# Cyruscxy/TinyPathTracer

Measured on AMD Instinct MI355X. Metric: Mrays/s at 1920x1080x1024spp (box.gltf, 8 bounces); achieved GB/s vs peak, higher is better.
Workload: dtype f32

## Files before the change

### include/tpt.h

```cpp
#ifndef TPT_H
#define TPT_H

#include <stdint.h>
#include <stddef.h>

#ifdef __cplusplus
extern "C" {
#endif

#define TPT_VERSION_MAJOR 0
#define TPT_VERSION_MINOR 1

typedef enum {
    TPT_OK = 0,
    TPT_ERR_INVALID_ARG = 1,
    TPT_ERR_HIP = 2,
    TPT_ERR_OOM = 3,
    TPT_ERR_IO = 4,
    TPT_ERR_PARSE = 5,
    TPT_ERR_NO_DEVICE = 6
} tpt_status;

typedef struct {
    float base_color[3];
    float emission_factor;
    float eta;
    float metallic;
    float subsurface, specular, roughness, specular_tint, anisotropic,
          sheen, sheen_tint, clearcoat, clearcoat_gloss;
} tpt_material;

typedef struct {
    int32_t type;
    float color[3];
    float intensity;
    float pos[3];
    float direction[3];
    float cos_outer;
    float inv_cos_cone_diff;
} tpt_light;

typedef struct {
    int32_t begin;
    int32_t mtl;
} tpt_interval;

typedef struct {
    const uint32_t* indices;      uint32_t n_faces;
    const float* vertices;        const float* normals;  uint32_t n_vertices;
    const tpt_interval* lut;      uint32_t n_objects;
    const float* vert_trans;      const float* normal_trans;
    const tpt_material* materials; uint32_t n_materials;
    const tpt_light* lights;      uint32_t n_lights;
    uint32_t flags;
} tpt_scene_desc;

#define TPT_DESC_DELTALIGHT_LAYOUT 0x1

typedef struct {
    float c2w[16];
    float vfov;
    float aspect;
    float znear;
} tpt_camera;

typedef struct {
    int32_t width, height;
    int32_t spp;
    int32_t max_depth;
    uint64_t seed;
    int32_t band_rows, band_count, band_index;
    int32_t spp_per_launch;
    int32_t flags;
    int32_t refill;
    int32_t pipe_sets, pipe_chunks;
    int32_t lanes_per_pixel;
    int32_t leaf_batch;
    int32_t wf_slots, wf_refill;
    int32_t band_list_len;
    const int32_t* band_list;
    float* band_cost;
} tpt_params;

#define TPT_FLAG_NO_COUNTERS   0x1
#define TPT_FLAG_REF_ORDER     0x2
#define TPT_FLAG_ENV_IS        0x8
#define TPT_FLAG_APPROX_CULL   0x10
#define TPT_FLAG_WAVEFRONT     0x20
#define TPT_FLAG_FAST          0x40
#define TPT_FLAG_ACCUMULATE    0x4

typedef struct {
    uint64_t traversals;
    uint64_t internal_visits;
    uint64_t leaf_tests;
    uint64_t shade_hits;
    uint64_t pixels;
    uint64_t samples;
    double rng_init_ms;
    double trace_ms;
    double resolve_ms;
    double total_ms;
    int32_t trace_launches;
    int32_t pad;
    uint64_t wide_visits;
    uint64_t accumulated_spp;
    double trace_kernel_ms;
    uint64_t local_rays;
    double tree_wait_ms;
    uint64_t resident_lanes;
    int32_t lanes_per_pixel;
    int32_t drained;
} tpt_stats;

typedef struct tpt_scene tpt_scene;
typedef struct tpt_env tpt_env;

const char* tpt_version(void);
const char* tpt_last_error(void);
int tpt_device_count(void);

tpt_status tpt_scene_create(const tpt_scene_desc* desc, int device, tpt_scene** out);
tpt_status tpt_scene_build(tpt_scene* scene);
tpt_status tpt_scene_build_async(tpt_scene* scene);
tpt_status tpt_scene_set_build_threads(tpt_scene* scene, int32_t threads);
tpt_status tpt_scene_set_transforms(tpt_scene* scene, uint32_t first_object, uint32_t n_objects,
                                    const float* vert_trans, const float* normal_trans);
void tpt_scene_destroy(tpt_scene* scene);

tpt_status tpt_env_create(const uint8_t* rgba, int32_t width, int32_t height, int device, tpt_env** out);
void tpt_env_destroy(tpt_env* env);

tpt_status tpt_env_load(const char* path, int device, tpt_env** out);
tpt_status tpt_image_load(const char* path, uint8_t** rgba, int32_t* width, int32_t* height);
void tpt_image_free(uint8_t* rgba);
tpt_status tpt_render(tpt_scene* scene, const tpt_env* env, const tpt_camera* camera,
                      const tpt_params* params, float* radiance_out, uint8_t* bgra_out,
                      tpt_stats* stats);

tpt_status tpt_render_frames(tpt_scene* scene, const tpt_env* env, const tpt_camera* camera,
                             const tpt_params* params, int32_t n_frames, const uint64_t* seeds,
                             float* const* radiance_outs, uint8_t* const* bgra_outs, tpt_stats* stats);


typedef struct {
    float*   albedo;
    float*   normal;
    float*   depth;
    int32_t* face;
    int32_t* material;
} tpt_aov;

tpt_status tpt_render_aov(tpt_scene* scene, const tpt_camera* camera, int32_t width, int32_t height,
                          const tpt_aov* out, double* trace_ms);

#define TPT_DENOISE_DEMODULATE 0x1
#define TPT_DENOISE_DIRECT     0x2

typedef struct {
    int32_t iterations;
    float   sigma_color;
    float   sigma_normal;
    float   sigma_depth;
    int32_t flags;
} tpt_denoise_params;

typedef struct { double pack_ms, filter_ms, resolve_ms; } tpt_denoise_stats;

tpt_status tpt_denoise(tpt_scene* scene, int32_t width, int32_t height, const float* radiance_in,
                       const tpt_aov* guides, const tpt_denoise_params* params, float* radiance_out,
                       uint8_t* bgra_out, tpt_denoise_stats* stats);

typedef struct tpt_history tpt_history;
tpt_status tpt_history_create(tpt_scene* scene, int32_t width, int32_t height, tpt_history** out);
tpt_status tpt_history_reset(tpt_history* h);
void tpt_history_destroy(tpt_history* h);

#define TPT_TEMPORAL_DEMODULATE 0x1
#define TPT_TEMPORAL_TILES      0x2

typedef struct {
    float   alpha;
    float   depth_tol;
    float   normal_min;
    int32_t max_history;
    int32_t flags;
} tpt_temporal_params;

typedef struct {
    double   kernel_ms;
    uint64_t reprojected;
} tpt_temporal_stats;

tpt_status tpt_temporal(tpt_history* h, const tpt_camera* camera, const float* radiance_in,
                        const tpt_aov* guides, const tpt_temporal_params* params,
                        float* radiance_out, float* variance_out, float* history_len_out,
                        uint8_t* bgra_out, tpt_temporal_stats* stats);

tpt_status tpt_temporal_motion(tpt_history* h, const tpt_camera* camera, const float* radiance_in,
                               const tpt_aov* guides, const tpt_temporal_params* params,
                               float* radiance_out, float* variance_out, float* history_len_out,
                               float* motion_out, uint8_t* bgra_out, tpt_temporal_stats* stats);

#define TPT_SVGF_DEMODULATE 0x1
#define TPT_SVGF_DIRECT     0x2

typedef struct {
    int32_t iterations;
    float   sigma_lum;
    float   sigma_normal;
    float   sigma_depth;
    int32_t min_history;
    int32_t flags;
} tpt_svgf_params;

typedef struct {
    double   pack_ms, estimate_ms, filter_ms, resolve_ms;
    uint64_t estimated;
} tpt_svgf_stats;

tpt_status tpt_denoise_svgf(tpt_scene* scene, int32_t width, int32_t height, const float* radiance_in,
                            const tpt_aov* guides, const float* variance_in, const float* history_len_in,
                            const tpt_svgf_params* params, float* radiance_out, float* variance_out,
                            uint8_t* bgra_out, tpt_svgf_stats* stats);

tpt_status tpt_scene_read_bvh(tpt_scene* scene, void* nodes36, int64_t* keys);
tpt_status tpt_scene_read_world(tpt_scene* scene, float* wverts, float* wnorms);
tpt_status tpt_debug_rng_init(int device, uint64_t seed, uint64_t first_pixel, uint32_t n, uint32_t* states);
tpt_status tpt_debug_trace_rays(tpt_scene* scene, uint32_t n, const float* origins, const float* dirs,
                                const int32_t* origin_fid, int32_t mode, int32_t* hit, float* t, float* uv);
tpt_status tpt_debug_hot_kat(int device, int32_t op, uint32_t n, const float* in, float* out);
tpt_status tpt_debug_step_latency(tpt_scene* scene, uint32_t n, const float* origins, const float* dirs,
                                  int32_t mode, int32_t flags, uint64_t* out);
int32_t tpt_wide_tree_build(int32_t n, const float* leaf_box, const uint32_t* leaf_emit, float* nodes,
                            int32_t cap, int32_t* stack_need, int32_t threads);

int32_t tpt_motion_matrices(uint32_t n_objects, const float* prev16, const float* cur16, float* out24);

typedef struct tpt_gltf tpt_gltf;
tpt_status tpt_gltf_load(const char* path, tpt_gltf** out);
tpt_status tpt_gltf_desc(const tpt_gltf* g, tpt_scene_desc* desc, tpt_camera* camera);
int tpt_gltf_missing_material(const tpt_gltf* g);
void tpt_gltf_free(tpt_gltf* g);

#ifdef __cplusplus
}
#endif
#endif
```

### tinypathtracer_amd/_lib.py

```python
from __future__ import annotations

import ctypes as C
import os

HERE = os.path.dirname(os.path.abspath(__file__))
LIB_PATH = os.environ.get("TPT_LIB", os.path.join(HERE, "libtpt.so"))

TPT_OK = 0
STATUS_NAMES = {0: "OK", 1: "INVALID_ARG", 2: "HIP_ERROR", 3: "OOM", 4: "IO", 5: "PARSE", 6: "NO_DEVICE"}
FLAG_NO_COUNTERS = 0x1
FLAG_REF_ORDER = 0x2
FLAG_ACCUMULATE = 0x4
FLAG_ENV_IS = 0x8
FLAG_APPROX_CULL = 0x10
FLAG_WAVEFRONT = 0x20
FLAG_FAST = 0x40
DESC_DELTALIGHT_LAYOUT = 0x1
DENOISE_DEMODULATE = 0x1
DENOISE_DIRECT = 0x2
TEMPORAL_DEMODULATE = 0x1
TEMPORAL_TILES = 0x2
MOTION_TRACKED, MOTION_IDENTITY, MOTION_UNTRACKED = 0, 1, 2
SVGF_DEMODULATE = 0x1
SVGF_DIRECT = 0x2


class Material(C.Structure):
    _fields_ = [("base_color", C.c_float * 3), ("emission_factor", C.c_float), ("eta", C.c_float),
                ("metallic", C.c_float), ("subsurface", C.c_float), ("specular", C.c_float),
                ("roughness", C.c_float), ("specular_tint", C.c_float), ("anisotropic", C.c_float),
                ("sheen", C.c_float), ("sheen_tint", C.c_float), ("clearcoat", C.c_float),
                ("clearcoat_gloss", C.c_float)]


class Light(C.Structure):
    _fields_ = [("type", C.c_int32), ("color", C.c_float * 3), ("intensity", C.c_float),
                ("pos", C.c_float * 3), ("direction", C.c_float * 3), ("cos_outer", C.c_float),
                ("inv_cos_cone_diff", C.c_float)]


class Interval(C.Structure):
    _fields_ = [("begin", C.c_int32), ("mtl", C.c_int32)]


class SceneDesc(C.Structure):
    _fields_ = [("indices", C.POINTER(C.c_uint32)), ("n_faces", C.c_uint32),
                ("vertices", C.POINTER(C.c_float)), ("normals", C.POINTER(C.c_float)),
                ("n_vertices", C.c_uint32), ("lut", C.POINTER(Interval)), ("n_objects", C.c_uint32),
                ("vert_trans", C.POINTER(C.c_float)), ("normal_trans", C.POINTER(C.c_float)),
                ("materials", C.POINTER(Material)), ("n_materials", C.c_uint32),
                ("lights", C.POINTER(Light)), ("n_lights", C.c_uint32), ("flags", C.c_uint32)]


class Camera(C.Structure):
    _fields_ = [("c2w", C.c_float * 16), ("vfov", C.c_float), ("aspect", C.c_float), ("znear", C.c_float)]


class Params(C.Structure):
    _fields_ = [("width", C.c_int32), ("height", C.c_int32), ("spp", C.c_int32), ("max_depth", C.c_int32),
                ("seed", C.c_uint64), ("band_rows", C.c_int32), ("band_count", C.c_int32),
                ("band_index", C.c_int32), ("spp_per_launch", C.c_int32), ("flags", C.c_int32),
                ("refill", C.c_int32), ("pipe_sets", C.c_int32), ("pipe_chunks", C.c_int32),
                ("lanes_per_pixel", C.c_int32), ("leaf_batch", C.c_int32), ("wf_slots", C.c_int32),
                ("wf_refill", C.c_int32), ("band_list_len", C.c_int32), ("band_list", C.POINTER(C.c_int32)),
                ("band_cost", C.POINTER(C.c_float))]


class SvgfParams(C.Structure):
    _fields_ = [("iterations", C.c_int32), ("sigma_lum", C.c_float), ("sigma_normal", C.c_float),
                ("sigma_depth", C.c_float), ("min_history", C.c_int32), ("flags", C.c_int32)]


class SvgfStats(C.Structure):
    _fields_ = [("pack_ms", C.c_double), ("estimate_ms", C.c_double), ("filter_ms", C.c_double),
                ("resolve_ms", C.c_double), ("estimated", C.c_uint64)]

    def as_dict(self):
        return {k: getattr(self, k) for k, _ in self._fields_}


class Stats(C.Structure):
    _fields_ = [("traversals", C.c_uint64), ("internal_visits", C.c_uint64), ("leaf_tests", C.c_uint64),
                ("shade_hits", C.c_uint64), ("pixels", C.c_uint64), ("samples", C.c_uint64),
                ("rng_init_ms", C.c_double), ("trace_ms", C.c_double), ("resolve_ms", C.c_double),
                ("total_ms", C.c_double), ("trace_launches", C.c_int32), ("pad", C.c_int32),
                ("wide_visits", C.c_uint64), ("accumulated_spp", C.c_uint64), ("trace_kernel_ms", C.c_double),
                ("local_rays", C.c_uint64), ("tree_wait_ms", C.c_double), ("resident_lanes", C.c_uint64),
                ("lanes_per_pixel", C.c_int32), ("drained", C.c_int32)]

    def as_dict(self):
        return {k: getattr(self, k) for k, _ in self._fields_ if k != "pad"}


class Aov(C.Structure):
    _fields_ = [("albedo", C.c_void_p), ("normal", C.c_void_p), ("depth", C.c_void_p), ("face", C.c_void_p),
                ("material", C.c_void_p)]


class DenoiseParams(C.Structure):
    _fields_ = [("iterations", C.c_int32), ("sigma_color", C.c_float), ("sigma_normal", C.c_float),
                ("sigma_depth", C.c_float), ("flags", C.c_int32)]


class DenoiseStats(C.Structure):
    _fields_ = [("pack_ms", C.c_double), ("filter_ms", C.c_double), ("resolve_ms", C.c_double)]

    def as_dict(self):
        return {k: getattr(self, k) for k, _ in self._fields_}


class TemporalParams(C.Structure):
    _fields_ = [("alpha", C.c_float), ("depth_tol", C.c_float), ("normal_min", C.c_float),
                ("max_history", C.c_int32), ("flags", C.c_int32)]


class TemporalStats(C.Structure):
    _fields_ = [("kernel_ms", C.c_double), ("reprojected", C.c_uint64)]

    def as_dict(self):
        return {k: getattr(self, k) for k, _ in self._fields_}


SIGNATURES = [
    ("tpt_version", C.c_char_p, []),
    ("tpt_last_error", C.c_char_p, []),
    ("tpt_device_count", C.c_int, []),
    ("tpt_scene_create", C.c_int, [C.POINTER(SceneDesc), C.c_int, C.POINTER(C.c_void_p)]),
    ("tpt_scene_build", C.c_int, [C.c_void_p]),
    ("tpt_scene_build_async", C.c_int, [C.c_void_p]),
    ("tpt_scene_set_build_threads", C.c_int, [C.c_void_p, C.c_int32]),
    ("tpt_scene_set_transforms", C.c_int, [C.c_void_p, C.c_uint32, C.c_uint32, C.c_void_p, C.c_void_p]),
    ("tpt_scene_destroy", None, [C.c_void_p]),
    ("tpt_env_create", C.c_int, [C.c_void_p, C.c_int32, C.c_int32, C.c_int, C.POINTER(C.c_void_p)]),
    ("tpt_env_destroy", None, [C.c_void_p]),
    ("tpt_env_load", C.c_int, [C.c_char_p, C.c_int, C.POINTER(C.c_void_p)]),
    ("tpt_image_load", C.c_int, [C.c_char_p, C.POINTER(C.POINTER(C.c_uint8)), C.POINTER(C.c_int32),
                                 C.POINTER(C.c_int32)]),
    ("tpt_image_free", None, [C.c_void_p]),
    ("tpt_render", C.c_int, [C.c_void_p, C.c_void_p, C.POINTER(Camera), C.POINTER(Params), C.c_void_p,
                             C.c_void_p, C.POINTER(Stats)]),
    ("tpt_render_frames", C.c_int, [C.c_void_p, C.c_void_p, C.POINTER(Camera), C.POINTER(Params), C.c_int32,
                                    C.POINTER(C.c_uint64), C.POINTER(C.c_void_p), C.POINTER(C.c_void_p),
                                    C.POINTER(Stats)]),
    ("tpt_render_aov", C.c_int, [C.c_void_p, C.POINTER(Camera), C.c_int32, C.c_int32, C.POINTER(Aov),
                                 C.POINTER(C.c_double)]),
    ("tpt_denoise", C.c_int, [C.c_void_p, C.c_int32, C.c_int32, C.c_void_p, C.POINTER(Aov),
                              C.POINTER(DenoiseParams), C.c_void_p, C.c_void_p, C.POINTER(DenoiseStats)]),
    ("tpt_history_create", C.c_int, [C.c_void_p, C.c_int32, C.c_int32, C.POINTER(C.c_void_p)]),
    ("tpt_history_reset", C.c_int, [C.c_void_p]),
    ("tpt_history_destroy", None, [C.c_void_p]),
    ("tpt_temporal", C.c_int, [C.c_void_p, C.POINTER(Camera), C.c_void_p, C.POINTER(Aov),
                               C.POINTER(TemporalParams), C.c_void_p, C.c_void_p, C.c_void_p, C.c_void_p,
                               C.POINTER(TemporalStats)]),
    ("tpt_temporal_motion", C.c_int, [C.c_void_p, C.POINTER(Camera), C.c_void_p, C.POINTER(Aov),
                                      C.POINTER(TemporalParams), C.c_void_p, C.c_void_p, C.c_void_p, C.c_void_p,
                                      C.c_void_p, C.POINTER(TemporalStats)]),
    ("tpt_motion_matrices", C.c_int32, [C.c_uint32, C.c_void_p, C.c_void_p, C.c_void_p]),
    ("tpt_denoise_svgf", C.c_int, [C.c_void_p, C.c_int32, C.c_int32, C.c_void_p, C.POINTER(Aov), C.c_void_p,
                                   C.c_void_p, C.POINTER(SvgfParams), C.c_void_p, C.c_void_p, C.c_void_p,
                                   C.POINTER(SvgfStats)]),
    ("tpt_scene_read_bvh", C.c_int, [C.c_void_p, C.c_void_p, C.c_void_p]),
    ("tpt_scene_read_world", C.c_int, [C.c_void_p, C.c_void_p, C.c_void_p]),
    ("tpt_debug_rng_init", C.c_int, [C.c_int, C.c_uint64, C.c_uint64, C.c_uint32, C.c_void_p]),
    ("tpt_debug_trace_rays", C.c_int, [C.c_void_p, C.c_uint32, C.c_void_p, C.c_void_p, C.c_void_p, C.c_int32,
                                       C.c_void_p, C.c_void_p, C.c_void_p]),
    ("tpt_debug_hot_kat", C.c_int, [C.c_int, C.c_int32, C.c_uint32, C.c_void_p, C.c_void_p]),
    ("tpt_debug_step_latency", C.c_int, [C.c_void_p, C.c_uint32, C.c_void_p, C.c_void_p, C.c_int32, C.c_int32,
                                         C.c_void_p]),
    ("tpt_wide_tree_build", C.c_int32, [C.c_int32, C.c_void_p, C.c_void_p, C.c_void_p, C.c_int32,
                                        C.POINTER(C.c_int32), C.c_int32]),
    ("tpt_gltf_load", C.c_int, [C.c_char_p, C.POINTER(C.c_void_p)]),
    ("tpt_gltf_desc", C.c_int, [C.c_void_p, C.POINTER(SceneDesc), C.POINTER(Camera)]),
    ("tpt_gltf_missing_material", C.c_int, [C.c_void_p]),
    ("tpt_gltf_free", None, [C.c_void_p]),
]


class TPTError(RuntimeError):
    def __init__(self, status, msg):
        super().__init__(f"tpt error {STATUS_NAMES.get(status, status)}: {msg}")
        self.status = status


_lib = None


def build_identity() -> dict:
    import hashlib
    h = hashlib.sha256()
    with open(LIB_PATH, "rb") as f:
        for chunk in iter(lambda: f.read(1 << 20), b""):
            h.update(chunk)
    ident = {"lib_sha256": h.hexdigest()[:16], "git_head": None}
    try:
        with open(os.path.splitext(LIB_PATH)[0] + ".build") as f:
            ident["git_head"] = f.read().strip() or None
    except OSError:
        pass
    return ident


def lib():
    global _lib
    if _lib is None:
        try:
            import torch
        except Exception:
            pass
        if not os.path.exists(LIB_PATH):
            raise ImportError(f"libtpt.so not found at {LIB_PATH}: build it with "
                              f"`make -C {HERE}` or __graft_entry__.build()")
        L = C.CDLL(LIB_PATH)
        older = bool(os.environ.get("TPT_LIB"))
        for name, res, args in SIGNATURES:
            if older and name.startswith("tpt_debug_") and not hasattr(L, name):
                continue
            fn = getattr(L, name)
            fn.restype = res
            fn.argtypes = args
        _lib = L
    return _lib


def check(status):
    if status != TPT_OK:
        raise TPTError(status, lib().tpt_last_error().decode(errors="replace"))
```

### tinypathtracer_amd/csrc/common/device_api.hpp

```cpp
#pragma once

#include <hip/hip_runtime_api.h>
#include <stdint.h>

namespace tpt {

struct DevLight {
    int32_t type;
    float color[3];
    float intensity;
    float pos[3];
    float dir[3];
    float cos_outer;
    float inv_cos_cone_diff;
};

constexpr int kMaxLights = 16;
constexpr int kRngJumps = 16;
constexpr int kJumpWords = 160 * 5;

struct TraceArgs {
    const float4* inner;
    const float4* inner4;
    int32_t n4;
    int32_t lds_nodes;
    int32_t lds_nodes_offset;
    const float4* tri;
    const float4* shade;
    const float4* mtl;
    int32_t n_faces;
    int32_t n_materials;
    int32_t n_lights;
    int32_t stack_depth;
    const DevLight* lights;
    const uint32_t* env;
    int32_t env_w, env_h;
    int32_t is_b, is_bw, is_bh;
    const float* is_cond;
    const float* is_row;
    const float* is_marg;
    float is_total;
    const int32_t* is_guide_r;
    const int32_t* is_guide_c;
    int32_t is_kr, is_kc;
    int32_t env_is;
    float c2w[16];
    float origin[3];
    float sensor_w, sensor_h;
    float half_sw, half_sh;
    float inv_w, inv_h;
    int32_t width, height;
    int32_t band_rows, band_count, band_index, band_height;
    const int32_t* band_list;
    unsigned long long* band_cost;
    int32_t n_frames;
    int32_t max_depth;
    int32_t samples;
    int32_t flags;
    int32_t refill;
    int32_t leaf_kb;
    int32_t boxes_finite;
    int32_t any_emitter;
    int32_t emit_root;
    float4 emit_box[8];
    int32_t n_emit_box;
    const float4* sliver_groups;
    const float4* sliver_list;
    int32_t n_sliver_groups;
    float cull_eps;
    int32_t graze;
    int32_t pair;
    int32_t drained;
    int32_t quad;
    int32_t xcd_run;
    int32_t xcd_rot;
    int32_t lds_rec_offset;
    int32_t rec_lds_levels;
    int32_t stack_lds_slots;
    int32_t lds_stack_offset;
    int32_t lds_mtl_offset;
    int32_t mtl_in_lds;
    uint32_t* rng;
    float* accum;
    unsigned long long* counters;
    unsigned long long* debug_waves;
};

__host__ __device__ inline int rec_words(int n_lights, int n_materials) {
    return (n_lights > 0 || n_materials >= 0x7ffe) ? 5 : 2;
}

struct ResolveArgs {
    const float* accum;
    float* radiance;
    uint8_t* bgra;
    int32_t width, height;
    int32_t band_rows, band_count, band_index, band_height;
    const int32_t* band_list;
    int32_t spp;
};

hipError_t launch_rng_init(const uint32_t* jumps, uint64_t seed, int32_t width, int32_t band_rows,
                           int32_t band_count, int32_t band_index, const int32_t* band_list, int32_t band_height,
                           int32_t height, uint32_t* rng, hipStream_t s);
hipError_t launch_rng_init_linear(const uint32_t* jumps, uint64_t seed, uint64_t first, uint32_t n,
                                  uint32_t* states_aos, hipStream_t s);

struct BuildBuffers {
    int32_t n_faces, n_vertices, n_objects, n_materials;
    const uint32_t* indices;
    const float* vertices;
    const float* normals;
    const int2* lut;
    const float* vert_trans;
    const float* normal_trans;
    const float4* mtl;
    float* wverts;
    float* wnorms;
    unsigned long long* keys;
    unsigned long long* keys_sorted;
    uint32_t* fids;
    uint32_t* fids_sorted;
    float* leaf_box;
    int2* children;
    uint32_t* parent;
    float* node_box;
    uint32_t* flags;
    uint32_t* max_depth;
    unsigned long long* bfs_keys;
    unsigned long long* bfs_keys_sorted;
    uint32_t* bfs_ids;
    uint32_t* bfs_ids_sorted;
    uint32_t* bfs_newid;
    uint32_t* emit;
    void* sort_tmp;
    size_t sort_tmp_bytes;
    float4* inner;
    float4* inner4;
    float4* tri;
    float4* shade;
    void* nodes36;
    uint32_t out_max_depth;
    uint32_t out_boxes_finite;
    uint32_t out_n4;
};
constexpr uint32_t kMaxLbvhDepth = 4096;
hipError_t build_sort_tmp_bytes(int32_t n, size_t* bytes);
hipError_t launch_build(BuildBuffers& b, hipStream_t s);
hipError_t launch_sliver_scan(const float4* tri, int32_t n, uint8_t* sliver, unsigned long long* coord_max,
                              hipStream_t s);

constexpr int kWfShards = 8;
constexpr int kWfCtlStride = 1024;
constexpr int kWfCtlWords = (4 * kWfShards + 1) * kWfCtlStride;
struct WfArgs {
    TraceArgs t;
    int32_t n_slots;
    int32_t state_words;
    int32_t rec_words;
    int32_t ordered;
    uint32_t* st0;
    uint32_t* st1;
    float* rec;
    float4* q_ray0;
    float4* q_ray1;
    float4* q_hit;
    uint32_t* ctl;
    int32_t shard_cap;
    int32_t n_claims;
    int32_t refill;
    int32_t chunk;
    int32_t batch;
    int32_t logic_blocks, trace_blocks;
    int32_t it;
    int32_t stack_lds_slots, lds_stack_offset, lds_bytes;
};
hipError_t launch_wavefront(WfArgs w, uint32_t* h_count, hipEvent_t ev[2], int32_t* iterations, hipStream_t s);

hipError_t launch_trace(const TraceArgs& a, hipStream_t s);
bool trace_quad_fits(const TraceArgs& a);
int trace_waves_per_simd();
hipError_t launch_trace_ptr(const void* a, hipStream_t s);
hipError_t launch_step_latency_ptr(const void* a, uint32_t n, const float* o, const float* d, int nodes_lds,
                                   unsigned long long* out, hipStream_t s);
hipError_t launch_resolve(const ResolveArgs& a, hipStream_t s);
hipError_t launch_hot_kat(int op, uint32_t n, const float* in, float* out, hipStream_t s);
hipError_t launch_trace_rays(const TraceArgs& a, uint32_t n, const float* o, const float* d, const int32_t* ofid,
                             int mode, int32_t* hit, float* t, float* uv, hipStream_t s);

struct AovArgs {
    float* albedo;
    float* normal;
    float* depth;
    int32_t* face;
    int32_t* material;
};
hipError_t launch_aov(const TraceArgs& a, const AovArgs& o, hipStream_t s);

struct DenoiseArgs {
    const float* radiance_in;
    const float* albedo;
    const float* normal;
    const float* depth;
    float4* color0;
    float4* guide;
    float* radiance_out;
    uint8_t* bgra;
    size_t npix;
    int32_t width, height;
    int32_t demodulate;
};
struct AtrousArgs {
    const float4* src;
    const float4* guide;
    float4* dst;
    int32_t width, height;
    int32_t step;
    float inv_sc2;
    float inv_sn2;
    float sz2;
};
hipError_t launch_denoise_pack(const DenoiseArgs& a, hipStream_t s);
hipError_t launch_atrous(const AtrousArgs& a, bool use_lds, hipStream_t s);
hipError_t launch_denoise_resolve(const DenoiseArgs& a, hipStream_t s);

struct TemporalArgs {
    float c2w[16];
    float origin[3];
    float sensor_w, sensor_h, half_sw, half_sh;
    float inv_w, inv_h;
    float prev_inv[16];
    float prev_origin[3];
    float prev_sensor_w, prev_sensor_h, prev_half_sw, prev_half_sh;
    int32_t has_prev;
    int32_t width, height;
    int32_t demodulate;
    int32_t tiles;
    float alpha, depth_tol, normal_min, max_history;
    const float* radiance_in;
    const float* albedo;
    const float* normal;
    const float* depth;
    const int32_t* material;
    const float4* prev[3];
    float4* next[3];
    float* radiance_out;
    float* variance_out;
    float* history_out;
    uint8_t* bgra;
    unsigned long long* reprojected;
};
constexpr int kTemporalSlots = 256;
constexpr int kTemporalSlotStride = 16;
hipError_t launch_temporal(const TemporalArgs& a, hipStream_t s);

struct MotionArgs {
    const int32_t* face;
    const int32_t* face_object;
    const float4* records;
    float* motion_out;
    int32_t n_faces;
};
constexpr int kMotionRecordFloats = 24;
constexpr int32_t kMotionTracked = 0, kMotionIdentity = 1, kMotionUntracked = 2;
hipError_t launch_temporal_motion(const TemporalArgs& a, const MotionArgs& mo, hipStream_t s);

struct SvgfArgs {
    const float* radiance_in;
    const float* albedo;
    const float* normal;
    const float* depth;
    const float* variance_in;
    const float* history_len;
    const float4* src;
    float4* dst;
    float4* guide;
    float* radiance_out;
    float* variance_out;
    uint8_t* bgra;
    unsigned long long* estimated;
    size_t npix;
    int32_t width, height;
    int32_t demodulate;
    int32_t passthrough;
    float min_history;
    float inv_sn2;
    float sz2;
};
struct SvgfFilterArgs {
    const float4* src;
    const float4* guide;
    float4* dst;
    int32_t width, height;
    int32_t step;
    float sigma_lum;
    float inv_sn2;
    float sz2;
};
hipError_t launch_svgf_pack(const SvgfArgs& a, hipStream_t s);
hipError_t launch_svgf_estimate(const SvgfArgs& a, hipStream_t s);
hipError_t launch_svgf_filter(const SvgfFilterArgs& a, bool use_lds, hipStream_t s);
hipError_t launch_svgf_resolve(const SvgfArgs& a, hipStream_t s);

}

namespace tpt_fast {
hipError_t launch_trace_ptr(const void* a, hipStream_t s);
hipError_t launch_step_latency_ptr(const void* a, uint32_t n, const float* o, const float* d, int nodes_lds,
                                   unsigned long long* out, hipStream_t s);
}
```

### tinypathtracer_amd/csrc/host/api.cpp

```cpp
#include <cstdlib>
#include <new>

#include "api_internal.hpp"

static thread_local std::string g_last_error;

tpt_status tpt::host::fail(tpt_status st, const std::string& msg) {
    g_last_error = msg;
    return st;
}

extern "C" {

const char* tpt_version(void) { return "tpt-mi355x 0.1 (gfx950)"; }

const char* tpt_last_error(void) { return g_last_error.c_str(); }

int tpt_device_count(void) {
    int n = 0;
    if (hipGetDeviceCount(&n) != hipSuccess) {
        (void)hipGetLastError();
        return 0;
    }
    return n;
}

tpt_status tpt_image_load(const char* path, uint8_t** rgba, int32_t* width, int32_t* height) {
    if (!path || !rgba || !width || !height) return fail(TPT_ERR_INVALID_ARG, "null argument");
    *rgba = nullptr;
    std::vector<uint8_t> px;
    int w = 0, h = 0;
    try {
        tpt::load_image(path, px, w, h);
    } catch (const tpt::io_error& e) {
        return fail(TPT_ERR_IO, e.what());
    } catch (const std::exception& e) {
        return fail(TPT_ERR_PARSE, e.what());
    }
    uint8_t* buf = static_cast<uint8_t*>(std::malloc(px.size()));
    if (!buf) return fail(TPT_ERR_OOM, "host allocation failed");
    std::memcpy(buf, px.data(), px.size());
    *rgba = buf;
    *width = w;
    *height = h;
    return TPT_OK;
}

void tpt_image_free(uint8_t* rgba) { std::free(rgba); }

tpt_status tpt_scene_read_bvh(tpt_scene* s, void* nodes36, int64_t* keys) {
    if (!s || !s->built) return fail(TPT_ERR_INVALID_ARG, "scene not built");
    DeviceGuard g(s->device);
    const size_t n = (size_t)s->n_faces;
    if (nodes36) HIP_OR_FAIL(hipMemcpy(nodes36, s->nodes36.p, 36 * (2 * n - 1), hipMemcpyDeviceToHost));
    if (keys) HIP_OR_FAIL(hipMemcpy(keys, s->keys_sorted.p, 8 * n, hipMemcpyDeviceToHost));
    return TPT_OK;
}

tpt_status tpt_scene_read_world(tpt_scene* s, float* wv, float* wn) {
    if (!s || !s->built) return fail(TPT_ERR_INVALID_ARG, "scene not built");
    DeviceGuard g(s->device);
    const size_t nv = (size_t)s->n_vertices;
    if (wv) HIP_OR_FAIL(hipMemcpy(wv, s->wverts.p, 12 * nv, hipMemcpyDeviceToHost));
    if (wn) HIP_OR_FAIL(hipMemcpy(wn, s->wnorms.p, 12 * nv, hipMemcpyDeviceToHost));
    return TPT_OK;
}

tpt_status tpt_debug_rng_init(int device, uint64_t seed, uint64_t first, uint32_t n, uint32_t* states) {
    if (!states && n) return fail(TPT_ERR_INVALID_ARG, "null output");
    int ndev = tpt_device_count();
    if (ndev <= 0) return fail(TPT_ERR_NO_DEVICE, "no HIP device available");
    if (device < 0 || device >= ndev) return fail(TPT_ERR_INVALID_ARG, "bad device index");
    DeviceGuard g(device);
    DevBuf<uint32_t> jumps, out;
    const auto& hj = host_jumps();
    HIP_OR_FAIL(jumps.upload(hj.data(), hj.size(), nullptr));
    HIP_OR_FAIL(out.alloc(6 * (size_t)std::max(n, 1u)));
    HIP_OR_FAIL(tpt::launch_rng_init_linear(jumps.p, seed, first, n, out.p, nullptr));
    HIP_OR_FAIL(hipDeviceSynchronize());
    if (n) HIP_OR_FAIL(hipMemcpy(states, out.p, 24 * (size_t)n, hipMemcpyDeviceToHost));
    return TPT_OK;
}

tpt_status tpt_debug_trace_rays(tpt_scene* s, uint32_t n, const float* o, const float* d, const int32_t* origin_fid,
                                int32_t mode, int32_t* hit, float* t, float* uv) {
    if (!s || !s->built) return fail(TPT_ERR_INVALID_ARG, "scene not built");
    if (mode < 0 || mode > 3) return fail(TPT_ERR_INVALID_ARG, "unknown trace mode");
    {
        const tpt_status bs = finish_pending(s);
        if (bs != TPT_OK) return bs;
    }
    if (n && (!o || !d || !hit || !t || !uv)) return fail(TPT_ERR_INVALID_ARG, "null argument");
    DeviceGuard g(s->device);
    DevBuf<float> dorg, ddir, dt, duv;
    DevBuf<int32_t> dhit, dofid;
    HIP_OR_FAIL(dorg.upload(o, 3 * (size_t)n, s->stream));
    if (origin_fid) {
        for (uint32_t i = 0; i < n; ++i)
            if (origin_fid[i] >= s->n_faces) return fail(TPT_ERR_INVALID_ARG, "origin face out of range");
        HIP_OR_FAIL(dofid.upload(origin_fid, n, s->stream));
    }
    HIP_OR_FAIL(ddir.upload(d, 3 * (size_t)n, s->stream));
    HIP_OR_FAIL(dhit.alloc(n));
    HIP_OR_FAIL(dt.alloc(n));
    HIP_OR_FAIL(duv.alloc(2 * (size_t)n));
    tpt::TraceArgs a{};
    fill_trace_args(s, nullptr, nullptr, a);
    HIP_OR_FAIL(tpt::launch_trace_rays(a, n, dorg.p, ddir.p, origin_fid ? dofid.p : nullptr, mode, dhit.p, dt.p, duv.p,
                                       s->stream));
    HIP_OR_FAIL(hipStreamSynchronize(s->stream));
    if (n) {
        HIP_OR_FAIL(hipMemcpy(hit, dhit.p, 4 * (size_t)n, hipMemcpyDeviceToHost));
        HIP_OR_FAIL(hipMemcpy(t, dt.p, 4 * (size_t)n, hipMemcpyDeviceToHost));
        HIP_OR_FAIL(hipMemcpy(uv, duv.p, 8 * (size_t)n, hipMemcpyDeviceToHost));
    }
    return TPT_OK;
}

tpt_status tpt_debug_step_latency(tpt_scene* s, uint32_t n, const float* o, const float* d, int32_t mode,
                                  int32_t flags, uint64_t* out) {
    if (!s || !s->built) return fail(TPT_ERR_INVALID_ARG, "scene not built");
    if (n > 64 || (n && (!o || !d || !out))) return fail(TPT_ERR_INVALID_ARG, "1..64 rays and outputs");
    if (mode < 0 || mode > 2)
        return fail(TPT_ERR_INVALID_ARG, "mode: 0 nodes in global memory, 1 in LDS, 2 four lanes per ray");
    if (mode == 2 && n > 16) return fail(TPT_ERR_INVALID_ARG, "four lanes per ray: at most 16 rays");
    {
        const tpt_status bs = finish_pending(s);
        if (bs != TPT_OK) return bs;
    }
    const int nodes_lds = mode == 1 ? s->n4 : (mode == 2 ? -1 : 0);
    if ((size_t)std::max(nodes_lds, 0) * 128 + 64 * 256 * sizeof(int) > 160 * 1024)
        return fail(TPT_ERR_INVALID_ARG, "the 4-wide tree does not fit in LDS");
    DeviceGuard g(s->device);
    DevBuf<float> dorg, ddir;
    DevBuf<unsigned long long> dout;
    HIP_OR_FAIL(dorg.upload(o, 3 * (size_t)std::max(n, 1u), s->stream));
    HIP_OR_FAIL(ddir.upload(d, 3 * (size_t)std::max(n, 1u), s->stream));
    HIP_OR_FAIL(dout.alloc(4 * 64));
    tpt::TraceArgs a{};
    fill_trace_args(s, nullptr, nullptr, a);
    if (mode == 2 && a.stack_depth + 3 > 64) return fail(TPT_ERR_INVALID_ARG, "four lanes per ray: stack too deep");
    if (flags & TPT_FLAG_FAST) {
        a.cull_eps = 0.0f;
        a.n_sliver_groups = 0;
        a.graze = 0;
        HIP_OR_FAIL(tpt_fast::launch_step_latency_ptr(&a, n, dorg.p, ddir.p, nodes_lds, dout.p, s->stream));
    } else {
        HIP_OR_FAIL(tpt::launch_step_latency_ptr(&a, n, dorg.p, ddir.p, nodes_lds, dout.p, s->stream));
    }
    HIP_OR_FAIL(hipStreamSynchronize(s->stream));
    HIP_OR_FAIL(hipMemcpy(out, dout.p, 4 * 64 * sizeof(unsigned long long), hipMemcpyDeviceToHost));
    return TPT_OK;
}

tpt_status tpt_debug_hot_kat(int device, int32_t op, uint32_t n, const float* in, float* out) {
    static const int kIn[4] = {12, 15, 16, 3}, kOut[4] = {2, 4, 6, 3};
    if (op < 0 || op > 3) return fail(TPT_ERR_INVALID_ARG, "unknown KAT op");
    if (n && (!in || !out)) return fail(TPT_ERR_INVALID_ARG, "null argument");
    int ndev = tpt_device_count();
    if (ndev <= 0) return fail(TPT_ERR_NO_DEVICE, "no HIP device available");
    if (device < 0 || device >= ndev) return fail(TPT_ERR_INVALID_ARG, "bad device index");
    DeviceGuard g(device);
    DevBuf<float> din, dout;
    HIP_OR_FAIL(din.upload(in, (size_t)kIn[op] * n, nullptr));
    HIP_OR_FAIL(dout.alloc((size_t)kOut[op] * std::max(n, 1u)));
    HIP_OR_FAIL(tpt::launch_hot_kat(op, n, din.p, dout.p, nullptr));
    HIP_OR_FAIL(hipDeviceSynchronize());
    if (n) HIP_OR_FAIL(hipMemcpy(out, dout.p, sizeof(float) * kOut[op] * (size_t)n, hipMemcpyDeviceToHost));
    return TPT_OK;
}

tpt_status tpt_gltf_load(const char* path, tpt_gltf** out) {
    if (!path || !out) return fail(TPT_ERR_INVALID_ARG, "null argument");
    *out = nullptr;
    tpt_gltf* g = new (std::nothrow) tpt_gltf();
    if (!g) return fail(TPT_ERR_OOM, "host allocation failed");
    try {
        tpt::load_gltf(path, g->hs);
    } catch (const tpt::io_error& e) {
        delete g;
        return fail(TPT_ERR_IO, e.what());
    } catch (const std::exception& e) {
        delete g;
        return fail(TPT_ERR_PARSE, e.what());
    }
    *out = g;
    return TPT_OK;
}

tpt_status tpt_gltf_desc(const tpt_gltf* g, tpt_scene_desc* d, tpt_camera* cam) {
    if (!g || !d) return fail(TPT_ERR_INVALID_ARG, "null argument");
    const tpt::HostScene& h = g->hs;
    d->indices = h.indices.data();
    d->n_faces = (uint32_t)(h.indices.size() / 3);
    d->vertices = h.vertices.data();
    d->normals = h.normals.data();
    d->n_vertices = (uint32_t)(h.vertices.size() / 3);
    d->lut = h.lut.data();
    d->n_objects = (uint32_t)h.lut.size();
    d->vert_trans = h.vert_trans.data();
    d->normal_trans = h.normal_trans.data();
    d->materials = h.materials.empty() ? nullptr : h.materials.data();
    d->n_materials = (uint32_t)h.materials.size();
    d->lights = h.lights.empty() ? nullptr : h.lights.data();
    d->n_lights = (uint32_t)h.lights.size();
    d->flags = 0;
    if (cam) *cam = h.camera;
    return TPT_OK;
}

int tpt_gltf_missing_material(const tpt_gltf* g) { return g && g->hs.missing_material ? 1 : 0; }

void tpt_gltf_free(tpt_gltf* g) { delete g; }

}
```

### tinypathtracer_amd/csrc/host/api_render.cpp

```cpp
#include <chrono>
#include <cstdio>
#include <cstdlib>

#include "api_internal.hpp"

#ifndef TPT_XCD_ROT
#define TPT_XCD_ROT 1
#endif

void tpt::host::fill_trace_args(tpt_scene* s, const tpt_env* env, const tpt_camera* cam, tpt::TraceArgs& a) {
    a.inner = s->inner.p;
    a.inner4 = s->inner4.p;
    a.n4 = s->n4;
    a.tri = s->tri.p;
    a.shade = s->shade.p;
    a.mtl = s->mtl.p;
    a.n_faces = s->n_faces;
    a.n_materials = s->n_materials;
    a.n_lights = s->n_lights;
    a.lights = s->lights.p;
    a.stack_depth = s->stack_depth;
    a.boxes_finite = s->boxes_finite;
    a.any_emitter = s->any_emitter;
    a.emit_root = s->emit_root;
    a.n_emit_box = s->any_emitter ? s->n_emit_box : 0;
    for (int k = 0; k < a.n_emit_box; ++k) {
        const float* b = s->emit_box + 6 * k;
        a.emit_box[2 * k] = make_float4(b[0], b[1], b[2], 0.0f);
        a.emit_box[2 * k + 1] = make_float4(b[3], b[4], b[5], 0.0f);
    }
    a.sliver_groups = s->sliver_groups.p;
    a.sliver_list = s->sliver_list.p;
    a.n_sliver_groups = s->n_sliver_groups;
    a.cull_eps = s->cull_eps;
    a.graze = 1;
    a.env = env ? env->texels.p : nullptr;
    a.env_w = env ? env->w : 0;
    a.env_h = env ? env->h : 0;
    a.is_b = env ? env->is_b : 1;
    a.is_bw = env ? env->is_bw : 0;
    a.is_bh = env ? env->is_bh : 0;
    a.is_cond = env ? env->is_cond.p : nullptr;
    a.is_row = env ? env->is_row.p : nullptr;
    a.is_marg = env ? env->is_marg.p : nullptr;
    a.is_total = env ? env->is_total : 0.0f;
    a.is_guide_r = env ? env->is_guide_r.p : nullptr;
    a.is_guide_c = env ? env->is_guide_c.p : nullptr;
    a.is_kr = env ? env->is_kr : 1;
    a.is_kc = env ? env->is_kc : 1;
    if (cam) set_camera(a, camera_consts(cam));
}

namespace {

tpt_status render_wavefront(tpt_scene* s, const tpt::TraceArgs& a, const tpt_params* p, int n_frames, int bh,
                            double& trace_ms, double& kernel_ms, int& launches) {
    hipStream_t st = s->stream;
    const bool ordered = !(p->flags & TPT_FLAG_REF_ORDER);
    const bool lights = !ordered || a.env_is || tpt::rec_words(s->n_lights, s->n_materials) == 5;
    tpt::WfArgs w{};
    w.t = a;
    w.t.samples = p->spp;
    w.ordered = ordered ? 1 : 0;
    w.state_words = lights ? 32 : 16;
    w.rec_words = lights ? 5 : 2;
    const size_t gx = (size_t)(p->width + 15) / 16, gy = (size_t)((bh + 15) / 16) * (size_t)n_frames;
    const size_t claims = gx * gy * 256;
    if (bh <= 0) return TPT_OK;
    if (claims > (size_t)INT32_MAX / 2) return fail(TPT_ERR_INVALID_ARG, "wavefront: frame batch too large");
    if (p->wf_slots < 0 || p->wf_refill < 0 || p->wf_refill > 64)
        return fail(TPT_ERR_INVALID_ARG, "wavefront: wf_slots >= 0, wf_refill 0..64");
    size_t slots = p->wf_slots > 0 ? (size_t)p->wf_slots : claims;
    slots = std::min(slots, claims);
    slots = (slots + 255) / 256 * 256;
    w.n_claims = (int32_t)claims;
    w.n_slots = (int32_t)slots;
    HIP_OR_FAIL(s->wf_rec.alloc(slots * (size_t)p->max_depth * (size_t)w.rec_words));
    const size_t cap = ((slots / 256) + tpt::kWfShards - 1) / tpt::kWfShards * 256;
    const size_t qn = cap * tpt::kWfShards;
    HIP_OR_FAIL(s->wf_q0.alloc(2 * qn));
    HIP_OR_FAIL(s->wf_q1.alloc(2 * qn));
    HIP_OR_FAIL(s->wf_hit.alloc(qn));
    HIP_OR_FAIL(s->wf_state.alloc(2 * qn * (size_t)w.state_words));
    HIP_OR_FAIL(s->wf_ctl.alloc(tpt::kWfCtlWords));
    HIP_OR_FAIL(s->wf_count.alloc(2 * tpt::kWfShards));
    w.shard_cap = (int32_t)cap;
    for (auto& e : s->wf_ev)
        if (!e) HIP_OR_FAIL(hipEventCreateWithFlags(&e, hipEventDisableTiming));
    w.st0 = s->wf_state.p;
    w.st1 = s->wf_state.p + qn * (size_t)w.state_words;
    w.rec = s->wf_rec.p;
    w.q_ray0 = s->wf_q0.p;
    w.q_ray1 = s->wf_q1.p;
    w.q_hit = s->wf_hit.p;
    w.ctl = s->wf_ctl.p;
    w.refill = p->wf_refill > 0 ? p->wf_refill : 40;
    w.chunk = 128;
    w.batch = 32;
    w.logic_blocks = (int32_t)((std::min<size_t>((slots + 255) / 256, 2048) + tpt::kWfShards - 1) / tpt::kWfShards *
                               tpt::kWfShards);
    w.trace_blocks = 0;
    int32_t iters = 0;
    HIP_OR_FAIL(tpt::launch_wavefront(w, s->wf_count.p, s->wf_ev, &iters, st));
    HIP_OR_FAIL(hipEventRecord(s->ev[2], st));
    HIP_OR_FAIL(hipEventSynchronize(s->ev[2]));
    float ms = 0.0f;
    HIP_OR_FAIL(hipEventElapsedTime(&ms, s->ev[1], s->ev[2]));
    trace_ms = ms;
    kernel_ms = ms;
    launches = 1 + 2 * iters;
    return TPT_OK;
}

struct WaveDump {
    const char* path = nullptr;
    size_t words = 0;
};

tpt_status render_planned(tpt_scene* s, const tpt::TraceArgs& a, const tpt_params* p, const tpt::LaunchPlan& plan,
                          size_t list_len, WaveDump& dump, double& trace_ms, double& kernel_ms, int& launches) {
    hipStream_t st = s->stream;
    const int nset = plan.nset;
    const size_t nf = (size_t)a.n_frames;
    const bool listed = a.band_list != nullptr;
#if defined(TPT_PROFILE_PHASES) || defined(TPT_VERIFY_CULL)
    dump.path = std::getenv("TPT_DEBUG_WAVES");
#endif
    const size_t dbg_launch =
        8ull * 4 * (size_t)((a.width + 7) / 8) * (size_t)((std::max(a.band_height, 1) + 7) / 8) * nf;
    dump.words = dbg_launch * std::max<size_t>(plan.launches.size(), 1);
    if (dump.path) {
        HIP_OR_FAIL(s->debug.alloc(dump.words));
        HIP_OR_FAIL(hipMemsetAsync(s->debug.p, 0, dump.words * sizeof(unsigned long long), st));
    }
    HIP_OR_FAIL(s->ensure_launch_events(2 * plan.launches.size()));
    if (listed && nset > 1) {
        for (int k = 0; k < nset; ++k)
            std::copy(plan.set_list[k].begin(), plan.set_list[k].end(), s->band_lists_h.begin() + plan.set_off[k]);
        HIP_OR_FAIL(hipMemcpyAsync(s->band_lists.p + list_len, s->band_lists_h.data() + list_len,
                                   list_len * sizeof(int32_t), hipMemcpyHostToDevice, st));
    }
    hipStream_t qs[tpt::kMaxPipe] = {st};
    if (nset > 1) {
        HIP_OR_FAIL(s->ensure_pipe(nset));
        HIP_OR_FAIL(hipEventRecord(s->pipe_ev[0], st));
        for (int k = 0; k < nset; ++k) {
            qs[k] = s->pipe[k];
            HIP_OR_FAIL(hipStreamWaitEvent(qs[k], s->pipe_ev[0], 0));
        }
    }
#define SET_OR_FAIL(expr)                                                                                      \
    do {                                                                                                       \
        hipError_t e_ = (expr);                                                                                \
        if (e_ != hipSuccess) {                                                                                \
            for (int k_ = 0; nset > 1 && k_ < nset; ++k_) (void)hipStreamSynchronize(qs[k_]);                  \
            (void)hipStreamSynchronize(st);                                                                    \
            return fail(e_ == hipErrorOutOfMemory ? TPT_ERR_OOM : TPT_ERR_HIP,                                 \
                        std::string(#expr) + ": " + hipGetErrorString(e_));                                    \
        }                                                                                                      \
    } while (0)
    int set_chunks[tpt::kMaxPipe] = {};
    for (size_t oi = 0; oi < plan.order.size(); ++oi) {
        const size_t j = plan.order[oi];
        const int k = plan.launches[j].set;
        if (plan.set_rows[k] <= 0) continue;
        tpt::TraceArgs ak = a;
        ak.samples = plan.launches[j].samples;
        ak.xcd_rot = TPT_XCD_ROT ? (set_chunks[k]++ & 7) : 0;
        if (nset > 1) {
            ak.band_count = a.band_count * nset;
            ak.band_index = a.band_index + k * a.band_count;
            ak.band_height = plan.set_rows[k];
            if (listed) ak.band_list = s->band_lists.p + plan.set_off[k];
        }
#ifdef TPT_VERIFY_CULL
        if (dump.path) ak.debug_waves = s->debug.p;
#else
        if (dump.path) ak.debug_waves = s->debug.p + oi * dbg_launch;
#endif
        SET_OR_FAIL(hipEventRecord(s->lev[2 * j], qs[k]));
        SET_OR_FAIL((p->flags & TPT_FLAG_FAST) ? tpt_fast::launch_trace_ptr(&ak, qs[k]) : tpt::launch_trace(ak, qs[k]));
        SET_OR_FAIL(hipEventRecord(s->lev[2 * j + 1], qs[k]));
    }
    for (int k = 0; nset > 1 && k < nset; ++k) {
        SET_OR_FAIL(hipEventRecord(s->pipe_ev[1 + k], qs[k]));
        SET_OR_FAIL(hipStreamWaitEvent(st, s->pipe_ev[1 + k], 0));
    }
    SET_OR_FAIL(hipEventRecord(s->ev[2], st));
    SET_OR_FAIL(hipEventSynchronize(s->ev[2]));
#undef SET_OR_FAIL
    float ms = 0.0f;
    HIP_OR_FAIL(hipEventElapsedTime(&ms, s->ev[1], s->ev[2]));
    trace_ms = ms;
    for (size_t j = 0; j < plan.launches.size(); ++j) {
        if (plan.set_rows[plan.launches[j].set] <= 0) continue;
        HIP_OR_FAIL(hipEventElapsedTime(&ms, s->lev[2 * j], s->lev[2 * j + 1]));
        kernel_ms += ms;
        ++launches;
    }
    return TPT_OK;
}

}

extern "C" {

tpt_status tpt_render(tpt_scene* s, const tpt_env* env, const tpt_camera* cam, const tpt_params* p,
                      float* radiance_out, uint8_t* bgra_out, tpt_stats* stats) {
    if (!p) return fail(TPT_ERR_INVALID_ARG, "null argument");
    const uint64_t seed = p->seed;
    return tpt_render_frames(s, env, cam, p, 1, &seed, &radiance_out, &bgra_out, stats);
}

tpt_status tpt_render_frames(tpt_scene* s, const tpt_env* env, const tpt_camera* cam, const tpt_params* p,
                             int32_t n_frames, const uint64_t* seeds, float* const* radiance_outs,
                             uint8_t* const* bgra_outs, tpt_stats* stats) {
    auto t_start = std::chrono::steady_clock::now();
    if (!s || !cam || !p || !seeds) return fail(TPT_ERR_INVALID_ARG, "null argument");
    if (n_frames < 1 || n_frames > 65535) return fail(TPT_ERR_INVALID_ARG, "bad frame count");
    if (!s->built) return fail(TPT_ERR_INVALID_ARG, "scene not built (call tpt_scene_build)");
    if (p->width <= 0 || p->height <= 0 || p->spp <= 0 || p->max_depth < 1 || p->max_depth > 64)
        return fail(TPT_ERR_INVALID_ARG, "bad frame parameters");
    if ((int64_t)p->width * p->height > (int64_t)1 << 30) return fail(TPT_ERR_INVALID_ARG, "frame too large");
    const int band_rows = p->band_rows > 0 ? p->band_rows : 16;
    const bool listed = p->band_list != nullptr;
    const int band_count = listed ? 1 : (p->band_count > 0 ? p->band_count : 1);
    const int band_index = listed ? 0 : p->band_index;
    if (!listed && (p->band_index < 0 || p->band_index >= band_count))
        return fail(TPT_ERR_INVALID_ARG, "bad band index");
    if (env && env->device != s->device) return fail(TPT_ERR_INVALID_ARG, "env lives on another device");
    const int W = p->width, H = p->height;
    const int n_bands = (H + band_rows - 1) / band_rows;
    std::vector<int32_t> list;
    if (listed) {
        if (p->band_list_len < 0 || p->band_list_len > n_bands)
            return fail(TPT_ERR_INVALID_ARG, "band_list_len: 0 .. ceil(height / band_rows)");
        list.assign(p->band_list, p->band_list + p->band_list_len);
        std::vector<uint8_t> seen((size_t)n_bands, 0);
        const bool partial = H % band_rows != 0;
        for (size_t i = 0; i < list.size(); ++i) {
            if (list[i] < 0 || list[i] >= n_bands || seen[(size_t)list[i]]++ ||
                (partial && list[i] == n_bands - 1 && i + 1 != list.size()))
                return fail(TPT_ERR_INVALID_ARG, "band_list: distinct band ids below ceil(height / band_rows), "
                                                 "a short last band last");
        }
    }
    DeviceGuard g(s->device);
    hipStream_t st = s->stream;
    const size_t npix = (size_t)W * (size_t)H;
    const size_t nf = (size_t)n_frames;
    const int bh = listed ? tpt::band_list_rows(list.data(), list.size(), band_rows, H)
                          : tpt::band_height_of(H, band_rows, band_count, band_index);
    const std::vector<uint64_t> fseeds(seeds, seeds + nf);

    const bool resume = (p->flags & TPT_FLAG_ACCUMULATE) && s->acc_valid && s->acc_w == W && s->acc_h == H &&
                        s->acc_rows == band_rows && s->acc_count == band_count && s->acc_index == band_index &&
                        s->acc_list == list && s->acc_seeds == fseeds && s->rng.n == 6 * npix * nf &&
                        s->accum.n == 3 * npix * nf;
    s->acc_valid = false;
    HIP_OR_FAIL(s->rng.alloc(6 * npix * nf));
    HIP_OR_FAIL(s->accum.alloc(3 * npix * nf));
    HIP_OR_FAIL(s->counters.alloc(32));
    if (!resume) HIP_OR_FAIL(hipMemsetAsync(s->accum.p, 0, 3 * npix * nf * sizeof(float), st));
    HIP_OR_FAIL(hipMemsetAsync(s->counters.p, 0, 32 * sizeof(unsigned long long), st));
    const int32_t* d_list = nullptr;
    if (listed && !list.empty()) {
        s->band_lists_h.assign(2 * list.size(), 0);
        std::copy(list.begin(), list.end(), s->band_lists_h.begin());
        HIP_OR_FAIL(s->band_lists.alloc(std::max(s->band_lists.n, 2 * list.size())));
        HIP_OR_FAIL(hipMemcpyAsync(s->band_lists.p, s->band_lists_h.data(), list.size() * sizeof(int32_t),
                                   hipMemcpyHostToDevice, st));
        d_list = s->band_lists.p;
    }
    if (p->band_cost) {
        HIP_OR_FAIL(s->band_cost.alloc(std::max<size_t>(s->band_cost.n, (size_t)n_bands)));
        HIP_OR_FAIL(hipMemsetAsync(s->band_cost.p, 0, (size_t)n_bands * sizeof(unsigned long long), st));
    }

    HIP_OR_FAIL(hipEventRecord(s->ev[0], st));
    if (bh > 0 && !resume)
        for (size_t f = 0; f < nf; ++f)
            HIP_OR_FAIL(tpt::launch_rng_init(s->jumps.p, fseeds[f], W, band_rows, band_count, band_index, d_list, bh,
                                             H, s->rng.p + f * 6 * npix, st));
    HIP_OR_FAIL(hipEventRecord(s->ev[1], st));
    double tree_wait_ms = 0.0;
    {
        const tpt_status bs = finish_pending(s, &tree_wait_ms);
        if (bs != TPT_OK) return bs;
    }
    const uint64_t total_spp = (resume ? s->acc_spp : 0) + (uint64_t)p->spp;
    if (total_spp > (uint64_t)INT32_MAX) return fail(TPT_ERR_INVALID_ARG, "accumulated spp overflow");

    tpt::TraceArgs a{};
    fill_trace_args(s, env, cam, a);
    a.inv_w = 1.0f / (float)W;
    a.inv_h = 1.0f / (float)H;
    a.width = W;
    a.height = H;
    a.band_rows = band_rows;
    a.band_count = band_count;
    a.band_index = band_index;
    a.band_list = d_list;
    a.band_cost = p->band_cost ? s->band_cost.p : nullptr;
    a.band_height = bh;
    a.n_frames = n_frames;
    a.max_depth = p->max_depth;
    a.flags = p->flags;
    if (p->flags & (TPT_FLAG_APPROX_CULL | TPT_FLAG_FAST)) {
        a.cull_eps = 0.0f;
        a.n_sliver_groups = 0;
        a.graze = 0;
    }
    a.env_is = ((p->flags & TPT_FLAG_ENV_IS) && env && env->is_total > 0.0f) ? 1 : 0;
    a.rng = s->rng.p;
    a.accum = s->accum.p;
    a.counters = s->counters.p;
    a.debug_waves = nullptr;

    tpt::PlanInput pin;
    pin.width = W;
    pin.band_rows = band_rows;
    pin.bh = bh;
    pin.height = H;
    pin.n_frames = n_frames;
    pin.band_count = band_count;
    pin.band_index = band_index;
    pin.listed = listed;
    pin.list = list.data();
    pin.list_len = list.size();
    pin.spp = p->spp;
    pin.flags = p->flags;
    pin.lanes_per_pixel = p->lanes_per_pixel;
    pin.refill = p->refill;
    pin.leaf_batch = p->leaf_batch;
    pin.spp_per_launch = p->spp_per_launch;
    pin.pipe_sets = p->pipe_sets;
    pin.pipe_chunks = p->pipe_chunks;
    pin.n_faces = s->n_faces;
    pin.n_lights = s->n_lights;
    pin.n_materials = s->n_materials;
    pin.resident_lanes = s->resident_lanes;
    pin.env_is = a.env_is != 0;
    pin.quad_fits = tpt::trace_quad_fits(a);
    const tpt::LaunchPlan plan = tpt::plan_launches(pin);
    if (plan.status != TPT_OK) return fail(plan.status, plan.message);
    a.pair = plan.pair ? 1 : 0;
    a.quad = plan.quad ? 1 : 0;
    a.refill = plan.refill;
    a.drained = plan.drained ? 1 : 0;
    a.leaf_kb = plan.leaf_kb;
    a.xcd_run = plan.xcd_run;
    a.xcd_rot = 0;

    double trace_ms = 0.0, kernel_ms = 0.0;
    int launches = 0;
    WaveDump dump;
    if ((p->flags & TPT_FLAG_WAVEFRONT) && (p->flags & (TPT_FLAG_FAST | TPT_FLAG_APPROX_CULL)))
        return fail(TPT_ERR_INVALID_ARG, "TPT_FLAG_WAVEFRONT runs the exact traversal only");
    const tpt_status ts = (p->flags & TPT_FLAG_WAVEFRONT)
                              ? render_wavefront(s, a, p, n_frames, bh, trace_ms, kernel_ms, launches)
                              : render_planned(s, a, p, plan, list.size(), dump, trace_ms, kernel_ms, launches);
    if (ts != TPT_OK) return ts;

    HIP_OR_FAIL(hipEventRecord(s->ev[2], st));
    Staging sg(st);
    for (size_t f = 0; f < nf; ++f) {
        tpt::ResolveArgs r{};
        r.accum = s->accum.p + f * 3 * npix;
        r.width = W;
        r.height = H;
        r.band_rows = band_rows;
        r.band_count = band_count;
        r.band_index = band_index;
        r.band_list = d_list;
        r.band_height = bh;
        r.spp = (int)total_spp;
        HIP_OR_FAIL(sg.inout(s->radiance_tmp, radiance_outs ? radiance_outs[f] : nullptr, 3 * npix, &r.radiance));
        HIP_OR_FAIL(sg.inout(s->bgra_tmp, bgra_outs ? bgra_outs[f] : nullptr, 4 * npix, &r.bgra));
        if (bh > 0 && (r.radiance || r.bgra)) HIP_OR_FAIL(tpt::launch_resolve(r, st));
        HIP_OR_FAIL(sg.finish());
    }
    HIP_OR_FAIL(hipEventRecord(s->ev[3], st));
    unsigned long long cnt[32] = {0};
    HIP_OR_FAIL(hipMemcpyAsync(cnt, s->counters.p, sizeof cnt, hipMemcpyDeviceToHost, st));
    HIP_OR_FAIL(hipStreamSynchronize(st));
    if (cnt[4] != 0) return fail(TPT_ERR_HIP, "traversal stack overflow (BVH deeper than sized)");
    if (p->band_cost) {
        s->band_cost_h.resize((size_t)n_bands);
        HIP_OR_FAIL(hipMemcpy(s->band_cost_h.data(), s->band_cost.p, (size_t)n_bands * sizeof(unsigned long long),
                              hipMemcpyDeviceToHost));
        for (int b = 0; b < n_bands; ++b) {
            const bool mine = listed ? std::find(list.begin(), list.end(), b) != list.end()
                                     : b % band_count == band_index;
            if (mine) p->band_cost[b] = (float)((double)s->band_cost_h[(size_t)b] / 100.0);
        }
    }
    if (dump.path) {
#ifdef TPT_VERIFY_CULL
        const size_t dump_words = std::min<size_t>(dump.words, 16 * std::min<unsigned long long>(cnt[24], 4096));
#else
        const size_t dump_words = dump.words;
#endif
        std::vector<unsigned long long> h(dump_words);
        if (dump_words)
            HIP_OR_FAIL(hipMemcpy(h.data(), s->debug.p, dump_words * sizeof(unsigned long long), hipMemcpyDeviceToHost));
        if (FILE* f = std::fopen(dump.path, "wb")) {
            std::fwrite(h.data(), sizeof(unsigned long long), h.size(), f);
            std::fclose(f);
        }
    }
#if defined(TPT_PROFILE_PHASES) || defined(TPT_VERIFY_CULL)
    if (std::getenv("TPT_DEBUG_COUNTERS")) {
        std::fprintf(stderr, "tpt counters:");
        for (int i = 0; i < 32; ++i) std::fprintf(stderr, " %llu", cnt[i]);
        std::fprintf(stderr, "\n");
    }
#endif
    if (stats) {
        std::memset(stats, 0, sizeof *stats);
        stats->traversals = cnt[0];
        stats->internal_visits = cnt[1];
        stats->wide_visits = cnt[5];
        stats->local_rays = cnt[9];
        stats->accumulated_spp = total_spp;
        stats->leaf_tests = cnt[2];
        stats->shade_hits = cnt[3];
        stats->pixels = (uint64_t)W * (uint64_t)bh * (uint64_t)nf;
        stats->samples = stats->pixels * (uint64_t)p->spp;
        float ms = 0.0f;
        (void)hipEventElapsedTime(&ms, s->ev[0], s->ev[1]);
        stats->rng_init_ms = ms;
        stats->trace_ms = trace_ms;
        stats->trace_kernel_ms = kernel_ms;
        stats->tree_wait_ms = tree_wait_ms;
        (void)hipEventElapsedTime(&ms, s->ev[2], s->ev[3]);
        stats->resolve_ms = ms;
        stats->trace_launches = launches;
        stats->resident_lanes = s->resident_lanes;
        stats->lanes_per_pixel = plan.quad ? 4 : (plan.pair_kernel ? 2 : 1);
        stats->drained = a.drained;
        stats->total_ms =
            std::chrono::duration<double, std::milli>(std::chrono::steady_clock::now() - t_start).count();
    }
    s->acc_valid = true;
    s->acc_w = W;
    s->acc_h = H;
    s->acc_rows = band_rows;
    s->acc_count = band_count;
    s->acc_index = band_index;
    s->acc_list = list;
    s->acc_seeds = fseeds;
    s->acc_spp = total_spp;
    return TPT_OK;
}

}
```

### tinypathtracer_amd/csrc/kernels/trace.hip

```cpp
#include <type_traits>

#include "trace_dev.hpp"

namespace tpt {
#ifdef TPT_VERIFY_CULL
template <bool ORDERED>
__device__ __forceinline__ void trav_lane(Trav& r, const TraceArgs& a, LaneStack<int>& stk, uint32_t& c_ovf);
constexpr unsigned long long kVerifyCap = 4096;
__device__ __noinline__ void verify_ray(const TraceArgs& a, const Trav& r, int phase, const float4* mtl) {
    Trav q;
    trav_begin(q, r.o, r.d, TM_CLOSEST);
    LaneStack<int> vs;
    vs.lds = nullptr;
    vs.nlds = 0;
    uint32_t ovf = 0;
    trav_lane<false>(q, a, vs, ovf);
    bool bad;
    if (r.mode == TM_ANY) {
        bad = (q.fid >= 0) != (r.fid >= 0);
    } else if (r.mode == TM_CLOSEST && phase != 3) {
        bad = (q.fid != r.fid) || (__float_as_uint(q.t) != __float_as_uint(r.t)) ||
              (__float_as_uint(q.u) != __float_as_uint(r.u)) || (__float_as_uint(q.v) != __float_as_uint(r.v));
    } else {
        const float er = q.fid >= 0 ? mtl[2 * __float_as_int(a.shade[3 * q.fid].w)].w : 0.0f;
        const float eo = (r.fid >= 0 && r.mode != TM_OCCLUDED) ? mtl[2 * __float_as_int(a.shade[3 * r.fid].w)].w : 0.0f;
        bad = er != eo;
    }
    if (!bad) return;
    const unsigned long long k = atomicAdd(&a.counters[24], 1ull);
    if (k >= kVerifyCap || !a.debug_waves) return;
    unsigned long long* o = a.debug_waves + 16 * k;
    o[0] = (unsigned long long)r.mode;
    o[1] = (unsigned long long)phase;
    o[2] = (unsigned long long)(long long)r.fid;
    o[3] = (unsigned long long)(long long)q.fid;
    o[4] = __float_as_uint(r.t);
    o[5] = __float_as_uint(q.t);
    o[6] = __float_as_uint(r.o.x);
    o[7] = __float_as_uint(r.o.y);
    o[8] = __float_as_uint(r.o.z);
    o[9] = __float_as_uint(r.d.x);
    o[10] = __float_as_uint(r.d.y);
    o[11] = __float_as_uint(r.d.z);
    o[12] = (unsigned long long)(long long)r.hpos;
    o[13] = (unsigned long long)(long long)q.hpos;
    o[14] = __float_as_uint(r.u);
    o[15] = (unsigned long long)(r.fin ? 1u : 0u) | ((unsigned long long)__float_as_uint(r.lim) << 32);
}
#endif

template <int MAXD, bool ORDERED, bool LIGHTS, bool MTL_LDS, typename StackT, bool ENVIS = false, bool PAIR = false,
          bool DRAIN = false, bool QUAD = false, bool NOEMIT = false>
__global__ __launch_bounds__(256, ENVIS ? TPT_TRACE_WAVES_IS
                                        : (PAIR ? TPT_TRACE_WAVES_PAIR
                                                : (QUAD ? TPT_TRACE_WAVES_QUAD
                                                        : (DRAIN ? TPT_TRACE_WAVES_DRAIN : TPT_TRACE_WAVES))))
void k_trace(TraceArgs a) {
    static_assert(!PAIR || (ORDERED && LIGHTS), "pair mode: ordered variants with 5-word records");
    static_assert(!QUAD || (ORDERED && !LIGHTS && !PAIR && !ENVIS && !DRAIN), "four lanes per pixel: one-lane logic");
    extern __shared__ __attribute__((aligned(16))) char lds[];
    const int tid = threadIdx.x, lane = tid & 63, wave = tid >> 6;
    const int nfr = a.n_frames > 0 ? a.n_frames : 1;
    int bx = (int)blockIdx.x, by = (int)blockIdx.y;
    if (a.xcd_run > 0) {
        const int g = a.xcd_run, k = ((bx & 7) + by + a.xcd_rot) & 7, m = bx >> 3;
        bx = ((m / g) * 8 + k) * g + m % g;
    }
    const int frame = by % nfr;
    const bool side = PAIR && (lane & 1);
    const bool lead = !QUAD || (lane & 3) == 0;
    const int pl = PAIR ? (lane >> 1) : (QUAD ? (lane >> 2) : lane);
    const int x = QUAD ? bx * 8 + (wave & 1) * 4 + (pl & 3) : bx * 16 + (wave & 1) * 8 + (pl & 7);
    const int ly = PAIR   ? (by / nfr) * 8 + (wave >> 1) * 4 + (pl >> 3)
                   : QUAD ? (by / nfr) * 8 + (wave >> 1) * 4 + (pl >> 2)
                          : (by / nfr) * 16 + (wave >> 1) * 8 + (pl >> 3);
    const int y = band_row(ly, a.band_rows, a.band_count, a.band_index, a.band_list);
    const bool pixel = x < a.width && ly < a.band_height && y < a.height;
    const unsigned long long t_cost0 = a.band_cost ? wall_clock64() : 0ull;
    const bool active = pixel && !side;
    uint32_t c_trav = 0, c_inner = 0, c_wide = 0, c_leaf = 0, c_shade = 0, c_ovf = 0;
    uint32_t c_local = 0;
    const size_t npix = (size_t)a.width * (size_t)a.height;
    const size_t off = active ? (size_t)x + (size_t)y * (size_t)a.width : 0;
    uint32_t* const g_rng = a.rng + (size_t)frame * 6 * npix;
    float* const g_acc = a.accum + (size_t)frame * 3 * npix;
    const int nint = a.n_faces - 1;
    TPT_LDS char* slds = (TPT_LDS char*)lds;
    TPT_LDS LdsF4* smtl = (TPT_LDS LdsF4*)(slds + a.lds_mtl_offset);
    if constexpr (MTL_LDS) {
        for (int i = tid; i < 2 * (a.n_materials + 1); i += 256) {
            const float4 m = a.mtl[i];
            smtl[i].x = m.x;
            smtl[i].y = m.y;
            smtl[i].z = m.z;
            smtl[i].w = m.w;
        }
    }
    TPT_LDS LdsF4* snodes = (TPT_LDS LdsF4*)(slds + a.lds_nodes_offset);
    for (int i = tid; i < 8 * a.lds_nodes; i += 256) {
        const float4 m = a.inner4[i];
        snodes[i].x = m.x;
        snodes[i].y = m.y;
        snodes[i].z = m.z;
        snodes[i].w = m.w;
    }
    if (MTL_LDS || a.lds_nodes > 0) __syncthreads();
    auto MT = [&](int i) -> float4 {
        if constexpr (MTL_LDS) {
            return make_float4(smtl[i].x, smtl[i].y, smtl[i].z, smtl[i].w);
        } else {
            return a.mtl[i];
        }
    };
    LaneStack<StackT, QUAD> stk;
    stk.lds = (TPT_LDS StackT*)(slds + a.lds_stack_offset) + (QUAD ? (tid & ~3) : tid);
    stk.nlds = a.stack_lds_slots;
    PathRecords<MAXD, PAIR ? 128 : 256> rec;
    rec.lds = (TPT_LDS float*)(slds + a.lds_rec_offset) + (PAIR ? wave * 32 + pl : tid);
    rec.nlds = a.rec_lds_levels;
    rec.words = LIGHTS ? 5 : 2;

    uint32_t st[6];
    V3 total = v3(0.0f, 0.0f, 0.0f);
    if (active) {
#pragma unroll
        for (int i = 0; i < 6; ++i) st[i] = g_rng[i * npix + off];
        total = v3(g_acc[off], g_acc[npix + off], g_acc[2 * npix + off]);
    }
    int remaining = a.samples;
    int phase = PH_CAMERA;
    int depth = 0, li = 0;
    uint32_t mk = 0;
    bool env_pending = false;
    V3 env_k = v3(0.0f, 0.0f, 0.0f);
    float env_x1 = 0.0f, env_x2 = 0.0f;
    V3 env_nf = v3(0.0f, 0.0f, 0.0f);
    V3 rd = v3(0.0f, 0.0f, 0.0f), nd = rd, nrm = rd, direct = rd;
    Trav r;
    trav_begin(r, rd, v3(1.0f, 1.0f, 1.0f), TM_CLOSEST);
    int ts = active ? TS_DONE : ((PAIR && side && pixel) ? TS_IDLE : TS_DEAD);
#ifdef TPT_VERIFY_CULL
    bool vpend = false;
#endif
    bool sl_pend = false;
    Surf gsurf = no_surface();
    bool graze_next = false;
    float4 pq0 = make_float4(0.0f, 0.0f, 0.0f, 0.0f), pq1 = pq0, pq2 = pq0;
    const int refill = a.refill;
    bool delegated = false, post = false, ready = false;
    bool post_env = false;
    int pend = -1, jlevel = 0;
    auto put_level = [&](uint32_t pm, V3 dl) {
        if constexpr (PAIR) {
            rec.template put_dst<true>(depth, mk, pm, dl);
            if (!delegated) {
                rec.put(depth, 2, direct.x);
                rec.put(depth, 3, direct.y);
                rec.put(depth, 4, direct.z);
            }
        } else {
            rec.put_dst(depth, mk, pm, dl);
        }
    };

#ifdef TPT_PROFILE_PHASES
    const unsigned long long t_wave0 = wall_clock64();
    unsigned long long p_done = 0, p_trav = 0, p_steps = 0, t_iter0 = 0, t_loop0 = 0, p_outer = 0;
    unsigned long long p_lt = 0, p_lw = 0, p_lx = 0, p_lp = 0;
    unsigned int p_sec[8] = {0, 0, 0, 0, 0, 0, 0, 0};
    unsigned long long t_sec = 0;
    bool p_lead = false;
#endif
#ifdef TPT_PROFILE_PHASES
#define TPT_SEC_BEGIN()                                                       \
    {                                                                         \
        __builtin_amdgcn_s_waitcnt(0);                                        \
        t_sec = wall_clock64();                                               \
        p_lead = __builtin_amdgcn_readfirstlane(lane) == lane;                \
    }
#define TPT_SEC(k)                                                            \
    {                                                                         \
        __builtin_amdgcn_s_waitcnt(0);                                        \
        const unsigned long long t_ = wall_clock64();                         \
        if (p_lead) p_sec[k] += (unsigned int)(t_ - t_sec);                   \
        t_sec = t_;                                                           \
    }
#else
#define TPT_SEC_BEGIN()
#define TPT_SEC(k)
#endif
    for (;;) {
#ifdef TPT_PROFILE_PHASES
        {
            const unsigned long long now = wall_clock64();
            if (t_loop0) p_trav += now - t_loop0;
            t_iter0 = now;
        }
#endif
        if (ORDERED && a.n_sliver_groups > 0) {
            if (ts == TS_DONE && sl_pend) {
                sl_pend = false;
                sliver_pass(r, a, c_leaf);
            }
        }
        if (ORDERED && !NOEMIT && ts == TS_DONE && phase == PH_PROBE && r.fin && r.fid >= 0 && r.mode == TM_EMIT &&
            a.graze && grazing(Surf{a.shade[3 * r.fid + 1].w, a.shade[3 * r.fid + 2].w}, r.d)) {
            trav_begin(r, r.o, r.d, r.mode, a.boxes_finite != 0, a.emit_root, a.cull_eps, true);
            ts = TS_TRAV;
            sl_pend = false;
        }
        if (ORDERED && !NOEMIT && ts == TS_DONE && phase == PH_PROBE && r.mode == TM_EMIT && r.fid >= 0) {
            r.mode = TM_OCCL;
            r.node = 0;
            r.sp = 0;
            r.pend = -1;
            ts = TS_TRAV;
            sl_pend = true;
        }
#ifdef TPT_VERIFY_CULL
        if (ts == TS_DONE && vpend) {
            vpend = false;
            if (!(phase == PH_EXT && r.fin && r.fid >= 0 && a.graze &&
                  grazing(Surf{a.shade[3 * r.fid + 1].w, a.shade[3 * r.fid + 2].w}, r.d)))
                verify_ray(a, r, phase, a.mtl);
        }
#endif
#ifdef TPT_PROFILE_PHASES
        if (__ballot(ts == TS_DONE) != 0ull) p_lp += (unsigned long long)__popcll(__ballot(ts == TS_DONE));
#endif
        const bool in_pass = ts == TS_DONE;
        bool finish = false;
        bool redo = false;
        bool shadow = false;
        bool tg = false;
        V3 L = v3(0.0f, 0.0f, 0.0f), td = rd;
        if (in_pass) {
            TPT_SEC_BEGIN()
            bool lights_next = false, after = false;
            if (!LIGHTS) rd = r.d;
            Surf gpass = gsurf;
            if (phase == PH_EXT) {
                if (r.fid < 0) {
                    if (a.env) L = env_lookup<ENVIS>(a.env, a.env_w, a.env_h, rd);
                    finish = true;
                } else {
                    const float4* sh = a.shade + 3 * r.fid;
                    const float4 s0 = sh[0], s1 = sh[1], s2 = sh[2];
                    redo = ORDERED && r.fin && a.graze && grazing(Surf{s1.w, s2.w}, rd);
                    if (!redo) {
                        ++c_shade;
                        const float w = 1.0f - r.u - r.v;
                        nrm = normalize(((w * v3(s0.x, s0.y, s0.z)) + (r.u * v3(s1.x, s1.y, s1.z))) +
                                        (r.v * v3(s2.x, s2.y, s2.z)));
                        gpass = a.graze ? Surf{s1.w, s2.w} : no_surface();
                        if constexpr (LIGHTS) gsurf = gpass;
                        r.o = r.o + (r.t * rd);
                        const int mtl = __float_as_int(s0.w);
                        const float4 m1 = MT(2 * mtl + 1);
                        float af;
                        const float prob = new_direction(rd, nrm, m1.x, m1.y, st, nd, af);
                        graze_next = grazing(gpass, nd);
                        rec.put(depth, 0, af);
                        mk = (uint32_t)mtl | (p_kind(prob) << 30);
                        direct = v3(0.0f, 0.0f, 0.0f);
                        li = 0;
                        delegated = false;
                        env_pending = ENVIS && !(m1.x > 0.0f) && !(m1.y > 0.0f);
                        lights_next = true;
                    }
                }
            } else if (LIGHTS && phase == PH_SHADOW) {
                if (r.fid < 0) {
                    V3 ldir, lrad;
                    light_sample(a.lights, li, r.o, ldir, lrad);
                    const float4 m0 = MT(2 * (mk & 0x3fffffffu));
                    direct = direct + (v3(m0.x, m0.y, m0.z) * lrad);
                }
                ++li;
                lights_next = true;
            } else if (ENVIS && phase == PH_ENVSHADOW) {
                if (r.fid < 0) direct = direct + env_k;
                lights_next = true;
            } else if (!NOEMIT && phase == PH_PROBE) {
                V3 dl = LIGHTS ? direct : v3(0.0f, 0.0f, 0.0f);
                uint32_t pm = kNoProbe;
                if (r.fid >= 0 && r.mode != TM_OCCLUDED) {
                    pm = (uint32_t)__float_as_int(a.shade[3 * r.fid].w);
                    const float e = MT(2 * pm).w;
                    if (!PAIR) dl = (v3(1.0f, 1.0f, 1.0f) * v3(e, e, e)) + dl;
                }
                put_level(pm, dl);
                after = true;
            } else if (PAIR && phase == PH_WAIT) {
                L = direct;
                finish = true;
            }
            TPT_SEC(1)
            td = rd;
            tg = redo;
            if (PAIR && lights_next && !side && li == 0 && pend < 0 && (a.n_lights > 0 || (ENVIS && env_pending))) {
                post = true;
                jlevel = depth;
                pend = depth;
                delegated = true;
                li = a.n_lights;
                if (ENVIS && env_pending) {
                    env_pending = false;
                    env_x1 = xorwow_uniform(st);
                    env_x2 = xorwow_uniform(st);
                    env_nf = (dot(rd, nrm) > 0.0f ? -1.0f : 1.0f) * nrm;
                    post_env = true;
                }
            }
            if (PAIR && lights_next && side && li >= a.n_lights && !(ENVIS && env_pending)) {
                ready = true;
                ts = TS_IDLE;
                lights_next = false;
            }
            if (lights_next) {
                const float4 m1 = MT(2 * (mk & 0x3fffffffu) + 1);
                if (LIGHTS && li < a.n_lights) {
                    V3 lrad;
                    light_sample(a.lights, li, r.o, td, lrad);
                    tg = grazing(gsurf, td);
                    phase = PH_SHADOW;
                    shadow = true;
                } else {
                    bool env_ray = false;
                    if (ENVIS && env_pending) {
                        env_pending = false;
                        V3 nf = env_nf;
                        float x1 = env_x1, x2 = env_x2;
                        if (!(PAIR && side)) {
                            nf = (dot(rd, nrm) > 0.0f ? -1.0f : 1.0f) * nrm;
                            x1 = xorwow_uniform(st);
                            x2 = xorwow_uniform(st);
                        }
                        if (env_is_sample(a, nf, x1, x2, td, env_k)) {
                            phase = PH_ENVSHADOW;
                            shadow = true;
                            env_ray = true;
                            tg = grazing(gsurf, td);
                        }
                    }
                    if (env_ray) {
                    } else if (PAIR && side) {
                        ready = true;
                        ts = TS_IDLE;
                    } else if (!(m1.x >= 1.0f || m1.y > 0.0f)) {
                        float af2;
                        new_direction(rd, nrm, m1.x, m1.y, st, td, af2);
                        if ((ORDERED && (NOEMIT || !a.any_emitter)) ||
                            (ORDERED && probe_misses_emitters(a, r.o, td))) {
                            ++c_trav;
                            ++c_local;
                            put_level(kNoProbe, direct);
                            after = true;
                        } else {
                            tg = grazing(gpass, td);
                            phase = PH_PROBE;
                        }
                    } else {
                        put_level(kNoProbe, direct);
                        after = true;
                    }
                }
            }
            TPT_SEC(2)
            if (after) {
                const float e = MT(2 * (mk & 0x3fffffffu)).w;
                if (e > 0.0f) {
                    L = e * v3(1.0f, 1.0f, 1.0f);
                    finish = true;
                } else {
                    rd = nd;
                    td = rd;
                    tg = graze_next;
                    ++depth;
                    if (depth == a.max_depth) finish = true;
                    else phase = PH_EXT;
                }
            }
            TPT_SEC(3)
        }
        bool woke = false;
        if constexpr (PAIR && ENVIS) {
            const int jready = __shfl_xor((int)ready, 1, 64);
            const float dx = __shfl_xor(direct.x, 1, 64), dy = __shfl_xor(direct.y, 1, 64),
                        dz = __shfl_xor(direct.z, 1, 64);
            const int rl = __shfl_xor(jlevel, 1, 64);
            if (!side && jready) {
                rec.put(rl, 2, dx);
                rec.put(rl, 3, dy);
                rec.put(rl, 4, dz);
                pend = -1;
                if (!in_pass && phase == PH_WAIT) {
                    woke = true;
                    ts = TS_DONE;
                    L = direct;
                    finish = true;
                    td = rd;
                }
            }
            ready = false;
        }
        if (in_pass || woke) {
            if (PAIR && finish && pend >= 0) {
                direct = L;
                phase = PH_WAIT;
                ts = TS_IDLE;
                finish = false;
            }
            bool unwound = false;
            if constexpr (DRAIN && !LIGHTS && MAXD == 8) {
                static_assert(!PAIR && !LIGHTS, "DRAIN unwind: one-lane 2-word records");
                if (finish && rec.nlds >= 8) {
                    unwound = true;
                    float af[8];
                    uint32_t w1[8];
#pragma unroll
                    for (int k = 0; k < 8; ++k) {
                        af[k] = rec.template lds_at<2>(k, 0);
                        w1[k] = k < depth ? __float_as_uint(rec.template lds_at<2>(k, 1)) : (kNoProbe << 15);
                    }
                    float4 mb[8];
                    float ee[8];
#pragma unroll
                    for (int k = 0; k < 8; ++k) {
                        mb[k] = MT(2 * (w1[k] & 0x7fffu));
                        const uint32_t pm = (w1[k] >> 15) & 0x7fffu;
                        ee[k] = MT(2 * (pm == kNoProbe ? 0u : pm)).w;
                    }
#pragma unroll
                    for (int k = 7; k >= 0; --k) {
                        if (k < depth) {
                            const V3 att = af[k] * v3(mb[k].x, mb[k].y, mb[k].z);
                            const uint32_t kind = w1[k] >> 30;
                            const float prob = kind == 0u ? af[k] : (kind == 1u ? -0.0f : 0.0f);
                            const float ivp = 1.0f / prob;
                            const uint32_t pm = (w1[k] >> 15) & 0x7fffu;
                            const float e = pm == kNoProbe ? 0.0f : ee[k];
                            const V3 dst = pm == kNoProbe ? v3(0.0f, 0.0f, 0.0f)
                                                          : (v3(1.0f, 1.0f, 1.0f) * v3(e, e, e)) + v3(0.0f, 0.0f, 0.0f);
                            L = ivp * ((dst + L) * att);
                        }
                    }
                    total = total + L;
                    phase = PH_CAMERA;
                }
            }
            if (finish && !unwound) {
                for (int k = depth - 1; k >= 0; --k) {
                    const float af = rec.get(k, 0);
                    const uint32_t w1 = __float_as_uint(rec.get(k, 1));
                    const bool packed = rec.words == 2;
                    const float4 mb = MT(2 * (w1 & ((packed || PAIR) ? 0x7fffu : 0x3fffffffu)));
                    const V3 att = af * v3(mb.x, mb.y, mb.z);
                    const uint32_t kind = w1 >> 30;
                    const float prob = kind == 0u ? af : (kind == 1u ? -0.0f : 0.0f);
                    const float ivp = 1.0f / prob;
                    V3 dst;
                    if (packed) {
                        const uint32_t pm = (w1 >> 15) & 0x7fffu;
                        const float e = pm == kNoProbe ? 0.0f : MT(2 * pm).w;
                        dst = pm == kNoProbe ? v3(0.0f, 0.0f, 0.0f)
                                             : (v3(1.0f, 1.0f, 1.0f) * v3(e, e, e)) + v3(0.0f, 0.0f, 0.0f);
                    } else if (PAIR) {
                        const uint32_t pm = (w1 >> 15) & 0x7fffu;
                        const V3 dd = v3(rec.get(k, 2), rec.get(k, 3), rec.get(k, 4));
                        const float e = pm == kNoProbe ? 0.0f : MT(2 * pm).w;
                        dst = pm == kNoProbe ? dd : (v3(1.0f, 1.0f, 1.0f) * v3(e, e, e)) + dd;
                    } else {
                        dst = v3(rec.get(k, 2), rec.get(k, 3), rec.get(k, 4));
                    }
                    L = ivp * ((dst + L) * att);
                }
                total = total + L;
                phase = PH_CAMERA;
            }
            TPT_SEC(4)
            V3 to = r.o;
            if (phase == PH_CAMERA) {
                if (remaining == 0) {
                    ts = TS_DEAD;
                } else {
                    --remaining;
                    const float ju = xorwow_uniform(st);
                    const float jv = xorwow_uniform(st);
                    float lx = ju * 1.0f, lyf = jv * 1.0f;
                    lx = lx + (float)x;
                    lyf = lyf + (float)y;
                    lx = lx * a.inv_w;
                    lyf = lyf * a.inv_h;
                    lx = lx * a.sensor_w;
                    lyf = lyf * a.sensor_h;
                    float r4[4];
                    mat4_vec4(a.c2w, lx - a.half_sw, lyf - a.half_sh, 0.0f - 1.0f, 0.0f, r4);
                    rd = normalize(v3(r4[0], r4[1], r4[2]));
                    td = rd;
                    to = v3(a.origin[0], a.origin[1], a.origin[2]);
                    tg = false;
                    depth = 0;
                    phase = PH_EXT;
                }
            }
            TPT_SEC(5)
            if (ts != TS_DEAD && ts != TS_IDLE) {
                if (!redo) ++c_trav;
                trav_begin(r, to, td, shadow ? TM_ANY : ((ORDERED && phase == PH_PROBE) ? TM_EMIT : TM_CLOSEST),
                           a.boxes_finite != 0, a.emit_root, a.cull_eps, tg);
                ts = TS_TRAV;
                sl_pend = true;
#ifdef TPT_VERIFY_CULL
                vpend = true;
#endif
            }
            TPT_SEC(6)
        }
        if constexpr (PAIR) {
            const int jpost = __shfl_xor((int)post, 1, 64);
            const float jx = __shfl_xor(r.o.x, 1, 64), jy = __shfl_xor(r.o.y, 1, 64), jz = __shfl_xor(r.o.z, 1, 64);
            const int jmk = __shfl_xor((int)mk, 1, 64), jl = __shfl_xor(jlevel, 1, 64);
            const Surf jgs = Surf{__shfl_xor(gsurf.x, 1, 64), __shfl_xor(gsurf.y, 1, 64)};
            bool jenv = false;
            if constexpr (ENVIS) {
                jenv = __shfl_xor((int)post_env, 1, 64) != 0;
                const float e1 = __shfl_xor(env_x1, 1, 64), e2 = __shfl_xor(env_x2, 1, 64);
                const float n0 = __shfl_xor(env_nf.x, 1, 64), n1 = __shfl_xor(env_nf.y, 1, 64),
                            n2 = __shfl_xor(env_nf.z, 1, 64);
                if (side && jpost) {
                    env_pending = jenv;
                    env_x1 = e1;
                    env_x2 = e2;
                    env_nf = v3(n0, n1, n2);
                }
            }
            if (side && jpost) {
                mk = (uint32_t)jmk;
                jlevel = jl;
                gsurf = jgs;
                li = 0;
                direct = v3(0.0f, 0.0f, 0.0f);
                V3 ldir, lrad;
                const V3 jo = v3(jx, jy, jz);
                bool go = true;
                if (a.n_lights > 0) {
                    light_sample(a.lights, 0, jo, ldir, lrad);
                    phase = PH_SHADOW;
                } else if (ENVIS && env_pending) {
                    env_pending = false;
                    go = env_is_sample(a, env_nf, env_x1, env_x2, ldir, env_k);
                    phase = PH_ENVSHADOW;
                } else {
                    go = false;
                }
                if (go) {
                    ++c_trav;
                    trav_begin(r, jo, ldir, TM_ANY, a.boxes_finite != 0, a.emit_root, a.cull_eps, grazing(gsurf, ldir));
                    ts = TS_TRAV;
                    sl_pend = true;
#ifdef TPT_VERIFY_CULL
                    vpend = true;
#endif
                } else {
                    r.o = jo;
                    ready = true;
                    ts = TS_IDLE;
                }
            }
            post = false;
            post_env = false;
            const int jready = __shfl_xor((int)ready, 1, 64);
            const float dx = __shfl_xor(direct.x, 1, 64), dy = __shfl_xor(direct.y, 1, 64),
                        dz = __shfl_xor(direct.z, 1, 64);
            const int rl = __shfl_xor(jlevel, 1, 64);
            if (!side && jready) {
                rec.put(rl, 2, dx);
                rec.put(rl, 3, dy);
                rec.put(rl, 4, dz);
                pend = -1;
                if (phase == PH_WAIT) ts = TS_DONE;
            }
            ready = false;
            const int pdead = __shfl_xor((int)(ts == TS_DEAD), 1, 64);
            if (side && ts == TS_IDLE && pdead) ts = TS_DEAD;
        }
        if (__ballot(ts != TS_DEAD) == 0ull) break;
#ifdef TPT_PROFILE_PHASES
        t_loop0 = wall_clock64();
        p_done += t_loop0 - t_iter0;
        ++p_outer;
#endif
        const int thr = refill;
        for (;;) {
#ifdef TPT_PROFILE_PHASES
            ++p_steps;
#endif
            const int cnt = __popcll(__ballot(lead && ts == TS_TRAV));
#ifdef TPT_PROFILE_PHASES
            p_lt += (unsigned long long)cnt;
            p_lw += (unsigned long long)__popcll(__ballot(ts == TS_DONE));
            p_lx += (unsigned long long)__popcll(__ballot(ts == TS_DEAD || ts == TS_IDLE));
#endif
            if (cnt == 0) break;
            if (cnt < thr && __ballot(lead && ts == TS_DONE) != 0ull) break;
            bool inner_ready = false, has = false, blocked = false;
            const bool at_inner = ts == TS_TRAV && r.node >= 0 && r.node < nint;
            if (ts == TS_TRAV) {
                if (at_inner) {
                    int next;
                    if (QUAD && r.fin) {
                        ++c_wide;
                        bool stop;
                        next = inner_visit4_quad(r, a.inner4, a.tri, nint, a.cull_eps, stk, r.sp, stop, c_leaf);
                        if (stop) {
                            r.sp = 0;
                            next = -1;
                        }
                    } else if (ORDERED && r.fin) {
                        ++c_wide;
                        next = inner_visit4(r, a.inner4, a.lds_nodes, stk, r.sp);
                    } else {
                        ++c_inner;
                        int deferred;
                        bool push;
                        inner_visit<ORDERED>(r, a.inner, next, push, deferred);
                        stk.put(r.sp, deferred);
                        r.sp += push ? 1 : 0;
                    }
                    if (r.sp > a.stack_depth) {
                        ++c_ovf;
                        r.sp = 0;
                        next = -1;
                    }
                    r.node = next >= 0 ? next : (r.sp == 0 ? -1 : stk.get(--r.sp));
                }
                if (r.node >= nint && r.pend < 0) {
                    r.pend = r.node - nint;
                    r.node = r.sp == 0 ? -1 : stk.get(--r.sp);
                    if constexpr (DRAIN) {
                        const TriQ tq = tri_load(a.tri, r.pend);
                        pq0 = tq.q0;
                        pq1 = tq.q1;
                        pq2 = tq.q2;
                    }
                }
                has = r.pend >= 0;
                inner_ready = r.node >= 0 && r.node < nint;
                blocked = has && !inner_ready;
            }
            const unsigned long long hb = __ballot(has);
            if (hb != 0ull) {
                const bool go = __popcll(__ballot(blocked)) >= a.leaf_kb || __popcll(hb) >= TPT_LEAF_KP ||
                                __ballot(inner_ready) == 0ull;
                if (go && has) {
                    ++c_leaf;
                    const bool stop = DRAIN ? leaf_test_q<ORDERED>(r, pq0, pq1, pq2, r.pend, a.cull_eps)
                                            : leaf_test<ORDERED>(r, a.tri, r.pend, a.cull_eps);
                    if (stop) {
                        r.node = -1;
                        r.sp = 0;
                    }
                    r.pend = -1;
                }
            }
            if (ts == TS_TRAV && r.node < 0 && r.pend < 0) ts = TS_DONE;
        }
    }
    if (active && lead) {
#pragma unroll
        for (int i = 0; i < 6; ++i) g_rng[i * npix + off] = st[i];
        g_acc[off] = total.x;
        g_acc[npix + off] = total.y;
        g_acc[2 * npix + off] = total.z;
    }
    if (!lead) {
        c_trav = c_inner = c_wide = c_leaf = c_shade = c_ovf = c_local = 0;
    }
    const unsigned long long s_wide = wave_sum(c_wide), s_local = wave_sum(c_local);
    const unsigned long long s_trav = wave_sum(c_trav), s_inner = wave_sum(c_inner), s_leaf = wave_sum(c_leaf),
                             s_shade = wave_sum(c_shade), s_ovf = wave_sum(c_ovf);
#ifdef TPT_PROFILE_PHASES
    unsigned long long m_trav = c_trav;
#pragma unroll
    for (int off = 32; off > 0; off >>= 1) {
        const unsigned long long o2 = __shfl_xor(m_trav, off, 64);
        m_trav = o2 > m_trav ? o2 : m_trav;
    }
#endif
#ifdef TPT_PROFILE_PHASES
    unsigned long long s_sec[7];
#pragma unroll
    for (int k = 0; k < 7; ++k) s_sec[k] = wave_sum(p_sec[k]);
    if (lane == 0) {
#pragma unroll
        for (int k = 0; k < 7; ++k) atomicAdd(&a.counters[16 + k], s_sec[k]);
    }
#endif
    if (lane == 0) {
        atomicAdd(&a.counters[0], s_trav);
        atomicAdd(&a.counters[1], s_inner);
        atomicAdd(&a.counters[2], s_leaf);
        atomicAdd(&a.counters[3], s_shade);
        if (s_ovf) atomicAdd(&a.counters[4], s_ovf);
        atomicAdd(&a.counters[5], s_wide);
        atomicAdd(&a.counters[9], s_local);
        if (a.band_cost && ly < a.band_height)
            atomicAdd(&a.band_cost[band_of(ly / a.band_rows, a.band_count, a.band_index, a.band_list)],
                      wall_clock64() - t_cost0);
#ifdef TPT_PROFILE_PHASES
        atomicAdd(&a.counters[6], p_done);
        atomicAdd(&a.counters[7], p_trav);
        atomicAdd(&a.counters[8], p_steps);
        atomicAdd(&a.counters[12], p_outer);
        atomicAdd(&a.counters[25], p_lt);
        atomicAdd(&a.counters[26], p_lw);
        atomicAdd(&a.counters[27], p_lx);
        atomicAdd(&a.counters[28], p_lp);
        const unsigned long long life = wall_clock64() - t_wave0;
        atomicMax(&a.counters[13], life);
        atomicAdd(&a.counters[14], life);
        atomicAdd(&a.counters[15], 1ull);
        if (a.debug_waves) {
            const unsigned long long wid =
                ((unsigned long long)blockIdx.y * gridDim.x + blockIdx.x) * 4 + wave;
            unsigned long long* o = a.debug_waves + 8 * wid;
            o[0] = t_wave0;
            o[1] = life;
            o[2] = p_steps;
            o[3] = p_outer;
            o[4] = s_trav;
            o[5] = s_wide;
            o[6] = m_trav;
            o[7] = p_done;
        }
#endif
    }
}

__global__ void k_resolve(ResolveArgs a) {
    const int x = blockIdx.x * blockDim.x + threadIdx.x;
    const int ly = blockIdx.y;
    if (x >= a.width || ly >= a.band_height) return;
    const int y = band_row(ly, a.band_rows, a.band_count, a.band_index, a.band_list);
    if (y >= a.height) return;
    const size_t npix = (size_t)a.width * (size_t)a.height;
    const size_t off = (size_t)x + (size_t)y * (size_t)a.width;
    const float inv = 1.0f / (float)a.spp;
    const float r = (0.0f + a.accum[off]) * inv;
    const float g = (0.0f + a.accum[npix + off]) * inv;
    const float b = (0.0f + a.accum[2 * npix + off]) * inv;
    if (a.radiance) {
        a.radiance[3 * off] = r;
        a.radiance[3 * off + 1] = g;
        a.radiance[3 * off + 2] = b;
    }
    if (a.bgra) {
        uint8_t* px = a.bgra + 4 * ((size_t)(a.height - y - 1) * (size_t)a.width + (size_t)x);
        px[0] = to_uchar(b);
        px[1] = to_uchar(g);
        px[2] = to_uchar(r);
    }
}

constexpr int kRaysLdsSlots = 48;

__global__ __launch_bounds__(256) void k_trace_rays(TraceArgs a, uint32_t n, const float* __restrict__ o,
                                                    const float* __restrict__ d, const int32_t* __restrict__ ofid,
                                                    int mode, int32_t* hit, float* t, float* uv) {
    extern __shared__ __attribute__((aligned(16))) char lds[];
    const uint32_t i = blockIdx.x * 256 + threadIdx.x;
    uint32_t c_ovf = 0;
    if (i < n) {
        Trav r;
        const V3 ro = v3(o[3 * i], o[3 * i + 1], o[3 * i + 2]), rdir = v3(d[3 * i], d[3 * i + 1], d[3 * i + 2]);
        LaneStack<int> stk;
        stk.lds = (TPT_LDS int*)lds + threadIdx.x;
        stk.nlds = kRaysLdsSlots;
        int fid;
        if (mode == 0) {
            trav_begin(r, ro, rdir, TM_CLOSEST);
            trav_lane<false>(r, a, stk, c_ovf);
            fid = r.fid;
        } else {
            const int tm = mode == 1 ? TM_CLOSEST : (mode == 2 ? TM_ANY : TM_EMIT);
            const Surf gs = (a.graze && ofid && ofid[i] >= 0)
                                ? Surf{a.shade[3 * ofid[i] + 1].w, a.shade[3 * ofid[i] + 2].w}
                                : no_surface();
            trav_begin(r, ro, rdir, tm, a.boxes_finite != 0, a.emit_root, a.cull_eps, grazing(gs, rdir));
            uint32_t c_leaf = 0;
            if (mode == 3 && probe_misses_emitters(a, ro, rdir)) r.node = -1;
            trav_lane<true>(r, a, stk, c_ovf);
            if (a.n_sliver_groups > 0) sliver_pass(r, a, c_leaf);
            if (r.fin && r.fid >= 0 && ((mode == 1 && r.mode == TM_CLOSEST) || (mode == 3 && r.mode == TM_EMIT)) &&
                a.graze && grazing(Surf{a.shade[3 * r.fid + 1].w, a.shade[3 * r.fid + 2].w}, r.d)) {
                trav_begin(r, ro, rdir, r.mode, a.boxes_finite != 0, a.emit_root, a.cull_eps, true);
                trav_lane<true>(r, a, stk, c_ovf);
            }
            if (mode == 3 && r.mode == TM_EMIT && r.fid >= 0) {
                r.mode = TM_OCCL;
                r.node = 0;
                r.sp = 0;
                trav_lane<true>(r, a, stk, c_ovf);
                if (a.n_sliver_groups > 0) sliver_pass(r, a, c_leaf);
            }
            fid = (mode == 3 && r.mode == TM_OCCLUDED) ? -2 : r.fid;
            if (mode == 3 && fid >= 0) {
                const int m = __float_as_int(a.shade[3 * fid].w);
                if (a.mtl[2 * m].w == 0.0f) fid = -2;
            }
        }
        hit[i] = fid;
        t[i] = r.t;
        uv[2 * i] = r.u;
        uv[2 * i + 1] = r.v;
    }
}

__global__ __launch_bounds__(256) void k_hot_kat(int op, uint32_t n, const float* __restrict__ in,
                                                 float* __restrict__ out) {
    const uint32_t i = blockIdx.x * 256 + threadIdx.x;
    if (i >= n) return;
    if (op == 0) {
        const float* c = in + 12 * (size_t)i;
        const V3 o = v3(c[0], c[1], c[2]), d = v3(c[3], c[4], c[5]);
        const V3 inv = v3(1.0f / d.x, 1.0f / d.y, 1.0f / d.z);
        float t0, t1;
        const bool h = box_hit(o, inv, c[6], c[7], c[8], c[9], c[10], c[11], t0, t1);
        slab_minmax(o, inv, c[6], c[7], c[8], c[9], c[10], c[11], t0, t1);
        out[2 * (size_t)i] = h ? 1.0f : 0.0f;
        out[2 * (size_t)i + 1] = (fmaxf(t0, -kRealMax) <= fminf(t1, kRealMax)) ? 1.0f : 0.0f;
    } else if (op == 1) {
        const float* c = in + 15 * (size_t)i;
        const V3 v0 = v3(c[6], c[7], c[8]);
        const V3 e1 = v3(c[9], c[10], c[11]) - v0, e2 = v3(c[12], c[13], c[14]) - v0;
        float t, u, v;
        const bool h = tri_core(v3(c[0], c[1], c[2]), v3(c[3], c[4], c[5]), v0, e1, e2, t, u, v);
        float* q = out + 4 * (size_t)i;
        q[0] = h ? 1.0f : 0.0f;
        q[1] = t;
        q[2] = u;
        q[3] = v;
    } else if (op == 2) {
        const float* c = in + 16 * (size_t)i;
        DevLight L;
        L.type = (int)c[0];
        for (int k = 0; k < 3; ++k) {
            L.color[k] = c[1 + k];
            L.pos[k] = c[5 + k];
            L.dir[k] = c[8 + k];
        }
        L.intensity = c[4];
        L.cos_outer = c[11];
        L.inv_cos_cone_diff = c[12];
        V3 dir, rad;
        light_sample(&L, 0, v3(c[13], c[14], c[15]), dir, rad);
        float* q = out + 6 * (size_t)i;
        q[0] = dir.x;
        q[1] = dir.y;
        q[2] = dir.z;
        q[3] = rad.x;
        q[4] = rad.y;
        q[5] = rad.z;
    } else if (op == 3) {
        const float* c = in + 3 * (size_t)i;
        for (int k = 0; k < 3; ++k) out[3 * (size_t)i + k] = (float)to_uchar(c[k]);
    }
}

hipError_t launch_hot_kat(int op, uint32_t n, const float* in, float* out, hipStream_t s) {
    if (n == 0) return hipSuccess;
    hipLaunchKernelGGL(k_hot_kat, dim3((n + 255) / 256), dim3(256), 0, s, op, n, in, out);
    return hipGetLastError();
}

template <int MAXD, bool ORDERED, bool LIGHTS, bool MTL_LDS, typename StackT, bool ENVIS = false, bool PAIR = false,
          bool DRAIN = false, bool QUAD = false, bool NOEMIT = false>
static void launch_one(const TraceArgs& a, dim3 grid, size_t lds, hipStream_t s) {
    hipLaunchKernelGGL((k_trace<MAXD, ORDERED, LIGHTS, MTL_LDS, StackT, ENVIS, PAIR, DRAIN, QUAD, NOEMIT>), grid,
                       dim3(256), lds, s, a);
}
template <bool MTL_LDS, typename StackT>
static void launch_quad(const TraceArgs& a, dim3 grid, size_t lds, hipStream_t s) {
    if (a.max_depth <= 8) launch_one<8, true, false, MTL_LDS, StackT, false, false, false, true>(a, grid, lds, s);
    else launch_one<64, true, false, MTL_LDS, StackT, false, false, false, true>(a, grid, lds, s);
}

template <bool LIGHTS, bool MTL_LDS, typename StackT, bool PAIR = false, bool ENVIS = false, bool DRAIN = false>
static void launch_ordered_d(const TraceArgs& a, dim3 grid, size_t lds, hipStream_t s) {
    if constexpr (PAIR) {
        if (!a.any_emitter) {
            if (a.max_depth <= 8)
                launch_one<8, true, LIGHTS, MTL_LDS, StackT, ENVIS, PAIR, DRAIN, false, true>(a, grid, lds, s);
            else
                launch_one<64, true, LIGHTS, MTL_LDS, StackT, ENVIS, PAIR, DRAIN, false, true>(a, grid, lds, s);
            return;
        }
    }
    if (a.max_depth <= 8) launch_one<8, true, LIGHTS, MTL_LDS, StackT, ENVIS, PAIR, DRAIN>(a, grid, lds, s);
    else launch_one<64, true, LIGHTS, MTL_LDS, StackT, ENVIS, PAIR, DRAIN>(a, grid, lds, s);
}
template <bool LIGHTS, bool MTL_LDS, typename StackT, bool PAIR = false, bool ENVIS = false>
static void launch_ordered(const TraceArgs& a, dim3 grid, size_t lds, hipStream_t s) {
    if constexpr (!PAIR && !ENVIS) {
        if (a.drained) {
            launch_ordered_d<LIGHTS, MTL_LDS, StackT, PAIR, ENVIS, true>(a, grid, lds, s);
            return;
        }
    }
    launch_ordered_d<LIGHTS, MTL_LDS, StackT, PAIR, ENVIS, false>(a, grid, lds, s);
}

constexpr size_t kLdsBudget = (163840 / TPT_TRACE_WAVES) & ~(size_t)255;
constexpr size_t kLdsBudgetIS = (163840 / TPT_TRACE_WAVES_IS) & ~(size_t)255;
constexpr size_t kLdsBudgetPair = (163840 / TPT_TRACE_WAVES_PAIR) & ~(size_t)255;
constexpr size_t kLdsBudgetQuad = (163840 / TPT_TRACE_WAVES_QUAD) & ~(size_t)255;
#ifndef TPT_MTL_LDS_MAX
#define TPT_MTL_LDS_MAX 2048
#endif
constexpr size_t kLdsMtlMax = TPT_MTL_LDS_MAX;

size_t trace_lds_bytes(TraceArgs& a, int words, size_t elem, bool mtl_lds, int rec_cols = 256,
                       size_t lds_budget = kLdsBudget, bool quad = false) {
    const size_t mtl_bytes = mtl_lds ? ((size_t)(a.n_materials + 1) * 2 * 16 + 127) / 128 * 128 : 0;
    a.mtl_in_lds = mtl_lds ? 1 : 0;
    a.lds_mtl_offset = 0;
    const size_t budget = lds_budget - mtl_bytes;
    const size_t slot = quad ? 64 * elem : 256 * elem;
    const size_t level = (size_t)words * (size_t)rec_cols * sizeof(float);
    size_t slots = (size_t)a.stack_depth + 3;
    const size_t want = std::min<size_t>((size_t)a.max_depth, (budget - 12 * slot) / level);
    if (slots * slot + want * level > budget)
        slots = std::min(slots, std::max<size_t>(12, ((budget - want * level) / slot) & ~(size_t)1));
    const size_t stack = quad ? ((slots + 3) / 4 * 4 * slot + 15) / 16 * 16
                              : ((slots + 1) / 2 * 2 * slot + 15) / 16 * 16;
    size_t levels = (budget - stack) / level;
    if (levels > (size_t)a.max_depth) levels = (size_t)a.max_depth;
    a.lds_nodes = 0;
    a.lds_nodes_offset = (int)mtl_bytes;
    a.stack_lds_slots = (int)slots;
    a.lds_stack_offset = (int)mtl_bytes;
    a.lds_rec_offset = (int)(mtl_bytes + stack);
    a.rec_lds_levels = (int)levels;
    return mtl_bytes + stack + levels * level;
}

int trace_waves_per_simd() { return TPT_TRACE_WAVES; }

bool trace_quad_fits(const TraceArgs& a_in) {
    TraceArgs a = a_in;
    const bool small = (2 * (size_t)a.n_faces - 1) <= 65535;
    const bool mtl_lds = (size_t)(a.n_materials + 1) * 2 * sizeof(float4) <= kLdsMtlMax;
    trace_lds_bytes(a, 2, small ? 2 : 4, mtl_lds, 256, kLdsBudgetQuad, true);
    return rec_words(a.n_lights, a.n_materials) == 2 && a.stack_lds_slots >= a.stack_depth + 3;
}

template <typename F>
static void for_mtl_stack(bool mtl_lds, bool small, F f) {
    if (mtl_lds) {
        if (small) f(std::true_type{}, uint16_t{});
        else f(std::true_type{}, int{});
    } else {
        if (small) f(std::false_type{}, uint16_t{});
        else f(std::false_type{}, int{});
    }
}

hipError_t launch_trace(const TraceArgs& a_in, hipStream_t s) {
    TraceArgs a = a_in;
    dim3 grid((a.width + 15) / 16, ((a.band_height + 15) / 16) * (a.n_frames > 0 ? a.n_frames : 1));
    if (a.xcd_run > 0 && (grid.x % 8 != 0 || (grid.x / 8) % (unsigned)a.xcd_run != 0)) a.xcd_run = 0;
    if (a.flags & TPT_FLAG_REF_ORDER) {
        const size_t lds = trace_lds_bytes(a, 5, sizeof(int), false);
        if (a.env_is) launch_one<64, false, true, false, int, true>(a, grid, lds, s);
        else launch_one<64, false, true, false, int>(a, grid, lds, s);
        return hipGetLastError();
    }
    const bool small = (2 * (size_t)a.n_faces - 1) <= 65535;
    const bool mtl_lds = (size_t)(a.n_materials + 1) * 2 * sizeof(float4) <= kLdsMtlMax;
    if (a.env_is) {
        const bool pair_is = a.pair && (a.n_materials + 1) < (int)kNoProbe;
        if (pair_is) grid.y = ((a.band_height + 7) / 8) * (a.n_frames > 0 ? a.n_frames : 1);
        const size_t lds = trace_lds_bytes(a, 5, small ? 2 : 4, mtl_lds, pair_is ? 128 : 256, kLdsBudgetIS);
        for_mtl_stack(mtl_lds, small, [&](auto m, auto st) {
            if (pair_is) launch_ordered<true, decltype(m)::value, decltype(st), true, true>(a, grid, lds, s);
            else launch_ordered<true, decltype(m)::value, decltype(st), false, true>(a, grid, lds, s);
        });
        return hipGetLastError();
    }
    const bool lights = rec_words(a.n_lights, a.n_materials) == 5;
    if (a.quad) {
        grid = dim3((a.width + 7) / 8, ((a.band_height + 7) / 8) * (a.n_frames > 0 ? a.n_frames : 1));
        a.xcd_run = 0;
        const size_t lds = trace_lds_bytes(a, 2, small ? 2 : 4, mtl_lds, 256, kLdsBudgetQuad, true);
        if (lights || a.stack_lds_slots < a.stack_depth + 3) return hipErrorInvalidValue;
        for_mtl_stack(mtl_lds, small, [&](auto m, auto st) {
            launch_quad<decltype(m)::value, decltype(st)>(a, grid, lds, s);
        });
        return hipGetLastError();
    }
    const bool pair = a.pair && lights && a.n_lights > 0 && (a.n_materials + 1) < (int)kNoProbe;
    if (pair) {
        grid.y = ((a.band_height + 7) / 8) * (a.n_frames > 0 ? a.n_frames : 1);
        const size_t lds = trace_lds_bytes(a, 5, small ? 2 : 4, mtl_lds, 128, kLdsBudgetPair);
        for_mtl_stack(mtl_lds, small, [&](auto m, auto st) {
            launch_ordered<true, decltype(m)::value, decltype(st), true>(a, grid, lds, s);
        });
        return hipGetLastError();
    }
    const size_t lds = trace_lds_bytes(a, lights ? 5 : 2, small ? 2 : 4, mtl_lds);
    for_mtl_stack(mtl_lds, small, [&](auto m, auto st) {
        if (lights) launch_ordered<true, decltype(m)::value, decltype(st)>(a, grid, lds, s);
        else launch_ordered<false, decltype(m)::value, decltype(st)>(a, grid, lds, s);
    });
    return hipGetLastError();
}

constexpr int kLatStackSlots = 64;
constexpr size_t kLatStackBytes = (size_t)kLatStackSlots * 256 * sizeof(int);
__global__ __launch_bounds__(64) void k_step_latency(TraceArgs a, uint32_t n, const float* __restrict__ o,
                                                     const float* __restrict__ d, int nodes_lds,
                                                     unsigned long long* __restrict__ out) {
    extern __shared__ __attribute__((aligned(16))) char lds[];
    TPT_LDS char* slds = (TPT_LDS char*)lds;
    const int lane = threadIdx.x;
    TPT_LDS LdsF4* snodes = (TPT_LDS LdsF4*)slds;
    for (int i = lane; i < 8 * nodes_lds; i += 64) {
        const float4 m = a.inner4[i];
        snodes[i].x = m.x;
        snodes[i].y = m.y;
        snodes[i].z = m.z;
        snodes[i].w = m.w;
    }
    __syncthreads();
    LaneStack<int> stk;
    stk.lds = (TPT_LDS int*)(slds + (size_t)nodes_lds * 128) + lane;
    stk.nlds = kLatStackSlots;
    const int nint = a.n_faces - 1;
    const bool active = (uint32_t)lane < n;
    Trav r;
    trav_begin(r, active ? v3(o[3 * lane], o[3 * lane + 1], o[3 * lane + 2]) : v3(0.0f, 0.0f, 0.0f),
               active ? v3(d[3 * lane], d[3 * lane + 1], d[3 * lane + 2]) : v3(1.0f, 1.0f, 1.0f), TM_CLOSEST,
               a.boxes_finite != 0, a.emit_root, a.cull_eps, false);
    if (!active) r.node = -1;
    unsigned long long steps = 0, iters = 0;
    __builtin_amdgcn_s_waitcnt(0);
    const unsigned long long t0 = __builtin_amdgcn_s_memtime();
    while (__ballot(r.node >= 0) != 0ull) {
        ++iters;
        if (r.node >= 0) {
            ++steps;
            if (r.node < nint) {
                int next;
                if (r.fin) {
                    if (r.node < nodes_lds) {
                        const TPT_LDS LdsF4* nd = snodes + 8 * r.node;
                        next = inner_visit4_q(r, lds_f4(nd), lds_f4(nd + 1), lds_f4(nd + 2), lds_f4(nd + 3),
                                              lds_f4(nd + 4), lds_f4(nd + 5), lds_f4(nd + 6), stk, r.sp);
                    } else {
                        next = inner_visit4(r, a.inner4, 0, stk, r.sp);
                    }
                } else {
                    int deferred;
                    bool push;
                    inner_visit<true>(r, a.inner, next, push, deferred);
                    stk.put(r.sp, deferred);
                    r.sp += push ? 1 : 0;
                }
                if (r.sp > a.stack_depth) {
                    r.sp = 0;
                    next = -1;
                }
                r.node = next >= 0 ? next : (r.sp == 0 ? -1 : stk.get(--r.sp));
            } else {
                const bool stop = leaf_test<true>(r, a.tri, r.node - nint, a.cull_eps);
                r.node = (stop || r.sp == 0) ? -1 : stk.get(--r.sp);
            }
        }
    }
    __builtin_amdgcn_s_waitcnt(0);
    const unsigned long long t1 = __builtin_amdgcn_s_memtime();
    uint32_t c_leaf = 0;
    if (a.n_sliver_groups > 0 && r.fin) sliver_pass(r, a, c_leaf);
    out[4 * lane] = steps;
    out[4 * lane + 1] = iters;
    out[4 * lane + 2] = t1 - t0;
    out[4 * lane + 3] = (unsigned long long)(long long)r.fid;
}

__global__ __launch_bounds__(64) void k_step_latency_quad(TraceArgs a, uint32_t n, const float* __restrict__ o,
                                                          const float* __restrict__ d,
                                                          unsigned long long* __restrict__ out) {
    extern __shared__ __attribute__((aligned(16))) char lds[];
    const int lane = threadIdx.x, q = lane >> 2, k = lane & 3;
    LaneStack<int, true> stk;
    stk.lds = (TPT_LDS int*)lds + 4 * q;
    stk.nlds = kLatStackSlots;
    const int nint = a.n_faces - 1;
    const bool active = (uint32_t)q < n;
    Trav r;
    trav_begin(r, active ? v3(o[3 * q], o[3 * q + 1], o[3 * q + 2]) : v3(0.0f, 0.0f, 0.0f),
               active ? v3(d[3 * q], d[3 * q + 1], d[3 * q + 2]) : v3(1.0f, 1.0f, 1.0f), TM_CLOSEST,
               a.boxes_finite != 0, a.emit_root, a.cull_eps, false);
    if (!active || !r.fin) r.node = -1;
    unsigned long long steps = 0, iters = 0;
    uint32_t c_leaf = 0;
    __builtin_amdgcn_s_waitcnt(0);
    const unsigned long long t0 = __builtin_amdgcn_s_memtime();
    while (__ballot(r.node >= 0) != 0ull) {
        ++iters;
        if (r.node >= 0) {
            ++steps;
            if (r.node >= nint) {
                leaf_test<true>(r, a.tri, r.node - nint, a.cull_eps);
                r.node = -1;
            } else {
                bool stop;
                int next = inner_visit4_quad(r, a.inner4, a.tri, nint, a.cull_eps, stk, r.sp, stop, c_leaf);
                if (stop || r.sp > a.stack_depth) {
                    r.sp = 0;
                    next = -1;
                }
                r.node = next >= 0 ? next : (r.sp == 0 ? -1 : stk.get(--r.sp));
            }
        }
    }
    __builtin_amdgcn_s_waitcnt(0);
    const unsigned long long t1 = __builtin_amdgcn_s_memtime();
    if (a.n_sliver_groups > 0 && r.fin) sliver_pass(r, a, c_leaf);
    if (k == 0) {
        out[4 * q] = steps;
        out[4 * q + 1] = iters;
        out[4 * q + 2] = t1 - t0;
        out[4 * q + 3] = (unsigned long long)(long long)r.fid;
    }
}

hipError_t launch_step_latency_ptr(const void* a, uint32_t n, const float* o, const float* d, int nodes_lds,
                                   unsigned long long* out, hipStream_t s) {
    if (nodes_lds < 0) {
        hipLaunchKernelGGL(k_step_latency_quad, dim3(1), dim3(64), kLatStackBytes, s,
                           *static_cast<const TraceArgs*>(a), n, o, d, out);
        return hipGetLastError();
    }
    const size_t lds = (size_t)nodes_lds * 128 + kLatStackBytes;
    hipLaunchKernelGGL(k_step_latency, dim3(1), dim3(64), lds, s, *static_cast<const TraceArgs*>(a), n, o, d,
                       nodes_lds, out);
    return hipGetLastError();
}

hipError_t launch_trace_ptr(const void* a, hipStream_t s) { return launch_trace(*static_cast<const TraceArgs*>(a), s); }

hipError_t launch_resolve(const ResolveArgs& a, hipStream_t s) {
    dim3 grid((a.width + 255) / 256, a.band_height);
    hipLaunchKernelGGL(k_resolve, grid, dim3(256), 0, s, a);
    return hipGetLastError();
}

hipError_t launch_trace_rays(const TraceArgs& a, uint32_t n, const float* o, const float* d, const int32_t* ofid,
                             int mode, int32_t* hit, float* t, float* uv, hipStream_t s) {
    if (n == 0) return hipSuccess;
    const size_t lds = (size_t)kRaysLdsSlots * 256 * sizeof(int);
    hipLaunchKernelGGL(k_trace_rays, dim3((n + 255) / 256), dim3(256), lds, s, a, n, o, d, ofid, mode, hit, t, uv);
    return hipGetLastError();
}

}
```

### tinypathtracer_amd/csrc/kernels/trace_dev.hpp

```cpp
#pragma once
#include <hip/hip_runtime.h>

#include <algorithm>

#include "../common/device_api.hpp"
#include "../common/ptrig.hpp"
#include "../common/rng.hpp"
#include "../common/tri_rec.hpp"
#include "../common/tpt_math.hpp"
#include "tpt.h"

#ifndef TPT_FAST
#define TPT_FAST 0
#endif
#ifndef TPT_FAST_SINCOS
#define TPT_FAST_SINCOS 1
#endif
#ifndef TPT_FAST_RCP
#define TPT_FAST_RCP 1
#endif
#ifndef TPT_LEAF_KP
#define TPT_LEAF_KP 24
#endif
#ifndef TPT_TRACE_WAVES
#define TPT_TRACE_WAVES 5
#endif

#ifndef TPT_TRACE_WAVES_IS
#define TPT_TRACE_WAVES_IS 4
#endif
#ifndef TPT_TRACE_WAVES_PAIR
#define TPT_TRACE_WAVES_PAIR 4
#endif
#ifndef TPT_TRACE_WAVES_DRAIN
#define TPT_TRACE_WAVES_DRAIN 4
#endif
#ifndef TPT_TRACE_WAVES_QUAD
#define TPT_TRACE_WAVES_QUAD 4
#endif

namespace tpt {

#define TPT_LDS __attribute__((address_space(3)))
struct alignas(16) LdsF4 {
    float x, y, z, w;
};
__device__ __forceinline__ float4 lds_f4(const TPT_LDS LdsF4* p) { return make_float4(p->x, p->y, p->z, p->w); }

__device__ __forceinline__ bool box_hit(const V3& o, const V3& inv, float nx, float ny, float nz, float xx,
                                        float xy, float xz, float& t0, float& t1) {
    bool miss;
    float a, b, lo, hi;
    t0 = -kRealMax;
    t1 = kRealMax;
    a = (nx - o.x) * inv.x;
    b = (xx - o.x) * inv.x;
    lo = a > b ? b : a;
    hi = a > b ? a : b;
    miss = (t0 > hi) | (lo > t1);
    t0 = fmx(t0, lo);
    t1 = fmn(t1, hi);
    a = (ny - o.y) * inv.y;
    b = (xy - o.y) * inv.y;
    lo = a > b ? b : a;
    hi = a > b ? a : b;
    miss = miss | (t0 > hi) | (lo > t1);
    t0 = fmx(t0, lo);
    t1 = fmn(t1, hi);
    a = (nz - o.z) * inv.z;
    b = (xz - o.z) * inv.z;
    lo = a > b ? b : a;
    hi = a > b ? a : b;
    miss = miss | (t0 > hi) | (lo > t1);
    t0 = fmx(t0, lo);
    t1 = fmn(t1, hi);
    return !miss;
}

enum : int { TM_CLOSEST = 0, TM_ANY = 1, TM_EMIT = 2, TM_OCCL = 3, TM_OCCLUDED = 4 };
constexpr int kLinkMask = 0x3fffffff;

struct Trav {
    V3 o, d, inv;
    int node, sp, hpos, fid;
    int pend;
    float t, u, v;
    float lim;
    int mode;
    bool fin;
};

__device__ __forceinline__ void trav_begin(Trav& r, V3 o, V3 d, int mode, bool boxes_finite = false,
                                           int emit_root = -1, float cull_eps = 0.0f, bool graze = false) {
    r.o = o;
    r.d = d;
    if (TPT_FAST && TPT_FAST_RCP)
        r.inv = v3(__builtin_amdgcn_rcpf(d.x), __builtin_amdgcn_rcpf(d.y), __builtin_amdgcn_rcpf(d.z));
    else
        r.inv = v3(1.0f / d.x, 1.0f / d.y, 1.0f / d.z);
    r.node = 0;
    r.sp = 0;
    r.pend = -1;
    r.hpos = -1;
    r.fid = -1;
    r.t = kRealMax;
    r.u = 0.0f;
    r.v = 0.0f;
    r.mode = mode;
    r.fin = boxes_finite & !graze & __builtin_isfinite(o.x) & __builtin_isfinite(o.y) & __builtin_isfinite(o.z) &
            __builtin_isfinite(r.inv.x) & __builtin_isfinite(r.inv.y) & __builtin_isfinite(r.inv.z);
    r.lim = kRealMax;
    (void)cull_eps;
    if (mode == TM_EMIT && r.fin) {
        if (emit_root >= 0) r.node = emit_root;
        else r.mode = TM_CLOSEST;
    }
}

constexpr float kGraze = 1e-3f;
struct Surf {
    float x, y;
};
__device__ __forceinline__ Surf no_surface() { return Surf{__builtin_nanf(""), 0.0f}; }
__device__ __forceinline__ bool grazing(Surf g, V3 d) {
    if (!(g.x == g.x)) return false;
    const float zz = fmaxf(0.0f, 1.0f - g.x * g.x - g.y * g.y);
    const float z = (__float_as_uint(g.x) & 1u) ? -__builtin_amdgcn_sqrtf(zz) : __builtin_amdgcn_sqrtf(zz);
    const float dn = d.x * g.x + d.y * g.y + d.z * z;
    const float dd = d.x * d.x + d.y * d.y + d.z * d.z;
    return dn * dn < (kGraze * kGraze) * dd;
}

template <bool ORDERED>
__device__ __forceinline__ void inner_visit(const Trav& r, const float4* __restrict__ inner, int& next, bool& push,
                                            int& deferred) {
    const float4* nd = inner + 4 * r.node;
    const float4 q0 = nd[0], q1 = nd[1], q2 = nd[2], q3 = nd[3];
    float l0, l1, r0, r1;
    bool hl = box_hit(r.o, r.inv, q0.x, q0.y, q0.z, q0.w, q1.x, q1.y, l0, l1);
    bool hr = box_hit(r.o, r.inv, q1.z, q1.w, q2.x, q2.y, q2.z, q2.w, r0, r1);
    const int lraw = __float_as_int(q3.x), rraw = __float_as_int(q3.y);
    const int lc = lraw & kLinkMask, rc = rraw & kLinkMask;
    if (ORDERED && r.mode == TM_EMIT) {
        hl = hl & ((lraw >> 30) != 0);
        hr = hr & ((rraw >> 30) != 0);
    }
    const bool lfirst = ORDERED && (l0 < r0);
    push = hl & hr;
    deferred = lfirst ? rc : lc;
    next = push ? (lfirst ? lc : rc) : (hl ? lc : (hr ? rc : -1));
}

__device__ __forceinline__ void slab_minmax(const V3& o, const V3& inv, float nx, float ny, float nz, float xx,
                                            float xy, float xz, float& t0, float& t1) {
#if TPT_FAST
    const float ox = -(o.x * inv.x), oy = -(o.y * inv.y), oz = -(o.z * inv.z);
    const float ax = __builtin_fmaf(nx, inv.x, ox), bx = __builtin_fmaf(xx, inv.x, ox);
    const float ay = __builtin_fmaf(ny, inv.y, oy), by = __builtin_fmaf(xy, inv.y, oy);
    const float az = __builtin_fmaf(nz, inv.z, oz), bz = __builtin_fmaf(xz, inv.z, oz);
#else
    const float ax = (nx - o.x) * inv.x, bx = (xx - o.x) * inv.x;
    const float ay = (ny - o.y) * inv.y, by = (xy - o.y) * inv.y;
    const float az = (nz - o.z) * inv.z, bz = (xz - o.z) * inv.z;
#endif
    t0 = fmaxf(fmaxf(fminf(ax, bx), fminf(ay, by)), fminf(az, bz));
    t1 = fminf(fminf(fmaxf(ax, bx), fmaxf(ay, by)), fmaxf(az, bz));
}


constexpr int kMaxStackSlots = 160 + 3;

template <typename StackT, bool QS = false>
struct LaneStack {
    TPT_LDS StackT* lds;
    int nlds;
    StackT deep[kMaxStackSlots];
    __device__ static __forceinline__ int off(int i) {
        if constexpr (QS) return (i >> 2) * 256 + (i & 3);
        else return i * 256;
    }
    __device__ __forceinline__ void put(int i, int v) {
        if (i < nlds) lds[off(i)] = (StackT)v;
        else deep[i - nlds] = (StackT)v;
    }
    __device__ __forceinline__ int get(int i) const {
        return i < nlds ? (int)lds[off(i)] : (int)deep[i - nlds];
    }
};

template <typename StackT, bool QS>
__device__ __forceinline__ int inner_visit4_q(const Trav& r, float4 q0, float4 q1, float4 q2, float4 q3, float4 q4,
                                              float4 q5, float4 q6, LaneStack<StackT, QS>& stk, int& sp) {
    float k0, k1, k2, k3, e0, e1, e2, e3;
    slab_minmax(r.o, r.inv, q0.x, q0.y, q0.z, q0.w, q1.x, q1.y, k0, e0);
    slab_minmax(r.o, r.inv, q1.z, q1.w, q2.x, q2.y, q2.z, q2.w, k1, e1);
    slab_minmax(r.o, r.inv, q3.x, q3.y, q3.z, q3.w, q4.x, q4.y, k2, e2);
    slab_minmax(r.o, r.inv, q4.z, q4.w, q5.x, q5.y, q5.z, q5.w, k3, e3);
    const float hi = r.lim;
    int i0 = __float_as_int(q6.x), i1 = __float_as_int(q6.y), i2 = __float_as_int(q6.z), i3 = __float_as_int(q6.w);
    const float hd = 0.5f * kDelta;
    const bool h0 = (i0 >= 0) & (fmaxf(k0, hd) <= fminf(e0, hi));
    const bool h1 = (i1 >= 0) & (fmaxf(k1, hd) <= fminf(e1, hi));
    const bool h2 = (i2 >= 0) & (fmaxf(k2, hd) <= fminf(e2, hi));
    const bool h3 = (i3 >= 0) & (fmaxf(k3, hd) <= fminf(e3, hi));
    const int m = (int)h0 + (int)h1 + (int)h2 + (int)h3;
    i0 &= kLinkMask;
    i1 &= kLinkMask;
    i2 &= kLinkMask;
    i3 &= kLinkMask;
    const float inf = __builtin_inff();
    k0 = h0 ? k0 : inf;
    k1 = h1 ? k1 : inf;
    k2 = h2 ? k2 : inf;
    k3 = h3 ? k3 : inf;
    i0 = h0 ? i0 : -1;
    i1 = h1 ? i1 : -1;
    i2 = h2 ? i2 : -1;
    i3 = h3 ? i3 : -1;
#define TPT_CX(ka, ia, kb, ib)          \
    {                                   \
        const bool sw = kb < ka;        \
        const float tk = sw ? kb : ka;  \
        kb = sw ? ka : kb;              \
        ka = tk;                        \
        const int ti = sw ? ib : ia;    \
        ib = sw ? ia : ib;              \
        ia = ti;                        \
    }
    TPT_CX(k0, i0, k1, i1)
    TPT_CX(k2, i2, k3, i3)
    TPT_CX(k0, i0, k2, i2)
    TPT_CX(k1, i1, k3, i3)
    TPT_CX(k1, i1, k2, i2)
#undef TPT_CX
    const int np = m > 0 ? m - 1 : 0;
    const int v0 = np == 3 ? i3 : (np == 2 ? i2 : i1), v1 = np == 3 ? i2 : i1;
    if (sp + 3 <= stk.nlds) {
        stk.lds[stk.off(sp)] = (StackT)v0;
        stk.lds[stk.off(sp + 1)] = (StackT)v1;
        stk.lds[stk.off(sp + 2)] = (StackT)i1;
    } else {
        stk.put(sp, v0);
        stk.put(sp + 1, v1);
        stk.put(sp + 2, i1);
    }
    sp += np;
    return i0;
}
template <typename StackT, bool QS>
__device__ __forceinline__ int inner_visit4(const Trav& r, const float4* __restrict__ inner4, int nlds_nodes,
                                            LaneStack<StackT, QS>& stk, int& sp) {
    const float4* nd = inner4 + 8 * r.node;
    return inner_visit4_q(r, nd[0], nd[1], nd[2], nd[3], nd[4], nd[5], nd[6], stk, sp);
}

__device__ __forceinline__ bool tri_core(const V3& o, const V3& d, const V3& v0, const V3& e1, const V3& e2, float& t,
                                         float& u, float& v) {
    const V3 tv = o - v0;
    const V3 p = cross(d, e2);
    const V3 q = cross(tv, e1);
    const float denom = dot(p, e1);
    const float id = (TPT_FAST && TPT_FAST_RCP) ? __builtin_amdgcn_rcpf(denom) : 1.0f / denom;
    u = dot(p, tv) * id;
    v = dot(q, d) * id;
    t = dot(q, e2) * id;
    return (denom != 0.0f) & !((u < 0.0f) | (v < 0.0f) | (u + v > 1.0f));
}

__device__ __forceinline__ float cull_slack(const V3& inv, float cull_eps) {
    return cull_eps * fmaxf(fmaxf(fabsf(inv.x), fabsf(inv.y)), fabsf(inv.z));
}
template <bool ORDERED>
__device__ __forceinline__ bool leaf_test_q(Trav& r, const float4 q0, const float4 q1, const float4 q2, int pos,
                                            float cull_eps) {
    const V3 v0 = v3(q0.x, q0.y, q0.z), e1 = v3(q1.x, q1.y, q1.z), e2 = v3(q2.x, q2.y, q2.z);
    float t, u, v;
    const bool inside = tri_core(r.o, r.d, v0, e1, e2, t, u, v);
    const bool better = ORDERED ? ((t < r.t) | ((t == r.t) & (r.hpos >= 0) & (pos > r.hpos))) : (t < r.t);
    const bool take = inside & better & (t > kDelta);
    r.t = take ? t : r.t;
    if (ORDERED) r.lim = take ? fminf(kRealMax, t * 1.0001f + cull_slack(r.inv, cull_eps)) : r.lim;
    r.fid = take ? __float_as_int(q0.w) : r.fid;
    r.u = take ? u : r.u;
    r.v = take ? v : r.v;
    r.hpos = take ? pos : r.hpos;
    const bool occl = r.mode == TM_OCCL;
    r.mode = (take & occl) ? TM_OCCLUDED : r.mode;
    return take & ((r.mode == TM_ANY) | occl);
}
template <bool ORDERED>
__device__ __forceinline__ bool leaf_test(Trav& r, const float4* __restrict__ tri, int pos, float cull_eps) {
    const TriQ tq = tri_load(tri, pos);
    return leaf_test_q<ORDERED>(r, tq.q0, tq.q1, tq.q2, pos, cull_eps);
}

template <int CTRL>
__device__ __forceinline__ int quad_mov(int v) {
    return __builtin_amdgcn_update_dpp(0, v, CTRL, 0xf, 0xf, false);
}
template <int CTRL>
__device__ __forceinline__ float quad_mov(float v) {
    return __int_as_float(__builtin_amdgcn_update_dpp(0, __float_as_int(v), CTRL, 0xf, 0xf, false));
}
constexpr int kQuadXor1 = 0xb1, kQuadXor2 = 0x4e;
template <int CTRL>
__device__ __forceinline__ void quad_best(Trav& r) {
    const float t2 = quad_mov<CTRL>(r.t), u2 = quad_mov<CTRL>(r.u), v2 = quad_mov<CTRL>(r.v), l2 = quad_mov<CTRL>(r.lim);
    const int p2 = quad_mov<CTRL>(r.hpos), f2 = quad_mov<CTRL>(r.fid), m2 = quad_mov<CTRL>(r.mode);
    const bool take = (t2 < r.t) | ((t2 == r.t) & (r.hpos >= 0) & (p2 > r.hpos));
    r.t = take ? t2 : r.t;
    r.u = take ? u2 : r.u;
    r.v = take ? v2 : r.v;
    r.lim = take ? l2 : r.lim;
    r.hpos = take ? p2 : r.hpos;
    r.fid = take ? f2 : r.fid;
    r.mode = take ? m2 : r.mode;
}
template <typename StackT, bool QS>
__device__ __forceinline__ int inner_visit4_quad(Trav& r, const float4* __restrict__ inner4,
                                                 const float4* __restrict__ tri, int nint, float cull_eps,
                                                 LaneStack<StackT, QS>& stk, int& sp, bool& stop, uint32_t& c_leaf) {
    const int lane = (int)__lane_id(), k = lane & 3;
    const float* nf = (const float*)(inner4 + 8 * (size_t)r.node);
    const float2 b0 = *(const float2*)(nf + 6 * k), b1 = *(const float2*)(nf + 6 * k + 2),
                 b2 = *(const float2*)(nf + 6 * k + 4);
    const int link = ((const int*)nf)[24 + k];
    float kk, ee;
    slab_minmax(r.o, r.inv, b0.x, b0.y, b1.x, b1.y, b2.x, b2.y, kk, ee);
    const float hd = 0.5f * kDelta;
    const int id = link & kLinkMask;
    const bool h = (link >= 0) & (fmaxf(kk, hd) <= fminf(ee, r.lim));
    const bool lf = h & (id >= nint);
    stop = false;
    TriQ tq = TriQ{make_float4(0.0f, 0.0f, 0.0f, 0.0f), make_float4(0.0f, 0.0f, 0.0f, 0.0f),
                   make_float4(0.0f, 0.0f, 0.0f, 0.0f)};
    if (lf) tq = tri_load(tri, id - nint);
    const bool in = h & (id < nint);
    const float key = in ? kk : __builtin_inff();
    const float c0 = quad_mov<0x00>(key), c1 = quad_mov<0x55>(key), c2 = quad_mov<0xaa>(key), c3 = quad_mov<0xff>(key);
    const int rank = ((c0 < key) | ((c0 == key) & (0 < k))) + ((c1 < key) | ((c1 == key) & (1 < k))) +
                     ((c2 < key) | ((c2 == key) & (2 < k))) + ((c3 < key) | ((c3 == key) & (3 < k)));
    const int n_in = __popcll((__ballot(in) >> (lane & ~3)) & 0xfull);
    if (in & (rank > 0)) stk.put(sp + n_in - 1 - rank, id);
    int near = (in & (rank == 0)) ? id : -1;
    near = max(near, quad_mov<kQuadXor1>(near));
    near = max(near, quad_mov<kQuadXor2>(near));
    sp += n_in > 0 ? n_in - 1 : 0;
    if (__ballot(lf) != 0ull) {
        int s = 0;
        if (lf) {
            ++c_leaf;
            s = leaf_test_q<true>(r, tq.q0, tq.q1, tq.q2, id - nint, cull_eps) ? 1 : 0;
        }
        quad_best<kQuadXor1>(r);
        quad_best<kQuadXor2>(r);
        s |= quad_mov<kQuadXor1>(s);
        s |= quad_mov<kQuadXor2>(s);
        stop = s != 0;
    }
    return near;
}

__device__ __forceinline__ bool probe_misses_emitters(const TraceArgs& a, V3 o, V3 d) {
    if (a.n_emit_box <= 0) return false;
    const V3 inv = v3(__builtin_amdgcn_rcpf(d.x), __builtin_amdgcn_rcpf(d.y), __builtin_amdgcn_rcpf(d.z));
    bool miss = __builtin_isfinite(inv.x) & __builtin_isfinite(inv.y) & __builtin_isfinite(inv.z) &
                __builtin_isfinite(o.x) & __builtin_isfinite(o.y) & __builtin_isfinite(o.z);
    for (int k = 0; k < a.n_emit_box; ++k) {
        const float4 lo = a.emit_box[2 * k], hi = a.emit_box[2 * k + 1];
        float t0, t1;
        slab_minmax(o, inv, lo.x, lo.y, lo.z, hi.x, hi.y, hi.z, t0, t1);
        miss = miss & ((t0 - t1) > 0x1p-16f * (fabs_(t0) + fabs_(t1)));
    }
    return miss;
}

struct SliverHit {
    float t, u, v;
    int fid, hpos, mode, tests;
};
__device__ __forceinline__ SliverHit sliver_scan(const float4* __restrict__ groups, const float4* __restrict__ list,
                                              int n_groups, const float4* __restrict__ tri, V3 o, V3 d, V3 inv,
                                              float cull_eps, SliverHit h) {
    Trav r;
    r.o = o;
    r.d = d;
    r.inv = inv;
    r.t = h.t;
    r.u = h.u;
    r.v = h.v;
    r.fid = h.fid;
    r.hpos = h.hpos;
    r.mode = h.mode;
    r.lim = fminf(kRealMax, h.t * 1.0001f + cull_slack(inv, cull_eps));
    int tests = 0;
    float t0, t1;
    const float hd = 0.5f * kDelta, lim = r.lim;
    {
        const float4 lo = groups[0], hi = groups[1];
        if (!box_hit(o, inv, lo.x, lo.y, lo.z, hi.x, hi.y, hi.z, t0, t1) || (t0 >= hd && t1 <= lim)) n_groups = 0;
    }
    for (int g = 1; g < n_groups; ++g) {
        const float4 lo = groups[2 * g], hi = groups[2 * g + 1];
        if (!box_hit(o, inv, lo.x, lo.y, lo.z, hi.x, hi.y, hi.z, t0, t1)) continue;
        const int first = __float_as_int(lo.w), count = __float_as_int(hi.w);
        bool stop = false;
        for (int i = first; i < first + count && !stop; ++i) {
            const float4 bl = list[2 * i], bh = list[2 * i + 1];
            const int e = __float_as_int(bl.w);
            if (r.mode == TM_EMIT && !((e >> 30) & 1)) continue;
            const int pos = e & kLinkMask;
            if (!box_hit(o, inv, bl.x, bl.y, bl.z, bh.x, bh.y, bh.z, t0, t1)) continue;
            if (t1 >= hd && t0 <= lim) continue;
            ++tests;
            stop = leaf_test<true>(r, tri, pos, cull_eps);
        }
        if (stop) break;
    }
    return SliverHit{r.t, r.u, r.v, r.fid, r.hpos, r.mode, tests};
}
__device__ __forceinline__ void sliver_pass(Trav& r, const TraceArgs& a, uint32_t& c_leaf) {
    if (!r.fin || r.mode == TM_OCCLUDED || (r.mode == TM_ANY && r.fid >= 0)) return;
    const SliverHit h = sliver_scan(a.sliver_groups, a.sliver_list, a.n_sliver_groups, a.tri, r.o, r.d, r.inv, a.cull_eps,
                                    SliverHit{r.t, r.u, r.v, r.fid, r.hpos, r.mode, 0});
    r.t = h.t;
    r.u = h.u;
    r.v = h.v;
    r.fid = h.fid;
    r.hpos = h.hpos;
    r.mode = h.mode;
    r.lim = fminf(kRealMax, r.t * 1.0001f + cull_slack(r.inv, a.cull_eps));
    c_leaf += (uint32_t)h.tests;
}

__device__ __forceinline__ V3 reflect_dir(V3 d, V3 n) { return d - (2.0f * dot(d, n)) * n; }

struct Hemi {
    V3 n, xb;
    float q, r;
};
__device__ __forceinline__ Hemi hemi_basis(V3 d, V3 n) {
    const float sign = dot(d, n) > 0.0f ? -1.0f : 1.0f;
    n = sign * n;
    const float q = n.z == 0.0f ? 0.0f : -n.x / n.z;
    V3 xb = n.z == 0.0f ? v3(0.0f, 0.0f, 1.0f) : v3(1.0f, 0.0f, q);
    const float r = 1.0f / fsqrt(norm2(xb));
    xb = r * xb;
    return Hemi{n, xb, q, r};
}

__device__ __forceinline__ float new_direction(V3 d, V3 n, float eta_m, float metallic, uint32_t st[6], V3& next,
                                               float& atten) {
    if (eta_m > 0.0f) {
        float cos_i = dot(d, n);
        const float eta = cos_i > 0.0f ? eta_m : 1.0f / eta_m;
        const V3 nn = cos_i > 0.0f ? -n : n;
        cos_i = fabs_(cos_i);
        const float sin2i = 1.0f - cos_i * cos_i;
        const float sin2t = eta * eta * sin2i;
        const bool tir = sin2t >= 1.0f;
        V3 rf = v3(0.0f, 0.0f, 0.0f);
        float fr = 1.0f;
        if (!tir) {
            const float cos_t = fsqrt(1.0f - sin2t);
            rf = (eta * d) + ((cos_i * eta - cos_t) * nn);
            float f0 = (1.0f - eta) / (1.0f + eta);
            f0 *= f0;
            const float m = fclamp(1.0f - cos_i, 1.0f, 0.0f);
            const float m2 = m * m;
            fr = f0 + (1.0f - f0) * m2 * m2 * m;
        }
        const V3 rl = reflect_dir(d, n);
        next = xorwow_uniform(st) < fr ? rl : rf;
        atten = 1.0f;
        return 1.0f;
    } else if (metallic > 0.0f) {
        atten = 1.0f;
        next = reflect_dir(d, n);
        return 1.0f;
    }
    const Hemi hb = hemi_basis(d, n);
    n = hb.n;
    const V3 xb = hb.xb;
    const V3 zb = cross(xb, n);
    float sp, cp;
#if TPT_FAST && TPT_FAST_SINCOS
    const float u_phi = xorwow_uniform(st);
    const float cos_t = __builtin_amdgcn_sqrtf(xorwow_uniform(st));
    const float sin_t = __builtin_amdgcn_sqrtf(1.0f - cos_t * cos_t);
    sp = __builtin_amdgcn_sinf(u_phi);
    cp = __builtin_amdgcn_cosf(u_phi);
#else
    const float phi = 2.0f * kPi * xorwow_uniform(st);
    const float cos_t = fsqrt(xorwow_uniform(st));
    const float sin_t = fsqrt(1.0f - cos_t * cos_t);
    fsincos_2pi(phi, sp, cp);
#endif
    const float x = cp * sin_t;
    const float z = sp * sin_t;
    next = ((x * xb) + (cos_t * n)) + (z * zb);
    const float c = dot(next, n);
    atten = fabs_(c) / kPi;
    return (c / kPi) * (c > 0.0f ? 1.0f : 0.0f);
}

__device__ __forceinline__ void light_sample(const DevLight* __restrict__ Ls, int li, V3 p, V3& dir, V3& rad) {
    const DevLight& L = Ls[li];
    float dist = 0.0f;
    const V3 color = v3(L.color[0], L.color[1], L.color[2]);
    dir = v3(0.0f, 0.0f, 0.0f);
    rad = v3(0.0f, 0.0f, 0.0f);
    if (L.type == 0 || L.type == 2) {
        const V3 dd = v3(L.pos[0], L.pos[1], L.pos[2]) - p;
        dist = fsqrt(norm2(dd));
        dir = vdiv(dd, dist);
        rad = L.intensity * color;
        if (L.type == 2) {
            const float cos_t = dot(-dir, v3(L.dir[0], L.dir[1], L.dir[2]));
            const float fall = fsq(fsat(cos_t - L.cos_outer) * L.inv_cos_cone_diff);
            rad = fall * rad;
        }
    } else if (L.type == 1) {
        dir = -v3(L.dir[0], L.dir[1], L.dir[2]);
        rad = L.intensity * color;
    }
    const float d2 = dist * dist;
    float att = 1.0f / (d2 + 1.0f);
    att *= fsq(fsat(1.0f - fsq(d2 * 0.01f)));
    rad = att * rad;
}

__device__ __forceinline__ int env_col_exact(float z, float x, int w) {
    float u = patan2_fast(z, x) / (2.0f * kPi);
    if (u < 0.0f) u += 1.0f;
    const int ix = (int)floorf(u * (float)w);
    return ix < 0 ? 0 : (ix > w - 1 ? w - 1 : ix);
}
__device__ __forceinline__ int env_row_exact(float y, int h) {
    const float v = 1.0f - pacos_fast(fclamp(y, 1.0f, -1.0f)) / kPi;
    const int iy = (int)floorf(v * (float)h);
    return iy < 0 ? 0 : (iy > h - 1 ? h - 1 : iy);
}
static __device__ __noinline__ int env_col_exact_call(float z, float x, int w) { return env_col_exact(z, x, w); }
static __device__ __noinline__ int env_row_exact_call(float y, int h) { return env_row_exact(y, h); }
template <bool COLD>
__device__ __forceinline__ V3 env_lookup_inl(const uint32_t* __restrict__ env, int w, int h, V3 d) {
    int ix = env_col_fast(d.z, d.x, w);
    int iy = env_row_fast(d.y, h);
    if (ix < 0) ix = COLD ? env_col_exact_call(d.z, d.x, w) : env_col_exact(d.z, d.x, w);
    if (iy < 0) iy = COLD ? env_row_exact_call(d.y, h) : env_row_exact(d.y, h);
    const uint32_t t = env[(size_t)iy * (size_t)w + (size_t)ix];
    return (1.0f / 255.0f) * v3((float)(t & 0xffu), (float)((t >> 8) & 0xffu), (float)((t >> 16) & 0xffu));
}
static __device__ __noinline__ V3 env_lookup_call(const uint32_t* __restrict__ env, int w, int h, V3 d) {
    return env_lookup_inl<false>(env, w, h, d);
}
template <bool INLINE>
__device__ __forceinline__ V3 env_lookup(const uint32_t* __restrict__ env, int w, int h, V3 d) {
    if constexpr (INLINE) return env_lookup_inl<true>(env, w, h, d);
    else return env_lookup_call(env, w, h, d);
}

__device__ __forceinline__ int band_of(int lb, int band_count, int band_index, const int32_t* band_list) {
    return band_list ? band_list[lb] : lb * band_count + band_index;
}
__device__ __forceinline__ int band_row(int ly, int band_rows, int band_count, int band_index,
                                        const int32_t* band_list) {
    return band_of(ly / band_rows, band_count, band_index, band_list) * band_rows + (ly % band_rows);
}

__device__ __forceinline__ unsigned long long wave_sum(uint32_t v) {
    unsigned long long s = v;
#pragma unroll
    for (int off = 32; off > 0; off >>= 1) s += __shfl_xor(s, off, 64);
    return s;
}

enum : int { PH_CAMERA = 0, PH_EXT = 1, PH_SHADOW = 2, PH_PROBE = 3, PH_ENVSHADOW = 4 };

__device__ __forceinline__ int lower_bound_guided(const float* __restrict__ a, int n, float t, float x,
                                                  const int32_t* __restrict__ g, int K) {
    int k = (int)(x * (float)K);
    k = k < 0 ? 0 : (k > K ? K : k);
    int lo = g[k];
    int hi = k < K ? g[k + 1] : n - 1;
    hi = hi > n - 1 ? n - 1 : hi;
    while (hi - lo > 8) {
        const int mid = (lo + hi) >> 1;
        if (a[mid] >= t) hi = mid;
        else lo = mid + 1;
    }
    int cnt = 0;
#pragma unroll
    for (int j = 0; j < 8; ++j) {
        const int i = lo + j;
        const float v = i < hi ? a[i] : t;
        cnt += v < t ? 1 : 0;
    }
    return lo + cnt;
}

__device__ __forceinline__ bool env_is_sample(const TraceArgs& a, V3 nf, float x1, float x2, V3& dir, V3& k_le) {
    const int W = a.env_w, H = a.env_h, B = a.is_b, BW = a.is_bw, BH = a.is_bh;
    const float t1 = x1 * a.is_total;
    const int by = lower_bound_guided(a.is_marg, BH, t1, x1, a.is_guide_r, a.is_kr);
    const float lo1 = by > 0 ? a.is_marg[by - 1] : 0.0f;
    const float hi1 = a.is_marg[by];
    const float f1 = fminf((t1 - lo1) / (hi1 - lo1), 0.99999994f);
    const float* cond = a.is_cond + (size_t)by * (size_t)BW;
    const float rs = a.is_row[by];
    const float t2 = x2 * rs;
    const int bx = lower_bound_guided(cond, BW, t2, x2, a.is_guide_c + (size_t)by * (size_t)(a.is_kc + 1), a.is_kc);
    const float lo2 = bx > 0 ? cond[bx - 1] : 0.0f;
    const float hi2 = cond[bx];
    const float f2 = fminf((t2 - lo2) / (hi2 - lo2), 0.99999994f);
    const int x0 = bx * B, y0 = by * B;
    const int wb = min(B, W - x0), hb = min(B, H - y0);
    const float u = ((float)x0 + f2 * (float)wb) / (float)W;
    const float v = ((float)y0 + f1 * (float)hb) / (float)H;
    float sp, cp, sth, cth;
    fsincos_2pi((2.0f * kPi) * u, sp, cp);
    fsincos_2pi(kPi * (1.0f - v), sth, cth);
    dir = v3(sth * cp, cth, sth * sp);
    const float c = dot(dir, nf);
    const float pb = ((hi2 - lo2) / rs) * ((hi1 - lo1) / a.is_total);
    const float pdf = (pb * (((float)W * (float)H) / (float)(wb * hb))) / ((2.0f * kPi * kPi) * sth);
    if (!(sth > 0.0f) || !(c > 0.0f) || !(pdf > 0.0f) || !(pdf < kRealMax)) return false;
    const int ix = x0 + min((int)(f2 * (float)wb), wb - 1);
    const int iy = y0 + min((int)(f1 * (float)hb), hb - 1);
    const uint32_t tx = a.env[(size_t)iy * (size_t)W + (size_t)ix];
    const V3 le = (1.0f / 255.0f) * v3((float)(tx & 0xffu), (float)((tx >> 8) & 0xffu), (float)((tx >> 16) & 0xffu));
    const float k = c / (kPi * pdf);
    k_le = k * le;
    return true;
}
enum : int { TS_DONE = 0, TS_TRAV = 1, TS_DEAD = 2, TS_IDLE = 3 };
enum : int { PH_WAIT = 5 };

constexpr uint32_t kNoProbe = 0x7fffu;

__device__ __forceinline__ uint32_t p_kind(float prob) {
    const uint32_t pb = __float_as_uint(prob);
    return pb == 0x80000000u ? 1u : (pb == 0u ? 2u : 0u);
}

template <int MAXD, int RS = 256>
struct PathRecords {
    TPT_LDS float* lds;
    int nlds, words;
    float deep[MAXD * 5];

    __device__ __forceinline__ void put(int level, int w, float v) {
        if (level < nlds) lds[(level * words + w) * RS] = v;
        else deep[level * 5 + w] = v;
    }
    __device__ __forceinline__ float get(int level, int w) const {
        return level < nlds ? lds[(level * words + w) * RS] : deep[level * 5 + w];
    }
    template <int WORDS>
    __device__ __forceinline__ float lds_at(int level, int w) const {
        return lds[(level * WORDS + w) * RS];
    }
    template <bool PACKED_PROBE = false>
    __device__ __forceinline__ void put_dst(int level, uint32_t mk, uint32_t probe, V3 dst) {
        if (words == 2 || PACKED_PROBE) {
            put(level, 1, __uint_as_float(mk | (probe << 15)));
        } else {
            put(level, 1, __uint_as_float(mk));
            put(level, 2, dst.x);
            put(level, 3, dst.y);
            put(level, 4, dst.z);
        }
    }
};

__device__ __forceinline__ uint8_t to_uchar(float c) { return (uint8_t)fclamp(c * 255.0f, 255.0f, 0.0f); }

template <bool ORDERED>
__device__ __forceinline__ void trav_lane(Trav& r, const TraceArgs& a, LaneStack<int>& stk, uint32_t& c_ovf) {
    const int nint = a.n_faces - 1;
    while (r.node >= 0) {
        if (r.node < nint) {
            int next;
            if (ORDERED && r.fin) {
                next = inner_visit4(r, a.inner4, 0, stk, r.sp);
            } else {
                int deferred;
                bool push;
                inner_visit<ORDERED>(r, a.inner, next, push, deferred);
                stk.put(r.sp, deferred);
                r.sp += push ? 1 : 0;
            }
            if (r.sp > a.stack_depth) {
                ++c_ovf;
                r.sp = 0;
                next = -1;
            }
            r.node = next >= 0 ? next : (r.sp == 0 ? -1 : stk.get(--r.sp));
        } else {
            const bool stop = leaf_test<ORDERED>(r, a.tri, r.node - nint, a.cull_eps);
            r.node = (stop || r.sp == 0) ? -1 : stk.get(--r.sp);
        }
    }
}

}
```

Before: 15700.

## Launch trace kernel with one-wave workgroups and per-wave LDS budget

Makes the number of waves per k_trace workgroup a compile-time parameter. The default becomes one wave for the plain ordered and drain variants and four for the others. Each 8x8 tile is split across NB workgroups, and LDS sizing is recomputed per workgroup with a small slack. One-wave groups swap __syncthreads for a wave-level fence and barrier. The aim is to free schedulers from workgroup-granular residency and barrier stalls so waves retire and refill independently. The cost is reloading materials and nodes into LDS once per wave, plus more complex block index mapping.

```diff
diff --git a/include/tpt.h b/include/tpt.h
--- a/include/tpt.h
+++ b/include/tpt.h
@@ -102,7 +102,7 @@
     double resolve_ms;
     double total_ms;
     int32_t trace_launches;
-    int32_t pad;
+    int32_t wg_waves;
     uint64_t wide_visits;
     uint64_t accumulated_spp;
     double trace_kernel_ms;
@@ -230,6 +230,7 @@
 tpt_status tpt_debug_trace_rays(tpt_scene* scene, uint32_t n, const float* origins, const float* dirs,
                                 const int32_t* origin_fid, int32_t mode, int32_t* hit, float* t, float* uv);
 tpt_status tpt_debug_hot_kat(int device, int32_t op, uint32_t n, const float* in, float* out);
+int32_t tpt_debug_trace_wg_waves(int32_t family);
 tpt_status tpt_debug_step_latency(tpt_scene* scene, uint32_t n, const float* origins, const float* dirs,
                                   int32_t mode, int32_t flags, uint64_t* out);
 int32_t tpt_wide_tree_build(int32_t n, const float* leaf_box, const uint32_t* leaf_emit, float* nodes,
diff --git a/tinypathtracer_amd/_lib.py b/tinypathtracer_amd/_lib.py
--- a/tinypathtracer_amd/_lib.py
+++ b/tinypathtracer_amd/_lib.py
@@ -83,13 +83,13 @@
     _fields_ = [("traversals", C.c_uint64), ("internal_visits", C.c_uint64), ("leaf_tests", C.c_uint64),
                 ("shade_hits", C.c_uint64), ("pixels", C.c_uint64), ("samples", C.c_uint64),
                 ("rng_init_ms", C.c_double), ("trace_ms", C.c_double), ("resolve_ms", C.c_double),
-                ("total_ms", C.c_double), ("trace_launches", C.c_int32), ("pad", C.c_int32),
+                ("total_ms", C.c_double), ("trace_launches", C.c_int32), ("wg_waves", C.c_int32),
                 ("wide_visits", C.c_uint64), ("accumulated_spp", C.c_uint64), ("trace_kernel_ms", C.c_double),
                 ("local_rays", C.c_uint64), ("tree_wait_ms", C.c_double), ("resident_lanes", C.c_uint64),
                 ("lanes_per_pixel", C.c_int32), ("drained", C.c_int32)]
 
     def as_dict(self):
-        return {k: getattr(self, k) for k, _ in self._fields_ if k != "pad"}
+        return {k: getattr(self, k) for k, _ in self._fields_}
 
 
 class Aov(C.Structure):
@@ -165,6 +165,7 @@
     ("tpt_debug_trace_rays", C.c_int, [C.c_void_p, C.c_uint32, C.c_void_p, C.c_void_p, C.c_void_p, C.c_int32,
                                        C.c_void_p, C.c_void_p, C.c_void_p]),
     ("tpt_debug_hot_kat", C.c_int, [C.c_int, C.c_int32, C.c_uint32, C.c_void_p, C.c_void_p]),
+    ("tpt_debug_trace_wg_waves", C.c_int32, [C.c_int32]),
     ("tpt_debug_step_latency", C.c_int, [C.c_void_p, C.c_uint32, C.c_void_p, C.c_void_p, C.c_int32, C.c_int32,
                                          C.c_void_p]),
     ("tpt_wide_tree_build", C.c_int32, [C.c_int32, C.c_void_p, C.c_void_p, C.c_void_p, C.c_int32,
diff --git a/tinypathtracer_amd/csrc/common/device_api.hpp b/tinypathtracer_amd/csrc/common/device_api.hpp
--- a/tinypathtracer_amd/csrc/common/device_api.hpp
+++ b/tinypathtracer_amd/csrc/common/device_api.hpp
@@ -177,10 +177,12 @@
 };
 hipError_t launch_wavefront(WfArgs w, uint32_t* h_count, hipEvent_t ev[2], int32_t* iterations, hipStream_t s);
 
-hipError_t launch_trace(const TraceArgs& a, hipStream_t s);
+constexpr int kTraceShapeWords = 6;
+hipError_t launch_trace(const TraceArgs& a, hipStream_t s, int32_t* shape = nullptr);
 bool trace_quad_fits(const TraceArgs& a);
+int trace_family_wgw(int family);
 int trace_waves_per_simd();
-hipError_t launch_trace_ptr(const void* a, hipStream_t s);
+hipError_t launch_trace_ptr(const void* a, hipStream_t s, int32_t* shape);
 hipError_t launch_step_latency_ptr(const void* a, uint32_t n, const float* o, const float* d, int nodes_lds,
                                    unsigned long long* out, hipStream_t s);
 hipError_t launch_resolve(const ResolveArgs& a, hipStream_t s);
@@ -305,7 +307,7 @@
 }
 
 namespace tpt_fast {
-hipError_t launch_trace_ptr(const void* a, hipStream_t s);
+hipError_t launch_trace_ptr(const void* a, hipStream_t s, int32_t* shape);
 hipError_t launch_step_latency_ptr(const void* a, uint32_t n, const float* o, const float* d, int nodes_lds,
                                    unsigned long long* out, hipStream_t s);
 }
diff --git a/tinypathtracer_amd/csrc/host/api.cpp b/tinypathtracer_amd/csrc/host/api.cpp
--- a/tinypathtracer_amd/csrc/host/api.cpp
+++ b/tinypathtracer_amd/csrc/host/api.cpp
@@ -152,6 +152,8 @@
     HIP_OR_FAIL(hipMemcpy(out, dout.p, 4 * 64 * sizeof(unsigned long long), hipMemcpyDeviceToHost));
     return TPT_OK;
 }
+
+int32_t tpt_debug_trace_wg_waves(int32_t family) { return tpt::trace_family_wgw(family); }
 
 tpt_status tpt_debug_hot_kat(int device, int32_t op, uint32_t n, const float* in, float* out) {
     static const int kIn[4] = {12, 15, 16, 3}, kOut[4] = {2, 4, 6, 3};
diff --git a/tinypathtracer_amd/csrc/host/api_render.cpp b/tinypathtracer_amd/csrc/host/api_render.cpp
--- a/tinypathtracer_amd/csrc/host/api_render.cpp
+++ b/tinypathtracer_amd/csrc/host/api_render.cpp
@@ -118,7 +118,8 @@
 };
 
 tpt_status render_planned(tpt_scene* s, const tpt::TraceArgs& a, const tpt_params* p, const tpt::LaunchPlan& plan,
-                          size_t list_len, WaveDump& dump, double& trace_ms, double& kernel_ms, int& launches) {
+                          size_t list_len, WaveDump& dump, double& trace_ms, double& kernel_ms, int& launches,
+                          int32_t* shape) {
     hipStream_t st = s->stream;
     const int nset = plan.nset;
     const size_t nf = (size_t)a.n_frames;
@@ -179,7 +180,8 @@
         if (dump.path) ak.debug_waves = s->debug.p + oi * dbg_launch;
 #endif
         SET_OR_FAIL(hipEventRecord(s->lev[2 * j], qs[k]));
-        SET_OR_FAIL((p->flags & TPT_FLAG_FAST) ? tpt_fast::launch_trace_ptr(&ak, qs[k]) : tpt::launch_trace(ak, qs[k]));
+        SET_OR_FAIL((p->flags & TPT_FLAG_FAST) ? tpt_fast::launch_trace_ptr(&ak, qs[k], shape)
+                                               : tpt::launch_trace(ak, qs[k], shape));
         SET_OR_FAIL(hipEventRecord(s->lev[2 * j + 1], qs[k]));
     }
     for (int k = 0; nset > 1 && k < nset; ++k) {
@@ -355,12 +357,18 @@
     double trace_ms = 0.0, kernel_ms = 0.0;
     int launches = 0;
     WaveDump dump;
+    int32_t shape[tpt::kTraceShapeWords] = {};
     if ((p->flags & TPT_FLAG_WAVEFRONT) && (p->flags & (TPT_FLAG_FAST | TPT_FLAG_APPROX_CULL)))
         return fail(TPT_ERR_INVALID_ARG, "TPT_FLAG_WAVEFRONT runs the exact traversal only");
     const tpt_status ts = (p->flags & TPT_FLAG_WAVEFRONT)
                               ? render_wavefront(s, a, p, n_frames, bh, trace_ms, kernel_ms, launches)
-                              : render_planned(s, a, p, plan, list.size(), dump, trace_ms, kernel_ms, launches);
+                              : render_planned(s, a, p, plan, list.size(), dump, trace_ms, kernel_ms, launches, shape);
     if (ts != TPT_OK) return ts;
+    if (std::getenv("TPT_DEBUG_SHAPE"))
+        std::fprintf(stderr,
+                     "tpt trace shape: wg_waves %d resident_blocks %d need_blocks %d lds_bytes %d stack_slots %d "
+                     "rec_levels %d\n",
+                     shape[0], shape[1], shape[2], shape[3], shape[4], shape[5]);
 
     HIP_OR_FAIL(hipEventRecord(s->ev[2], st));
     Staging sg(st);
@@ -436,6 +444,7 @@
         (void)hipEventElapsedTime(&ms, s->ev[2], s->ev[3]);
         stats->resolve_ms = ms;
         stats->trace_launches = launches;
+        stats->wg_waves = shape[0];
         stats->resident_lanes = s->resident_lanes;
         stats->lanes_per_pixel = plan.quad ? 4 : (plan.pair_kernel ? 2 : 1);
         stats->drained = a.drained;
diff --git a/tinypathtracer_amd/csrc/kernels/trace.hip b/tinypathtracer_amd/csrc/kernels/trace.hip
--- a/tinypathtracer_amd/csrc/kernels/trace.hip
+++ b/tinypathtracer_amd/csrc/kernels/trace.hip
@@ -1,3 +1,6 @@
+#include <array>
+#include <map>
+#include <mutex>
 #include <type_traits>
 
 #include "trace_dev.hpp"
@@ -51,21 +54,28 @@
 
 template <int MAXD, bool ORDERED, bool LIGHTS, bool MTL_LDS, typename StackT, bool ENVIS = false, bool PAIR = false,
           bool DRAIN = false, bool QUAD = false, bool NOEMIT = false>
-__global__ __launch_bounds__(256, ENVIS ? TPT_TRACE_WAVES_IS
-                                        : (PAIR ? TPT_TRACE_WAVES_PAIR
-                                                : (QUAD ? TPT_TRACE_WAVES_QUAD
-                                                        : (DRAIN ? TPT_TRACE_WAVES_DRAIN : TPT_TRACE_WAVES))))
+__global__ __launch_bounds__((64 * trace_wgw<ORDERED, ENVIS, PAIR, DRAIN, QUAD>()),
+                             ENVIS ? TPT_TRACE_WAVES_IS
+                                   : (PAIR ? TPT_TRACE_WAVES_PAIR
+                                           : (QUAD ? TPT_TRACE_WAVES_QUAD
+                                                   : (DRAIN ? TPT_TRACE_WAVES_DRAIN : TPT_TRACE_WAVES))))
 void k_trace(TraceArgs a) {
     static_assert(!PAIR || (ORDERED && LIGHTS), "pair mode: ordered variants with 5-word records");
     static_assert(!QUAD || (ORDERED && !LIGHTS && !PAIR && !ENVIS && !DRAIN), "four lanes per pixel: one-lane logic");
+    constexpr int WGW = trace_wgw<ORDERED, ENVIS, PAIR, DRAIN, QUAD>(), NB = 4 / WGW, ROW = 64 * WGW;
     extern __shared__ __attribute__((aligned(16))) char lds[];
-    const int tid = threadIdx.x, lane = tid & 63, wave = tid >> 6;
+    const int tid = threadIdx.x, lane = tid & 63;
     const int nfr = a.n_frames > 0 ? a.n_frames : 1;
-    int bx = (int)blockIdx.x, by = (int)blockIdx.y;
+    int bx = (int)blockIdx.x / NB, part = (int)blockIdx.x % NB;
+    const int by = (int)blockIdx.y;
+    [[maybe_unused]] int tile_id = bx;
     if (a.xcd_run > 0) {
-        const int g = a.xcd_run, k = ((bx & 7) + by + a.xcd_rot) & 7, m = bx >> 3;
+        const int b = (int)blockIdx.x, g = a.xcd_run, k = ((b & 7) + by + a.xcd_rot) & 7, m = (b >> 3) / NB;
+        part = (b >> 3) % NB;
+        tile_id = m * 8 + (b & 7);
         bx = ((m / g) * 8 + k) * g + m % g;
     }
+    const int wave = part * WGW + (tid >> 6);
     const int frame = by % nfr;
     const bool side = PAIR && (lane & 1);
     const bool lead = !QUAD || (lane & 3) == 0;
@@ -88,7 +98,7 @@
     TPT_LDS char* slds = (TPT_LDS char*)lds;
     TPT_LDS LdsF4* smtl = (TPT_LDS LdsF4*)(slds + a.lds_mtl_offset);
     if constexpr (MTL_LDS) {
-        for (int i = tid; i < 2 * (a.n_materials + 1); i += 256) {
+        for (int i = tid; i < 2 * (a.n_materials + 1); i += ROW) {
             const float4 m = a.mtl[i];
             smtl[i].x = m.x;
             smtl[i].y = m.y;
@@ -97,14 +107,21 @@
         }
     }
     TPT_LDS LdsF4* snodes = (TPT_LDS LdsF4*)(slds + a.lds_nodes_offset);
-    for (int i = tid; i < 8 * a.lds_nodes; i += 256) {
+    for (int i = tid; i < 8 * a.lds_nodes; i += ROW) {
         const float4 m = a.inner4[i];
         snodes[i].x = m.x;
         snodes[i].y = m.y;
         snodes[i].z = m.z;
         snodes[i].w = m.w;
     }
-    if (MTL_LDS || a.lds_nodes > 0) __syncthreads();
+    if (MTL_LDS || a.lds_nodes > 0) {
+        if constexpr (WGW == 1) {
+            __builtin_amdgcn_fence(__ATOMIC_ACQ_REL, "wavefront");
+            __builtin_amdgcn_wave_barrier();
+        } else {
+            __syncthreads();
+        }
+    }
     auto MT = [&](int i) -> float4 {
         if constexpr (MTL_LDS) {
             return make_float4(smtl[i].x, smtl[i].y, smtl[i].z, smtl[i].w);
@@ -112,11 +129,11 @@
             return a.mtl[i];
         }
     };
-    LaneStack<StackT, QUAD> stk;
+    LaneStack<StackT, QUAD, ROW> stk;
     stk.lds = (TPT_LDS StackT*)(slds + a.lds_stack_offset) + (QUAD ? (tid & ~3) : tid);
     stk.nlds = a.stack_lds_slots;
-    PathRecords<MAXD, PAIR ? 128 : 256> rec;
-    rec.lds = (TPT_LDS float*)(slds + a.lds_rec_offset) + (PAIR ? wave * 32 + pl : tid);
+    PathRecords<MAXD, PAIR ? ROW / 2 : ROW> rec;
+    rec.lds = (TPT_LDS float*)(slds + a.lds_rec_offset) + (PAIR ? (tid >> 6) * 32 + pl : tid);
     rec.nlds = a.rec_lds_levels;
     rec.words = LIGHTS ? 5 : 2;
 
@@ -723,7 +740,7 @@
         atomicAdd(&a.counters[15], 1ull);
         if (a.debug_waves) {
             const unsigned long long wid =
-                ((unsigned long long)blockIdx.y * gridDim.x + blockIdx.x) * 4 + wave;
+                ((unsigned long long)blockIdx.y * (gridDim.x / NB) + tile_id) * 4 + wave;
             unsigned long long* o = a.debug_waves + 8 * wid;
             o[0] = t_wave0;
             o[1] = life;
@@ -874,68 +891,40 @@
     return hipGetLastError();
 }
 
-template <int MAXD, bool ORDERED, bool LIGHTS, bool MTL_LDS, typename StackT, bool ENVIS = false, bool PAIR = false,
-          bool DRAIN = false, bool QUAD = false, bool NOEMIT = false>
-static void launch_one(const TraceArgs& a, dim3 grid, size_t lds, hipStream_t s) {
-    hipLaunchKernelGGL((k_trace<MAXD, ORDERED, LIGHTS, MTL_LDS, StackT, ENVIS, PAIR, DRAIN, QUAD, NOEMIT>), grid,
-                       dim3(256), lds, s, a);
-}
-template <bool MTL_LDS, typename StackT>
-static void launch_quad(const TraceArgs& a, dim3 grid, size_t lds, hipStream_t s) {
-    if (a.max_depth <= 8) launch_one<8, true, false, MTL_LDS, StackT, false, false, false, true>(a, grid, lds, s);
-    else launch_one<64, true, false, MTL_LDS, StackT, false, false, false, true>(a, grid, lds, s);
-}
-
-template <bool LIGHTS, bool MTL_LDS, typename StackT, bool PAIR = false, bool ENVIS = false, bool DRAIN = false>
-static void launch_ordered_d(const TraceArgs& a, dim3 grid, size_t lds, hipStream_t s) {
-    if constexpr (PAIR) {
-        if (!a.any_emitter) {
-            if (a.max_depth <= 8)
-                launch_one<8, true, LIGHTS, MTL_LDS, StackT, ENVIS, PAIR, DRAIN, false, true>(a, grid, lds, s);
-            else
-                launch_one<64, true, LIGHTS, MTL_LDS, StackT, ENVIS, PAIR, DRAIN, false, true>(a, grid, lds, s);
-            return;
-        }
-    }
-    if (a.max_depth <= 8) launch_one<8, true, LIGHTS, MTL_LDS, StackT, ENVIS, PAIR, DRAIN>(a, grid, lds, s);
-    else launch_one<64, true, LIGHTS, MTL_LDS, StackT, ENVIS, PAIR, DRAIN>(a, grid, lds, s);
-}
-template <bool LIGHTS, bool MTL_LDS, typename StackT, bool PAIR = false, bool ENVIS = false>
-static void launch_ordered(const TraceArgs& a, dim3 grid, size_t lds, hipStream_t s) {
-    if constexpr (!PAIR && !ENVIS) {
-        if (a.drained) {
-            launch_ordered_d<LIGHTS, MTL_LDS, StackT, PAIR, ENVIS, true>(a, grid, lds, s);
-            return;
-        }
-    }
-    launch_ordered_d<LIGHTS, MTL_LDS, StackT, PAIR, ENVIS, false>(a, grid, lds, s);
-}
-
-constexpr size_t kLdsBudget = (163840 / TPT_TRACE_WAVES) & ~(size_t)255;
-constexpr size_t kLdsBudgetIS = (163840 / TPT_TRACE_WAVES_IS) & ~(size_t)255;
-constexpr size_t kLdsBudgetPair = (163840 / TPT_TRACE_WAVES_PAIR) & ~(size_t)255;
-constexpr size_t kLdsBudgetQuad = (163840 / TPT_TRACE_WAVES_QUAD) & ~(size_t)255;
 #ifndef TPT_MTL_LDS_MAX
 #define TPT_MTL_LDS_MAX 2048
 #endif
 constexpr size_t kLdsMtlMax = TPT_MTL_LDS_MAX;
-
-size_t trace_lds_bytes(TraceArgs& a, int words, size_t elem, bool mtl_lds, int rec_cols = 256,
-                       size_t lds_budget = kLdsBudget, bool quad = false) {
-    const size_t mtl_bytes = mtl_lds ? ((size_t)(a.n_materials + 1) * 2 * 16 + 127) / 128 * 128 : 0;
-    a.mtl_in_lds = mtl_lds ? 1 : 0;
+constexpr size_t kLdsSlack = 512;
+
+struct LdsSpec {
+    int words;
+    size_t elem;
+    bool mtl_lds;
+    bool pair;
+    bool quad;
+    int waves;
+};
+
+size_t trace_lds_bytes(TraceArgs& a, const LdsSpec& sp, int wgw, size_t max_slots = (size_t)-1,
+                       size_t max_levels = (size_t)-1) {
+    size_t lds_budget = ((163840 / (size_t)sp.waves) & ~(size_t)255) * (size_t)wgw / 4;
+    if (wgw < 4) lds_budget -= kLdsSlack * (size_t)wgw;
+    const size_t row = 64 * (size_t)wgw;
+    const size_t mtl_bytes = sp.mtl_lds ? ((size_t)(a.n_materials + 1) * 2 * 16 + 127) / 128 * 128 : 0;
+    a.mtl_in_lds = sp.mtl_lds ? 1 : 0;
     a.lds_mtl_offset = 0;
     const size_t budget = lds_budget - mtl_bytes;
-    const size_t slot = quad ? 64 * elem : 256 * elem;
-    const size_t level = (size_t)words * (size_t)rec_cols * sizeof(float);
-    size_t slots = (size_t)a.stack_depth + 3;
-    const size_t want = std::min<size_t>((size_t)a.max_depth, (budget - 12 * slot) / level);
+    const size_t slot = sp.quad ? row / 4 * sp.elem : row * sp.elem;
+    const size_t level = (size_t)sp.words * (sp.pair ? row / 2 : row) * sizeof(float);
+    size_t slots = std::min((size_t)a.stack_depth + 3, max_slots);
+    const size_t want = std::min(std::min<size_t>((size_t)a.max_depth, (budget - 12 * slot) / level), max_levels);
     if (slots * slot + want * level > budget)
         slots = std::min(slots, std::max<size_t>(12, ((budget - want * level) / slot) & ~(size_t)1));
-    const size_t stack = quad ? ((slots + 3) / 4 * 4 * slot + 15) / 16 * 16
-                              : ((slots + 1) / 2 * 2 * slot + 15) / 16 * 16;
+    const size_t stack = sp.quad ? ((slots + 3) / 4 * 4 * slot + 15) / 16 * 16
+                                 : ((slots + 1) / 2 * 2 * slot + 15) / 16 * 16;
     size_t levels = (budget - stack) / level;
-    if (levels > (size_t)a.max_depth) levels = (size_t)a.max_depth;
+    levels = std::min(std::min(levels, (size_t)a.max_depth), max_levels);
     a.lds_nodes = 0;
     a.lds_nodes_offset = (int)mtl_bytes;
     a.stack_lds_slots = (int)slots;
@@ -945,14 +934,118 @@
     return mtl_bytes + stack + levels * level;
 }
 
+struct LaunchCtx {
+    dim3 tiles;
+    LdsSpec lds;
+    hipStream_t s;
+    bool dry;
+    int32_t* shape;
+    hipError_t err;
+};
+
+struct LdsFit {
+    size_t max_slots, max_levels;
+    int resident, need;
+};
+
+template <typename K>
+static LdsFit fit_lds(K kern, const TraceArgs& a_in, const LdsSpec& sp, int wgw, int waves) {
+    LdsFit f{(size_t)-1, (size_t)-1, 0, 4 * waves / wgw};
+    int regs = 0;
+    if (hipOccupancyMaxActiveBlocksPerMultiprocessor(&regs, kern, 64 * wgw, 0) != hipSuccess) {
+        (void)hipGetLastError();
+        return f;
+    }
+    const int target = std::min(f.need, regs);
+    for (;;) {
+        TraceArgs a = a_in;
+        const size_t lds = trace_lds_bytes(a, sp, wgw, f.max_slots, f.max_levels);
+        if (hipOccupancyMaxActiveBlocksPerMultiprocessor(&f.resident, kern, 64 * wgw, lds) != hipSuccess) {
+            (void)hipGetLastError();
+            return f;
+        }
+        if (f.resident >= target) return f;
+        if (a.stack_lds_slots > 12) f.max_slots = std::max<size_t>(12, (size_t)(a.stack_lds_slots - 1) & ~(size_t)1);
+        else if (a.rec_lds_levels > 0) f.max_levels = (size_t)a.rec_lds_levels - 1;
+        else return f;
+    }
+}
+
+template <int MAXD, bool ORDERED, bool LIGHTS, bool MTL_LDS, typename StackT, bool ENVIS = false, bool PAIR = false,
+          bool DRAIN = false, bool QUAD = false, bool NOEMIT = false>
+static void launch_one(const TraceArgs& a_in, LaunchCtx& c) {
+    constexpr int WGW = trace_wgw<ORDERED, ENVIS, PAIR, DRAIN, QUAD>();
+    constexpr int kWaves = ENVIS ? TPT_TRACE_WAVES_IS
+                                 : (PAIR ? TPT_TRACE_WAVES_PAIR
+                                         : (QUAD ? TPT_TRACE_WAVES_QUAD
+                                                 : (DRAIN ? TPT_TRACE_WAVES_DRAIN : TPT_TRACE_WAVES)));
+    const auto kern = k_trace<MAXD, ORDERED, LIGHTS, MTL_LDS, StackT, ENVIS, PAIR, DRAIN, QUAD, NOEMIT>;
+    static std::mutex mu;
+    static std::map<std::array<int, 3>, LdsFit> fits;
+    const std::array<int, 3> key{a_in.stack_depth, a_in.max_depth, a_in.n_materials};
+    LdsFit f;
+    {
+        std::lock_guard<std::mutex> lock(mu);
+        auto it = fits.find(key);
+        if (it == fits.end()) it = fits.emplace(key, fit_lds(kern, a_in, c.lds, WGW, kWaves)).first;
+        f = it->second;
+    }
+    TraceArgs a = a_in;
+    const size_t lds = trace_lds_bytes(a, c.lds, WGW, f.max_slots, f.max_levels);
+    if (c.shape) {
+        c.shape[0] = WGW;
+        c.shape[1] = f.resident;
+        c.shape[2] = f.need;
+        c.shape[3] = (int32_t)lds;
+        c.shape[4] = a.stack_lds_slots;
+        c.shape[5] = a.rec_lds_levels;
+    }
+    if (QUAD && a.stack_lds_slots < a.stack_depth + 3) {
+        c.err = hipErrorInvalidValue;
+        return;
+    }
+    if (c.dry) return;
+    hipLaunchKernelGGL(kern, dim3(c.tiles.x * (4 / WGW), c.tiles.y), dim3(64 * WGW), lds, c.s, a);
+    c.err = hipGetLastError();
+}
+template <bool MTL_LDS, typename StackT>
+static void launch_quad(const TraceArgs& a, LaunchCtx& c) {
+    if (a.max_depth <= 8) launch_one<8, true, false, MTL_LDS, StackT, false, false, false, true>(a, c);
+    else launch_one<64, true, false, MTL_LDS, StackT, false, false, false, true>(a, c);
+}
+
+template <bool LIGHTS, bool MTL_LDS, typename StackT, bool PAIR = false, bool ENVIS = false, bool DRAIN = false>
+static void launch_ordered_d(const TraceArgs& a, LaunchCtx& c) {
+    if constexpr (PAIR) {
+        if (!a.any_emitter) {
+            if (a.max_depth <= 8)
+                launch_one<8, true, LIGHTS, MTL_LDS, StackT, ENVIS, PAIR, DRAIN, false, true>(a, c);
+            else
+                launch_one<64, true, LIGHTS, MTL_LDS, StackT, ENVIS, PAIR, DRAIN, false, true>(a, c);
+            return;
+        }
+    }
+    if (a.max_depth <= 8) launch_one<8, true, LIGHTS, MTL_LDS, StackT, ENVIS, PAIR, DRAIN>(a, c);
+    else launch_one<64, true, LIGHTS, MTL_LDS, StackT, ENVIS, PAIR, DRAIN>(a, c);
+}
+template <bool LIGHTS, bool MTL_LDS, typename StackT, bool PAIR = false, bool ENVIS = false>
+static void launch_ordered(const TraceArgs& a, LaunchCtx& c) {
+    if constexpr (!PAIR && !ENVIS) {
+        if (a.drained) {
+            launch_ordered_d<LIGHTS, MTL_LDS, StackT, PAIR, ENVIS, true>(a, c);
+            return;
+        }
+    }
+    launch_ordered_d<LIGHTS, MTL_LDS, StackT, PAIR, ENVIS, false>(a, c);
+}
+
 int trace_waves_per_simd() { return TPT_TRACE_WAVES; }
 
-bool trace_quad_fits(const TraceArgs& a_in) {
-    TraceArgs a = a_in;
-    const bool small = (2 * (size_t)a.n_faces - 1) <= 65535;
-    const bool mtl_lds = (size_t)(a.n_materials + 1) * 2 * sizeof(float4) <= kLdsMtlMax;
-    trace_lds_bytes(a, 2, small ? 2 : 4, mtl_lds, 256, kLdsBudgetQuad, true);
-    return rec_words(a.n_lights, a.n_materials) == 2 && a.stack_lds_slots >= a.stack_depth + 3;
+int trace_family_wgw(int family) {
+    static const int kWgw[6] = {trace_wgw<true, false, false, false, false>(), trace_wgw<true, false, false, true, false>(),
+                                trace_wgw<true, false, true, false, false>(),  trace_wgw<true, true, false, false, false>(),
+                                trace_wgw<true, false, false, false, true>(),  trace_wgw<false, false, false, false, false>()};
+    return family >= 0 && family < 6 ? kWgw[family] : 0;
 }
 
 template <typename F>
@@ -966,54 +1059,69 @@
     }
 }
 
-hipError_t launch_trace(const TraceArgs& a_in, hipStream_t s) {
+static hipError_t launch_trace_impl(const TraceArgs& a_in, hipStream_t s, bool dry, int32_t* shape) {
     TraceArgs a = a_in;
-    dim3 grid((a.width + 15) / 16, ((a.band_height + 15) / 16) * (a.n_frames > 0 ? a.n_frames : 1));
-    if (a.xcd_run > 0 && (grid.x % 8 != 0 || (grid.x / 8) % (unsigned)a.xcd_run != 0)) a.xcd_run = 0;
+    const unsigned nfr = (unsigned)(a.n_frames > 0 ? a.n_frames : 1);
+    LaunchCtx c{dim3((a.width + 15) / 16, ((a.band_height + 15) / 16) * nfr), LdsSpec{}, s, dry, shape, hipSuccess};
+    if (a.xcd_run > 0 && (c.tiles.x % 8 != 0 || (c.tiles.x / 8) % (unsigned)a.xcd_run != 0)) a.xcd_run = 0;
     if (a.flags & TPT_FLAG_REF_ORDER) {
-        const size_t lds = trace_lds_bytes(a, 5, sizeof(int), false);
-        if (a.env_is) launch_one<64, false, true, false, int, true>(a, grid, lds, s);
-        else launch_one<64, false, true, false, int>(a, grid, lds, s);
-        return hipGetLastError();
+        c.lds = LdsSpec{5, sizeof(int), false, false, false, TPT_TRACE_WAVES};
+        if (a.env_is) launch_one<64, false, true, false, int, true>(a, c);
+        else launch_one<64, false, true, false, int>(a, c);
+        return c.err;
     }
     const bool small = (2 * (size_t)a.n_faces - 1) <= 65535;
     const bool mtl_lds = (size_t)(a.n_materials + 1) * 2 * sizeof(float4) <= kLdsMtlMax;
+    const size_t elem = small ? 2 : 4;
     if (a.env_is) {
         const bool pair_is = a.pair && (a.n_materials + 1) < (int)kNoProbe;
-        if (pair_is) grid.y = ((a.band_height + 7) / 8) * (a.n_frames > 0 ? a.n_frames : 1);
-        const size_t lds = trace_lds_bytes(a, 5, small ? 2 : 4, mtl_lds, pair_is ? 128 : 256, kLdsBudgetIS);
+        if (pair_is) c.tiles.y = ((a.band_height + 7) / 8) * nfr;
+        c.lds = LdsSpec{5, elem, mtl_lds, pair_is, false, TPT_TRACE_WAVES_IS};
         for_mtl_stack(mtl_lds, small, [&](auto m, auto st) {
-            if (pair_is) launch_ordered<true, decltype(m)::value, decltype(st), true, true>(a, grid, lds, s);
-            else launch_ordered<true, decltype(m)::value, decltype(st), false, true>(a, grid, lds, s);
+            if (pair_is) launch_ordered<true, decltype(m)::value, decltype(st), true, true>(a, c);
+            else launch_ordered<true, decltype(m)::value, decltype(st), false, true>(a, c);
         });
-        return hipGetLastError();
+        return c.err;
     }
     const bool lights = rec_words(a.n_lights, a.n_materials) == 5;
     if (a.quad) {
-        grid = dim3((a.width + 7) / 8, ((a.band_height + 7) / 8) * (a.n_frames > 0 ? a.n_frames : 1));
+        if (lights) return hipErrorInvalidValue;
+        c.tiles = dim3((a.width + 7) / 8, ((a.band_height + 7) / 8) * nfr);
         a.xcd_run = 0;
-        const size_t lds = trace_lds_bytes(a, 2, small ? 2 : 4, mtl_lds, 256, kLdsBudgetQuad, true);
-        if (lights || a.stack_lds_slots < a.stack_depth + 3) return hipErrorInvalidValue;
+        c.lds = LdsSpec{2, elem, mtl_lds, false, true, TPT_TRACE_WAVES_QUAD};
         for_mtl_stack(mtl_lds, small, [&](auto m, auto st) {
-            launch_quad<decltype(m)::value, decltype(st)>(a, grid, lds, s);
+            launch_quad<decltype(m)::value, decltype(st)>(a, c);
         });
-        return hipGetLastError();
+        return c.err;
     }
     const bool pair = a.pair && lights && a.n_lights > 0 && (a.n_materials + 1) < (int)kNoProbe;
     if (pair) {
-        grid.y = ((a.band_height + 7) / 8) * (a.n_frames > 0 ? a.n_frames : 1);
-        const size_t lds = trace_lds_bytes(a, 5, small ? 2 : 4, mtl_lds, 128, kLdsBudgetPair);
+        c.tiles.y = ((a.band_height + 7) / 8) * nfr;
+        c.lds = LdsSpec{5, elem, mtl_lds, true, false, TPT_TRACE_WAVES_PAIR};
         for_mtl_stack(mtl_lds, small, [&](auto m, auto st) {
-            launch_ordered<true, decltype(m)::value, decltype(st), true>(a, grid, lds, s);
+            launch_ordered<true, decltype(m)::value, decltype(st), true>(a, c);
         });
-        return hipGetLastError();
-    }
-    const size_t lds = trace_lds_bytes(a, lights ? 5 : 2, small ? 2 : 4, mtl_lds);
+        return c.err;
+    }
+    c.lds = LdsSpec{lights ? 5 : 2, elem, mtl_lds, false, false, TPT_TRACE_WAVES};
     for_mtl_stack(mtl_lds, small, [&](auto m, auto st) {
-        if (lights) launch_ordered<true, decltype(m)::value, decltype(st)>(a, grid, lds, s);
-        else launch_ordered<false, decltype(m)::value, decltype(st)>(a, grid, lds, s);
+        if (lights) launch_ordered<true, decltype(m)::value, decltype(st)>(a, c);
+        else launch_ordered<false, decltype(m)::value, decltype(st)>(a, c);
     });
-    return hipGetLastError();
+    return c.err;
+}
+
+hipError_t launch_trace(const TraceArgs& a, hipStream_t s, int32_t* shape) {
+    return launch_trace_impl(a, s, false, shape);
+}
+
+bool trace_quad_fits(const TraceArgs& a_in) {
+    if (rec_words(a_in.n_lights, a_in.n_materials) != 2) return false;
+    TraceArgs a = a_in;
+    a.quad = 1;
+    a.env_is = 0;
+    a.flags &= ~TPT_FLAG_REF_ORDER;
+    return launch_trace_impl(a, nullptr, true, nullptr) == hipSuccess;
 }
 
 constexpr int kLatStackSlots = 64;
@@ -1149,7 +1257,9 @@
     return hipGetLastError();
 }
 
-hipError_t launch_trace_ptr(const void* a, hipStream_t s) { return launch_trace(*static_cast<const TraceArgs*>(a), s); }
+hipError_t launch_trace_ptr(const void* a, hipStream_t s, int32_t* shape) {
+    return launch_trace(*static_cast<const TraceArgs*>(a), s, shape);
+}
 
 hipError_t launch_resolve(const ResolveArgs& a, hipStream_t s) {
     dim3 grid((a.width + 255) / 256, a.band_height);
diff --git a/tinypathtracer_amd/csrc/kernels/trace_dev.hpp b/tinypathtracer_amd/csrc/kernels/trace_dev.hpp
--- a/tinypathtracer_amd/csrc/kernels/trace_dev.hpp
+++ b/tinypathtracer_amd/csrc/kernels/trace_dev.hpp
@@ -39,7 +39,32 @@
 #define TPT_TRACE_WAVES_QUAD 4
 #endif
 
+#ifdef TPT_WG_WAVES
+#define TPT_WGW_LANE TPT_WG_WAVES
+#define TPT_WGW_DRAIN TPT_WG_WAVES
+#define TPT_WGW_PAIR TPT_WG_WAVES
+#define TPT_WGW_IS TPT_WG_WAVES
+#define TPT_WGW_QUAD TPT_WG_WAVES
+#define TPT_WGW_REF TPT_WG_WAVES
+#else
+#define TPT_WGW_LANE 1
+#define TPT_WGW_DRAIN 1
+#define TPT_WGW_PAIR 4
+#define TPT_WGW_IS 4
+#define TPT_WGW_QUAD 4
+#define TPT_WGW_REF 4
+#endif
+
 namespace tpt {
+
+template <bool ORDERED, bool ENVIS, bool PAIR, bool DRAIN, bool QUAD>
+constexpr int trace_wgw() {
+    constexpr int w = !ORDERED ? TPT_WGW_REF
+                               : (ENVIS ? TPT_WGW_IS
+                                        : (PAIR ? TPT_WGW_PAIR : (QUAD ? TPT_WGW_QUAD : (DRAIN ? TPT_WGW_DRAIN : TPT_WGW_LANE))));
+    static_assert(w == 1 || w == 2 || w == 4, "waves per k_trace workgroup: 1, 2 or 4");
+    return w;
+}
 
 #define TPT_LDS __attribute__((address_space(3)))
 struct alignas(16) LdsF4 {
@@ -170,14 +195,14 @@
 
 constexpr int kMaxStackSlots = 160 + 3;
 
-template <typename StackT, bool QS = false>
+template <typename StackT, bool QS = false, int ROW = 256>
 struct LaneStack {
     TPT_LDS StackT* lds;
     int nlds;
     StackT deep[kMaxStackSlots];
     __device__ static __forceinline__ int off(int i) {
-        if constexpr (QS) return (i >> 2) * 256 + (i & 3);
-        else return i * 256;
+        if constexpr (QS) return (i >> 2) * ROW + (i & 3);
+        else return i * ROW;
     }
     __device__ __forceinline__ void put(int i, int v) {
         if (i < nlds) lds[off(i)] = (StackT)v;
@@ -188,9 +213,9 @@
     }
 };
 
-template <typename StackT, bool QS>
+template <typename StackT, bool QS, int ROW>
 __device__ __forceinline__ int inner_visit4_q(const Trav& r, float4 q0, float4 q1, float4 q2, float4 q3, float4 q4,
-                                              float4 q5, float4 q6, LaneStack<StackT, QS>& stk, int& sp) {
+                                              float4 q5, float4 q6, LaneStack<StackT, QS, ROW>& stk, int& sp) {
     float k0, k1, k2, k3, e0, e1, e2, e3;
     slab_minmax(r.o, r.inv, q0.x, q0.y, q0.z, q0.w, q1.x, q1.y, k0, e0);
     slab_minmax(r.o, r.inv, q1.z, q1.w, q2.x, q2.y, q2.z, q2.w, k1, e1);
@@ -247,9 +272,9 @@
     sp += np;
     return i0;
 }
-template <typename StackT, bool QS>
+template <typename StackT, bool QS, int ROW>
 __device__ __forceinline__ int inner_visit4(const Trav& r, const float4* __restrict__ inner4, int nlds_nodes,
-                                            LaneStack<StackT, QS>& stk, int& sp) {
+                                            LaneStack<StackT, QS, ROW>& stk, int& sp) {
     const float4* nd = inner4 + 8 * r.node;
     return inner_visit4_q(r, nd[0], nd[1], nd[2], nd[3], nd[4], nd[5], nd[6], stk, sp);
 }
@@ -316,10 +341,10 @@
     r.fid = take ? f2 : r.fid;
     r.mode = take ? m2 : r.mode;
 }
-template <typename StackT, bool QS>
+template <typename StackT, bool QS, int ROW>
 __device__ __forceinline__ int inner_visit4_quad(Trav& r, const float4* __restrict__ inner4,
                                                  const float4* __restrict__ tri, int nint, float cull_eps,
-                                                 LaneStack<StackT, QS>& stk, int& sp, bool& stop, uint32_t& c_leaf) {
+                                                 LaneStack<StackT, QS, ROW>& stk, int& sp, bool& stop, uint32_t& c_leaf) {
     const int lane = (int)__lane_id(), k = lane & 3;
     const float* nf = (const float*)(inner4 + 8 * (size_t)r.node);
     const float2 b0 = *(const float2*)(nf + 6 * k), b1 = *(const float2*)(nf + 6 * k + 2),
```

Result: faster. 16130, median of 6 (+2.7%).
